# brownvc/gftorf

Hardware: AMD Instinct MI355X
Metric: train iters/sec (fwd+bwd raster) + Mpix/s, 1M Gaussians @ 640x480 ToF (higher is better)
Workload: dtype f32; 1 GPU; 1M Gaussians, 640x480, SH deg 3, RGB+ToF phasor, forward+backward; P=1000000, W=640, H=480, sh_degree=3, P_visible=954168, num_rendered=3638471, longest_tile_list=0

## Files before the change

### gftorf_amd/_lib.py

```python
import ctypes as C
import os

_HERE = os.path.dirname(os.path.abspath(__file__))
LIB_PATH = os.path.join(_HERE, "libgftorf_rast.so")
ABI_VERSION = 16
DEFORM_MAX_INPUTS = 96
ACC_STRIDE = 16

_lib = None

_fp = C.c_void_p


class Config(C.Structure):
    _fields_ = [
        ("P", C.c_int32), ("D", C.c_int32), ("M", C.c_int32), ("M_p", C.c_int32),
        ("W", C.c_int32), ("H", C.c_int32),
        ("tanfovx", C.c_float), ("tanfovy", C.c_float), ("scale_modifier", C.c_float),
        ("near_n", C.c_float), ("far_n", C.c_float), ("depth_range", C.c_float),
        ("phase_offset", C.c_float), ("dc_offset", C.c_float),
        ("use_view_dependent_phase", C.c_int32), ("prefiltered", C.c_int32), ("debug", C.c_int32),
        ("want_backward", C.c_int32),
        ("acc_zeroed", C.c_int32),
        ("grads_zeroed", C.c_int32),
        ("grads_accumulate", C.c_int32),
        ("bg_stride_c", C.c_int64), ("bg_stride_y", C.c_int64), ("bg_stride_x", C.c_int64),
    ]


FORWARD_FIELDS = [
    "bg", "means3D", "colors_precomp", "phasors_precomp", "opacities", "scales", "rotations",
    "cov3D_precomp", "viewmatrix", "projmatrix", "campos", "shs", "shs_p",
    "geom", "img", "binning",
    "out_color", "out_phasor", "out_depth", "out_normal", "out_acc", "out_entropy",
    "out_depth_distortion", "out_amp_distortion", "pixels", "out_distribution", "radii", "acc",
]

BACKWARD_FIELDS = [
    "bg", "means3D", "radii", "scales", "rotations", "cov3D_precomp", "viewmatrix", "projmatrix",
    "campos", "shs", "shs_p", "opacities", "pixels",
    "dL_dout_color", "dL_dout_phasor", "dL_dout_depth", "dL_dout_acc", "dL_dout_depth_distortion",
    "geom", "img", "binning", "acc",
    "dL_dmeans3D", "dL_dmeans2D", "dL_dcolors", "dL_dopacity", "dL_dcov3D", "dL_dsh", "dL_dsh_p",
    "dL_dscales", "dL_drotations", "dL_dphase_offset", "dL_ddc_offset", "det_partials", "dirty_rows", "rows_report",
    "phase_offset_dev", "dc_offset_dev",
]

LAYOUT_FIELDS = [
    "geom_rec_a", "geom_rec_b", "geom_depth", "geom_tiles", "geom_rect", "geom_dirgrad", "geom_clamped", "geom_need",
    "geom_blockhist", "geom_total",
    "img_pix_state", "img_ranges", "img_tile_max", "img_ctrl", "img_tile_cnt", "img_tile_cut", "img_super_tab", "img_tile_cursor",
    "img_tile_order", "img_front_len", "img_unit_flag", "img_resume_state", "img_pix_sums", "img_snaps", "img_total",
    "bin_keys", "bin_point_list", "bin_total",
]

PROFILE_FIELDS = ["preprocess_fwd_ms", "tile_count_ms", "tile_scatter_ms", "tile_sort_ms",
                  "render_fwd_ms", "render_bwd_ms", "preprocess_bwd_ms", "memset_ms"]


class ForwardIO(C.Structure):
    _fields_ = [(n, _fp) for n in FORWARD_FIELDS] + [("grads_zero", _fp), ("grads_zero_bytes", C.c_size_t), ("tile_hints", _fp), ("tile_weights", _fp),
                                                           ("cell_sched", _fp), ("phase_offset_dev", _fp), ("dc_offset_dev", _fp)]


class BackwardIO(C.Structure):
    _fields_ = [(n, _fp) for n in BACKWARD_FIELDS]


class Layout(C.Structure):
    _fields_ = [(n, C.c_size_t) for n in LAYOUT_FIELDS]


class ForwardHints(C.Structure):
    _fields_ = [("binning_instances", C.c_int64), ("max_tile_list", C.c_int64), ("whole_lists", C.c_int64),
                ("use_cell_sched", C.c_int64)]


class ForwardReport(C.Structure):
    _fields_ = [("num_rendered", C.c_int64), ("max_tile_list", C.c_int64), ("list_entries", C.c_int64), ("hinted_tiles", C.c_int64),
                ("sched_misses", C.c_int64)]


class Profile(C.Structure):
    _fields_ = [(n, C.c_double) for n in PROFILE_FIELDS] + [("forward_calls", C.c_int64),
                                                           ("backward_calls", C.c_int64)]


ASSEMBLE_PTRS_IN = ["xyz", "screenspace", "opacity", "scaling", "rotation", "rotation_raw", "feat_color",
                    "feat_phasor", "motion_mask", "d_xyz", "d_rot", "d_sh", "d_sh_p"]
ASSEMBLE_SCALARS = ["d_xyz_scalar", "d_rot_scalar", "d_sh_scalar", "d_sh_p_scalar"]
ASSEMBLE_PTRS_OUT = ["scratch", "out_means3D", "out_means2D", "out_opacity", "out_scales", "out_rotations",
                     "out_shs", "out_shs_p"]
ASSEMBLE_RAW_FLAGS = ["opacity_is_raw", "scaling_is_raw"]
ASSEMBLE_PARTS = ["feat_dc_color", "feat_rest_color", "phase_dc", "phase_rest", "amp_dc", "amp_rest"]
ASSEMBLE_FIELDS = ASSEMBLE_PTRS_IN + ASSEMBLE_SCALARS + ASSEMBLE_PTRS_OUT + ["num_offset_rows"] + ASSEMBLE_RAW_FLAGS + ASSEMBLE_PARTS
ASSEMBLE_BWD_HEAD = ["scratch", "rotation_raw", "d_rot"]
ASSEMBLE_BWD_TAIL = ["g_means3D", "g_means2D", "g_opacity", "g_scales", "g_rotations", "g_shs", "g_shs_p",
                     "g_xyz", "g_screenspace", "g_opacity_in", "g_scaling", "g_rotation", "g_rotation_raw",
                     "g_feat_color", "g_feat_phasor", "g_d_xyz", "g_d_rot", "g_d_sh", "g_d_sh_p"]
ASSEMBLE_BWD_RAW = ["opacity_raw", "scaling_raw", "g_feat_dc_color", "g_feat_rest_color", "g_phase_dc", "g_phase_rest", "g_amp_dc", "g_amp_rest"]
ASSEMBLE_BWD_FIELDS = ASSEMBLE_BWD_HEAD + ["d_rot_scalar"] + ASSEMBLE_BWD_TAIL + ["static_from_raw"] + ASSEMBLE_BWD_RAW


class AssembleIO(C.Structure):
    _fields_ = ([(n, _fp) for n in ASSEMBLE_PTRS_IN] + [(n, C.c_float) for n in ASSEMBLE_SCALARS] +
                [(n, _fp) for n in ASSEMBLE_PTRS_OUT] + [("num_offset_rows", C.c_int64)] +
                [(n, C.c_int32) for n in ASSEMBLE_RAW_FLAGS] + [(n, _fp) for n in ASSEMBLE_PARTS])


class AssembleBwdIO(C.Structure):
    _fields_ = ([(n, _fp) for n in ASSEMBLE_BWD_HEAD] + [("d_rot_scalar", C.c_float)] +
                [(n, _fp) for n in ASSEMBLE_BWD_TAIL] + [("static_from_raw", C.c_int32)] + [(n, _fp) for n in ASSEMBLE_BWD_RAW])


class DeformParams(C.Structure):
    _fields_ = [("linear_w", _fp * 8), ("linear_b", _fp * 8), ("xyz_w", _fp), ("xyz_b", _fp), ("r_w", _fp), ("r_b", _fp),
                ("g_w", _fp), ("g_b", _fp), ("b_w", _fp), ("b_b", _fp)]


DEFORM_FIELDS = [f[0] for f in DeformParams._fields_]


class AdamTensor(C.Structure):
    _fields_ = [("param", _fp), ("grad", _fp), ("exp_avg", _fp), ("exp_avg_sq", _fp), ("n", C.c_int64), ("lr", C.c_double),
                ("step", C.c_int64)]

EXPORTS = [
    "gft_abi_version", "gft_lazy_sort", "gft_last_error", "gft_geom_bytes", "gft_image_bytes", "gft_cell_sched_words", "gft_binning_bytes", "gft_acc_bytes",
    "gft_det_partials_bytes", "gft_get_layout", "gft_binning_capacity", "gft_set_binning_mode", "gft_binning_mode", "gft_set_render_mode", "gft_forward_preprocess", "gft_forward_render", "gft_forward", "gft_forward_enqueue", "gft_backward", "gft_grads_rezero",
    "gft_mark_visible", "gft_profile_enable", "gft_profile_reset", "gft_profile_read",
    "gft_assemble_scratch_bytes", "gft_assemble_forward", "gft_assemble_num_dynamic", "gft_assemble_backward",
    "gft_knn_scratch_bytes", "gft_knn_mean_dist2", "gft_adam_step",
    "gft_deform_inputs", "gft_deform_packed_bytes", "gft_deform_saved_bytes", "gft_deform_scratch_bytes", "gft_deform_pack",
    "gft_deform_forward", "gft_deform_backward", "gft_deform_compact", "gft_deform_rows_work_bytes", "gft_deform_backward_rows",
    "gft_deform_dw_splits", "gft_deform_rows_splits_capacity",
    "gft_ssim_blocks", "gft_ssim_l2_forward", "gft_ssim_l2_backward",
    "gft_image_loss_forward", "gft_image_loss_backward", "gft_pixel_loss_blocks", "gft_pixel_loss_forward", "gft_pixel_loss_backward",
    "gft_grad_norm_scratch_bytes", "gft_grad_norm", "gft_grad_scale",
    "gft_densify_stats", "gft_rows_rank_scratch_bytes", "gft_rows_rank", "gft_rows_rank_dev", "gft_rows_gather", "gft_rows_any_nonzero",
    "gft_densify_plan_scratch_bytes", "gft_densify_classify", "gft_densify_layout", "gft_rows_remap",
    "gft_split_children",
]
FLOW_EXPORTS = ["gft_flow_loss_blocks", "gft_flow_loss_forward", "gft_flow_loss_backward", "gft_flow_points", "gft_flow_project",
                "gft_flow_project_backward"]
FEATURE_EXPORTS = ["gft_render_features", "gft_render_features_backward"]
REG_EXPORTS = ["gft_reg_blocks", "gft_reg_result_words", "gft_reg_forward", "gft_reg_backward"]
REG_PARTIAL_WORDS = 8
REG_MEANS, REG_COUNTS, REG_RECIPS, REG_TOTAL = 0, 4, 6, 10
TOF_EXPORTS = ["gft_tof_depth", "gft_tof_log_blocks", "gft_tof_log_row"]
TOF_PARTIAL_WORDS = 12
TOF_LOG_WORDS, TOF_LOG_MAX_EXTRAS = 24, 8
TOF_LOG_FLOATS = ("sp", "sp_tof", "gsp", "sp_err", "sp_tof_err", "depth_err", "tof_depth_err", "amp_err", "dd", "gs_sp",
                  "gs_sp_visible")
TOF_LOG_VISIBLE, TOF_LOG_PRESENT, TOF_LOG_NUM_EXTRAS, TOF_LOG_SEQ, TOF_LOG_EXTRAS = 11, 12, 13, 14, 16
TOF_HAS_GT_DEPTH, TOF_HAS_DD, TOF_HAS_AMP, TOF_HAS_VISIBLE = 1, 2, 4, 8
QUERY_EXPORTS = ["gft_query_inputs", "gft_query_combine", "gft_query_combine_backward"]
QUERY_MAX_TIMES, QUERY_MAX_OUTPUTS = 4, 4
METRICS_EXPORTS = ["gft_metrics_blocks", "gft_view_metrics", "gft_metrics_reset"]
METRICS_VALUES = ("l1", "psnr", "l1_p", "l2_p", "psnr_p", "l1_d", "l2_d", "l2_d_tof")
METRICS_MAX_PLANES, METRICS_PARTIAL_WORDS = 8, 36
METRICS_ROW_MSE, METRICS_ROW_PSNR, METRICS_ROW_PRESENT, METRICS_ROW_PLANES, METRICS_ROW_WORDS = 8, 16, 24, 25, 28
METRICS_ACC_SUMS, METRICS_ACC_VIEWS, METRICS_ACC_PRESENT, METRICS_ACC_WORDS = 0, 16, 17, 18
METRICS_HAS_COLOUR, METRICS_HAS_TOF, METRICS_HAS_DEPTH, METRICS_HAS_TOF_DEPTH = 1, 2, 4, 8
PRESENT_EXPORTS = ["gft_present_blocks", "gft_present_sheet_bytes", "gft_present_magma", "gft_present_view", "gft_present_ranges",
                   "gft_present_ranges_reset", "gft_present_seismic", "gft_present_quad"]
PRESENT_IMAGES = (("color", 3, "uint8", lambda H, W: (H, W, 3)), ("real", 3, "uint8", lambda H, W: (H, W, 3)),
                  ("imag", 3, "uint8", lambda H, W: (H, W, 3)), ("amp", 1, "uint8", lambda H, W: (H, W)),
                  ("quad", 4, "uint8", lambda H, W: (4, H, W)), ("depth", 4, "uint8", lambda H, W: (H, W, 4)),
                  ("depth_tof", 4, "uint8", lambda H, W: (H, W, 4)), ("depth_norm", 4, "uint8", lambda H, W: (H, W, 4)),
                  ("dd", 1, "uint8", lambda H, W: (H, W)), ("depth_tof_f", 4, "float32", lambda H, W: (H, W)),
                  ("depth_norm_f", 4, "float32", lambda H, W: (H, W)))
PRESENT_HAS_COLOR, PRESENT_HAS_PHASOR, PRESENT_HAS_QUAD, PRESENT_HAS_DEPTH, PRESENT_HAS_ACC, PRESENT_HAS_DD = 1, 2, 4, 8, 16, 32
PRESENT_ALIGN, PRESENT_PARTIAL_WORDS, PRESENT_RANGE_WORDS, PRESENT_MAGMA_ROWS = 16, 2, 6, 257
PRESENT_SEISMIC_ROWS = 257
FLOWVIZ_EXPORTS = ["gft_flowviz_blocks", "gft_flowviz_wheel", "gft_flowviz_images"]
FLOWVIZ_WHEEL_ROWS, FLOWVIZ_IMAGES, FLOWVIZ_RUN = 55, 3, 4
TRACKS_EXPORTS = ["gft_tracks_integrate", "gft_tracks_table_bytes", "gft_tracks_table"]
TRACKS_PARTS = ("index", "xy", "motion", "step_ok")
PLY_EXPORTS = ["gft_ply_pack", "gft_ply_unpack"]
PLY_ROWS, PLY_MAX_SOURCES, PLY_MAX_COLUMNS = 64, 16, 240
PCD_EXPORTS = ["gft_pcd_unproject", "gft_pcd_row_bytes", "gft_pcd_pack", "gft_pcd_unpack", "gft_pcd_create"]
PCD_ROWS, PCD_MAX_ROW_BYTES, PCD_STATUS_WORDS = 256, 128, 2
PCD_MODES = ("torf_init", "ftorf_init", "proxy")
PCD_FIELDS = ("x", "y", "z", "nx", "ny", "nz", "red", "green", "blue", "phase", "amplitude", "seg_red", "seg_green", "seg_blue")


def load():
    global _lib
    if _lib is not None:
        return _lib
    if not os.path.exists(LIB_PATH):
        raise RuntimeError(
            "gftorf_amd: %s is missing. Build it with `python -m gftorf_amd.build` "
            "(hipcc, gfx950). There is no CPU fallback for the rasterizer." % LIB_PATH)
    lib = C.CDLL(LIB_PATH)
    lib.gft_abi_version.restype = C.c_int
    if lib.gft_abi_version() != ABI_VERSION:
        raise RuntimeError("gftorf_amd: libgftorf_rast.so ABI %d != expected %d, rebuild"
                           % (lib.gft_abi_version(), ABI_VERSION))
    lib.gft_last_error.restype = C.c_char_p
    lib.gft_geom_bytes.restype = C.c_size_t
    lib.gft_geom_bytes.argtypes = [C.c_int32]
    lib.gft_image_bytes.restype = C.c_size_t
    lib.gft_image_bytes.argtypes = [C.c_int32, C.c_int32]
    lib.gft_cell_sched_words.restype = C.c_size_t
    lib.gft_cell_sched_words.argtypes = [C.c_int32, C.c_int32]
    lib.gft_binning_bytes.restype = C.c_size_t
    lib.gft_binning_bytes.argtypes = [C.c_int64, C.c_int32, C.c_int32]
    lib.gft_acc_bytes.restype = C.c_size_t
    lib.gft_acc_bytes.argtypes = [C.c_int32]
    lib.gft_det_partials_bytes.restype = C.c_size_t
    lib.gft_det_partials_bytes.argtypes = [C.c_int64, C.c_int32, C.c_int32]
    lib.gft_binning_capacity.restype = C.c_int64
    lib.gft_binning_capacity.argtypes = [C.c_size_t, C.c_int32, C.c_int32]
    lib.gft_set_binning_mode.restype = C.c_int
    lib.gft_set_binning_mode.argtypes = [C.c_int]
    lib.gft_set_render_mode.restype = C.c_int
    lib.gft_set_render_mode.argtypes = [C.c_int]
    lib.gft_binning_mode.restype = C.c_int
    lib.gft_binning_mode.argtypes = [C.POINTER(Config)]
    lib.gft_get_layout.restype = C.c_int
    lib.gft_get_layout.argtypes = [C.c_int32, C.c_int32, C.c_int32, C.c_int64, C.POINTER(Layout)]
    lib.gft_forward_preprocess.restype = C.c_int
    lib.gft_forward_preprocess.argtypes = [C.c_void_p, C.POINTER(Config), C.POINTER(ForwardIO),
                                           C.POINTER(C.c_int64), C.POINTER(C.c_int64)]
    lib.gft_forward_render.restype = C.c_int
    _ptrs = C.POINTER(C.c_void_p)
    lib.gft_adam_step.restype = C.c_int
    lib.gft_adam_step.argtypes = [C.c_void_p, C.c_int32, C.POINTER(AdamTensor), C.c_int64, C.c_void_p, _ptrs, _ptrs, C.c_void_p,
                                  C.c_double, C.c_double, C.c_double, C.c_double, C.c_void_p]
    lib.gft_grad_norm_scratch_bytes.restype = C.c_size_t
    lib.gft_grad_norm_scratch_bytes.argtypes = [C.c_int64, C.c_int32]
    lib.gft_grad_norm.restype = C.c_int
    lib.gft_grad_norm.argtypes = [C.c_void_p, C.c_int32, _ptrs, C.POINTER(C.c_int64), C.c_double, C.c_void_p, C.c_size_t, C.c_void_p]
    lib.gft_grad_scale.restype = C.c_int
    lib.gft_grad_scale.argtypes = [C.c_void_p, C.c_int32, _ptrs, C.POINTER(C.c_int64), C.c_void_p]
    lib.gft_deform_packed_bytes.restype = C.c_size_t
    lib.gft_deform_packed_bytes.argtypes = []
    lib.gft_deform_saved_bytes.restype = C.c_size_t
    lib.gft_deform_saved_bytes.argtypes = [C.c_int64]
    lib.gft_deform_scratch_bytes.restype = C.c_size_t
    lib.gft_deform_scratch_bytes.argtypes = [C.c_int64]
    lib.gft_deform_pack.restype = C.c_int
    lib.gft_deform_inputs.restype = C.c_int
    lib.gft_deform_inputs.argtypes = [C.c_int, C.c_int]
    lib.gft_deform_pack.argtypes = [C.c_void_p, C.c_int, C.c_int, C.POINTER(DeformParams), C.c_void_p]
    lib.gft_deform_forward.restype = C.c_int
    lib.gft_deform_forward.argtypes = [C.c_void_p, C.c_int, C.c_int, C.c_int64, C.c_void_p, C.c_void_p, C.c_int64, C.c_void_p, C.c_void_p,
                                       C.c_void_p, C.c_void_p]
    lib.gft_deform_backward.restype = C.c_int
    lib.gft_deform_backward.argtypes = [C.c_void_p, C.c_int, C.c_int, C.c_int64, C.c_void_p, C.c_void_p, C.c_void_p, C.c_void_p, C.c_void_p,
                                        C.POINTER(DeformParams)]
    lib.gft_deform_compact.restype = C.c_int
    lib.gft_deform_compact.argtypes = [C.c_void_p, C.c_int64, C.c_int64] + [C.c_void_p] * 9
    lib.gft_deform_rows_work_bytes.restype = C.c_size_t
    lib.gft_deform_rows_work_bytes.argtypes = [C.c_int64]
    lib.gft_deform_dw_splits.restype = C.c_int
    lib.gft_deform_dw_splits.argtypes = [C.c_int64]
    lib.gft_deform_rows_splits_capacity.restype = C.c_int
    lib.gft_deform_rows_splits_capacity.argtypes = [C.c_int64]
    lib.gft_deform_backward_rows.restype = C.c_int
    lib.gft_deform_backward_rows.argtypes = [C.c_void_p, C.c_int, C.c_int, C.c_int64, C.c_void_p, C.c_void_p, C.c_void_p, C.c_int64, C.c_void_p,
                                             C.c_void_p, C.c_void_p, C.POINTER(DeformParams), C.c_void_p]
    lib.gft_ssim_blocks.restype = C.c_int64
    lib.gft_ssim_blocks.argtypes = [C.c_int32, C.c_int32, C.c_int32]
    lib.gft_ssim_l2_forward.restype = C.c_int
    lib.gft_ssim_l2_forward.argtypes = [C.c_void_p, C.c_int32, C.c_int32, C.c_int32, C.c_void_p, C.c_void_p, C.POINTER(C.c_float),
                                        C.c_void_p, C.c_void_p]
    lib.gft_ssim_l2_backward.restype = C.c_int
    lib.gft_ssim_l2_backward.argtypes = [C.c_void_p, C.c_int32, C.c_int32, C.c_int32, C.c_void_p, C.c_void_p, C.POINTER(C.c_float),
                                         C.c_void_p, C.c_void_p, C.c_void_p, C.c_float, C.c_float, C.c_void_p]
    _kind_sizes = [C.c_void_p, C.c_int32, C.c_int32, C.c_int32, C.c_int32, C.c_int32, C.c_float, C.c_void_p, C.c_void_p]
    lib.gft_image_loss_forward.restype = C.c_int
    lib.gft_image_loss_forward.argtypes = _kind_sizes + [C.POINTER(C.c_float), C.c_void_p, C.c_void_p]
    lib.gft_image_loss_backward.restype = C.c_int
    lib.gft_image_loss_backward.argtypes = _kind_sizes + [C.POINTER(C.c_float), C.c_void_p, C.c_void_p, C.c_void_p, C.c_float,
                                                          C.c_float, C.c_void_p]
    lib.gft_pixel_loss_blocks.restype = C.c_int64
    lib.gft_pixel_loss_blocks.argtypes = [C.c_int32, C.c_int32, C.c_int32]
    lib.gft_pixel_loss_forward.restype = C.c_int
    lib.gft_pixel_loss_forward.argtypes = _kind_sizes + [C.c_float, C.c_void_p]
    lib.gft_pixel_loss_backward.restype = C.c_int
    lib.gft_pixel_loss_backward.argtypes = _kind_sizes + [C.c_void_p, C.c_float, C.c_void_p]
    _flow_cams = [C.c_void_p, C.c_int32, C.c_int32] + [C.c_void_p] * 5
    lib.gft_flow_loss_blocks.restype = C.c_int64
    lib.gft_flow_loss_blocks.argtypes = [C.c_int32, C.c_int32]
    lib.gft_flow_loss_forward.restype = C.c_int
    lib.gft_flow_loss_forward.argtypes = _flow_cams + [C.c_void_p] * 4 + [C.c_float, C.c_void_p]
    lib.gft_flow_loss_backward.restype = C.c_int
    lib.gft_flow_loss_backward.argtypes = _flow_cams + [C.c_void_p] * 6 + [C.c_float, C.c_void_p, C.c_void_p]
    lib.gft_flow_points.restype = C.c_int
    lib.gft_flow_points.argtypes = _flow_cams + [C.c_void_p, C.c_void_p]
    lib.gft_flow_project.restype = C.c_int
    lib.gft_flow_project.argtypes = [C.c_void_p, C.c_int32, C.c_int32] + [C.c_void_p] * 6
    lib.gft_flow_project_backward.restype = C.c_int
    lib.gft_flow_project_backward.argtypes = [C.c_void_p, C.c_int32, C.c_int32] + [C.c_void_p] * 6
    _feat_frame = [C.c_void_p, C.POINTER(Config)] + [C.c_void_p] * 3 + [C.c_int64, C.c_int32]
    lib.gft_render_features.restype = C.c_int
    lib.gft_render_features.argtypes = _feat_frame + [C.c_void_p] * 3
    lib.gft_render_features_backward.restype = C.c_int
    lib.gft_render_features_backward.argtypes = _feat_frame + [C.c_void_p] * 3
    _reg_inputs = ([C.c_void_p, C.c_int64, C.c_int64, C.c_int64, C.c_void_p, C.c_void_p, C.c_void_p, C.c_int32, C.c_void_p, C.c_int32,
                    C.c_int32, C.c_void_p, C.c_int32])
    _reg_weights = [C.c_void_p, C.c_float, C.c_float, C.c_float, C.c_float]
    lib.gft_reg_blocks.restype = C.c_int64
    lib.gft_reg_blocks.argtypes = [C.c_int64, C.c_int64, C.c_int64]
    lib.gft_reg_result_words.restype = C.c_int64
    lib.gft_reg_result_words.argtypes = []
    lib.gft_reg_forward.restype = C.c_int
    lib.gft_reg_forward.argtypes = _reg_inputs + [C.c_void_p] + _reg_weights + [C.c_void_p, C.c_void_p]
    lib.gft_reg_backward.restype = C.c_int
    lib.gft_reg_backward.argtypes = _reg_inputs + _reg_weights + [C.c_void_p] * 6
    lib.gft_tof_depth.restype = C.c_int
    lib.gft_tof_depth.argtypes = [C.c_void_p, C.c_int64, C.c_void_p, C.c_int64, C.c_void_p, C.c_float, C.c_void_p, C.c_float, C.c_void_p]
    lib.gft_tof_log_blocks.restype = C.c_int64
    lib.gft_tof_log_blocks.argtypes = [C.c_int64, C.c_int64]
    lib.gft_tof_log_row.restype = C.c_int
    lib.gft_tof_log_row.argtypes = [C.c_void_p, C.c_int64, C.c_int64, C.c_void_p, C.c_int64, C.c_void_p, C.c_void_p, C.c_int64, C.c_void_p,
                                    C.c_float, C.c_void_p, C.c_float, C.c_float, C.c_void_p, C.c_void_p, C.c_void_p, C.c_int64, C.c_void_p,
                                    C.c_int32, _ptrs, C.c_int32, C.c_void_p, C.c_void_p, C.c_int64, C.c_void_p]
    lib.gft_query_inputs.restype = C.c_int
    lib.gft_query_inputs.argtypes = [C.c_void_p, C.c_int64, C.c_void_p, C.c_void_p, C.c_void_p, C.c_void_p, C.c_int64, C.c_int32, C.c_float,
                                     C.c_void_p, C.POINTER(C.c_float), C.c_void_p, C.c_void_p]
    lib.gft_query_combine.restype = C.c_int
    lib.gft_query_combine.argtypes = [C.c_void_p, C.c_int64, C.c_int32, C.c_int32, C.c_void_p, C.c_void_p, C.POINTER(C.c_float), _ptrs]
    lib.gft_query_combine_backward.restype = C.c_int
    lib.gft_query_combine_backward.argtypes = [C.c_void_p, C.c_int64, C.c_int32, C.c_int32, _ptrs, C.c_void_p, C.POINTER(C.c_float),
                                               C.c_void_p]
    lib.gft_metrics_blocks.restype = C.c_int64
    lib.gft_metrics_blocks.argtypes = [C.c_int64]
    lib.gft_view_metrics.restype = C.c_int
    lib.gft_view_metrics.argtypes = ([C.c_void_p] + [C.c_int64, C.c_int32, C.c_void_p, C.c_int64, C.c_void_p, C.c_int64] * 2 +
                                     [C.c_void_p, C.c_void_p, C.c_void_p, C.c_int64, C.c_void_p, C.c_float, C.c_void_p, C.c_float,
                                      C.c_void_p, C.c_void_p, C.c_void_p])
    lib.gft_metrics_reset.restype = C.c_int
    lib.gft_metrics_reset.argtypes = [C.c_void_p, C.c_void_p]
    lib.gft_present_blocks.restype = C.c_int64
    lib.gft_present_blocks.argtypes = [C.c_int64]
    lib.gft_present_sheet_bytes.restype = C.c_int64
    lib.gft_present_sheet_bytes.argtypes = [C.c_int32, C.c_int32, C.c_int32, C.POINTER(C.c_int64)]
    lib.gft_present_magma.restype = C.POINTER(C.c_uint8)
    lib.gft_present_magma.argtypes = []
    lib.gft_present_view.restype = C.c_int
    lib.gft_present_view.argtypes = [C.c_void_p, C.c_int32, C.c_int32, C.c_void_p, C.c_int64, C.c_void_p, C.c_int64, C.c_int32, C.c_void_p,
                                     C.c_void_p, C.c_void_p, C.c_void_p, C.POINTER(C.c_float), C.c_void_p, C.c_float, C.c_void_p, C.c_float,
                                     C.c_float, C.c_float, C.c_float, C.c_void_p, C.c_void_p]
    lib.gft_present_ranges.restype = C.c_int
    lib.gft_present_ranges.argtypes = [C.c_void_p, C.c_int64, C.c_void_p, C.c_int64, C.c_void_p, C.c_void_p]
    lib.gft_present_ranges_reset.restype = C.c_int
    lib.gft_present_ranges_reset.argtypes = [C.c_void_p, C.c_void_p]
    lib.gft_present_seismic.restype = C.POINTER(C.c_uint8)
    lib.gft_present_seismic.argtypes = []
    lib.gft_present_quad.restype = C.c_int
    lib.gft_present_quad.argtypes = [C.c_void_p, C.c_int32, C.c_int32, C.c_void_p, C.c_int64, C.POINTER(C.c_int32), C.c_int32, C.c_int32,
                                     C.c_void_p]
    lib.gft_flowviz_blocks.restype = C.c_int64
    lib.gft_flowviz_blocks.argtypes = [C.c_int64]
    lib.gft_flowviz_wheel.restype = C.POINTER(C.c_uint8)
    lib.gft_flowviz_wheel.argtypes = []
# ... 148 lines not shown
```

### gftorf_amd/api.py

```python
import ctypes as C
import struct as _struct
from typing import NamedTuple, Optional

import torch
import torch.nn as nn

from . import _lib


class GaussianRasterizationSettings(NamedTuple):
    image_height: int
    image_width: int
    tanfovx: float
    tanfovy: float
    bg: torch.Tensor
    scale_modifier: float
    viewmatrix: torch.Tensor
    projmatrix: torch.Tensor
    sh_degree: int
    campos: torch.Tensor
    prefiltered: bool
    debug: bool
    near_n: Optional[float] = 0.01
    far_n: Optional[float] = 100.0
# ... 373 lines not shown


def _scratch(nbytes, dev):
    t = torch.empty((nbytes,), device=dev, dtype=torch.uint8)
    if _POISON:
        t.fill_(0x7f)
    return t


def binning_capacity(binning, W, H):
    return int(_lib.load().gft_binning_capacity(binning.numel(), int(W), int(H)))


class _Settings(NamedTuple):
    bg: torch.Tensor
    scale_modifier: float
    viewmatrix: torch.Tensor
    projmatrix: torch.Tensor
    tanfovx: float
    tanfovy: float
    image_height: int
    image_width: int
    sh_degree: int
    campos: torch.Tensor
    prefiltered: bool
    debug: bool
    near_n: float
    far_n: float
    depth_range: float
    use_view_dependent_phase: bool


_PLANE_SPLIT = (3, 7, 1, 3, 1, 1, 1, 1, 3)
_FWD_FMT = "=%dQ" % len(_lib.ForwardIO._fields_)
_BWD_FMT = "=%dQ" % len(_lib.BackwardIO._fields_)
assert _struct.calcsize(_FWD_FMT) == C.sizeof(_lib.ForwardIO) and _struct.calcsize(_BWD_FMT) == C.sizeof(_lib.BackwardIO)


def _p0(t):
    return 0 if t is None else t.data_ptr()


def _save_snapshot(cpu_args, path, note):
    if cpu_args is not None:
        torch.save(cpu_args, path)
        print(note)


def _forward_inputs(s, means3D, sh, sh_p, colors_precomp, phasors_precomp, opacities, scales, rotations, cov3Ds_precomp, H, W):
    dev = means3D.device
    g = lambda t, n: _f32(t, dev, n) if _present(t) else None
    means3D_c = _f32(means3D, dev, "means3D") if means3D.size(0) else means3D
    sh_c, sh_p_c = g(sh, "shs"), g(sh_p, "shs_p")
    colors_c, phasors_c = g(colors_precomp, "colors_precomp"), g(phasors_precomp, "phasors_precomp")
    opac_c = g(opacities, "opacities")
    scales_c, rot_c, cov_c = g(scales, "scales"), g(rotations, "rotations"), g(cov3Ds_precomp, "cov3D_precomp")
    consts = (_f32(s.viewmatrix, dev, "viewmatrix"), _f32(s.projmatrix, dev, "projmatrix"), _f32(s.campos, dev, "campos"))
    return ((means3D_c, opac_c, sh_c, sh_p_c, scales_c, rot_c, cov_c, colors_c, phasors_c), consts,
            _bg_strides(s.bg, H, W, dev))


def _forward_buffers(lib, dev, P, H, W):
    planes = torch.empty((21, H, W), device=dev, dtype=torch.float32)
    radii = torch.empty((P,), device=dev, dtype=torch.int32)
    pixels = torch.empty((P, 1), device=dev, dtype=torch.float32)
    gb = state.geom_bytes.get(P)
    if gb is None:
        gb = state.geom_bytes[P] = int(lib.gft_geom_bytes(P))
    ib = state.image_bytes.get((W, H))
    if ib is None:
        ib = state.image_bytes[(W, H)] = int(lib.gft_image_bytes(W, H))
    return planes, radii, pixels, _scratch(gb, dev), _scratch(ib, dev)


def _pack_forward_io(inputs, consts, bg_c, planes, pixels, radii, geom, img, off_dev):
    means3D_c, opac_c, sh_c, sh_p_c, scales_c, rot_c, cov_c, colors_c, phasors_c = inputs
    P = radii.size(0)
    io = _lib.ForwardIO()
    pl, hw4 = planes.data_ptr(), 4 * planes.size(1) * planes.size(2)
    _struct.pack_into(_FWD_FMT, io, 0,
                      _p0(bg_c), means3D_c.data_ptr() if P else 0, _p0(colors_c), _p0(phasors_c), _p0(opac_c), _p0(scales_c),
                      _p0(rot_c), _p0(cov_c), consts[0].data_ptr(), consts[1].data_ptr(), consts[2].data_ptr(), _p0(sh_c),
                      _p0(sh_p_c), geom.data_ptr(), img.data_ptr(), 0,
                      pl, pl + 3 * hw4, pl + 10 * hw4, pl + 11 * hw4, pl + 14 * hw4, pl + 15 * hw4, pl + 16 * hw4, pl + 17 * hw4,
                      pixels.data_ptr() if P else 0, pl + 18 * hw4, radii.data_ptr() if P else 0, 0, 0, 0, 0, 0, 0,
                      *((0, 0) if off_dev is None else (_p0(off_dev[0]), _p0(off_dev[1]))))
    return io


def _update_hint(key, R, max_list=None, decay=0.95):
    prev_r, prev_l = state.instance_hint.get(key, (0, 0))
    r = max(R, int((prev_r or 0) * decay))
    state.instance_hint[key] = (r, prev_l if max_list is None else max(max_list, int(prev_l * 0.95)))
    if len(state.instance_hint) > state.MAX_SHAPES:
        state.instance_hint.pop(next(iter(state.instance_hint)))
    return r


class _Launch:
    __slots__ = ("lib", "stream", "cfg", "io", "dev", "W", "H", "cam", "use_sched")

    def __init__(self, lib, stream, cfg, io, dev, W, H, cam, use_sched):
        self.lib, self.stream, self.cfg, self.io, self.dev, self.W, self.H = lib, stream, C.byref(cfg), io, dev, W, H
        self.cam, self.use_sched = cam, use_sched

    def alloc_binning(self, cap):
        binning = _scratch(self.lib.gft_binning_bytes(cap, self.W, self.H), self.dev)
        self.io.binning = binning.data_ptr()
        return binning

    def hints(self, cap, list_hint, use_sched=0):
        n_tiles = ((self.W + 15) // 16) * ((self.H + 15) // 16)
        return _lib.ForwardHints(binning_instances=cap, max_tile_list=int(list_hint * _LIST_HEADROOM) + 1,
                                 whole_lists=_whole_lists(self.cam, n_tiles), use_cell_sched=use_sched)



def _forward_no_host_read(fr, st, hint_key, hint, list_hint):
    a = st["np"]
    if int(a[_ST_OVERFLOWS]) != st["seen"]:
        n_over, st["seen"] = int(a[_ST_OVERFLOWS]) - st["seen"], int(a[_ST_OVERFLOWS])
        worst = int(a[_ST_MAX_R])
        _update_hint(hint_key, worst, decay=1)
        raise RuntimeError("gftorf_amd: %d earlier no-host-read forward(s) of this shape had up to %d instances, "
                           "more than their binning buffer held: their outputs were undefined (the buffer has "
                           "been enlarged for the following frames)" % (n_over, worst))
    if a[3]:
        prev_R = int(a[0])
        a[3] = 0
        if fr.cam is not None:
            fr.cam.hinted_tiles = int(a[8])
        if a[1] & 1:
            raise RuntimeError("Point is filtered although prefiltered is set. This shouldn't happen!")
        hint = _update_hint(hint_key, prev_R)
    cap = _guess_cap(hint)
    binning = fr.alloc_binning(cap)
    hints = fr.hints(cap, list_hint)
    _lib.check(fr.lib.gft_forward_enqueue(fr.stream, fr.cfg, C.byref(fr.io), C.byref(hints), st["dev"].data_ptr()))
    st["host"].copy_(st["dev"], non_blocking=True)
    return -1, cap, binning, 0, False


def _forward_first_frame(fr, hint_key):
    _status_of(hint_key, fr.dev, create=True)
    num_rendered, max_list = C.c_int64(0), C.c_int64(0)
    _lib.check(fr.lib.gft_forward_preprocess(fr.stream, fr.cfg, C.byref(fr.io), C.byref(num_rendered), C.byref(max_list)))
    R = int(num_rendered.value)
    cap = _canonical_cap(R)
    binning = fr.alloc_binning(cap)
    _lib.check(fr.lib.gft_forward_render(fr.stream, fr.cfg, C.byref(fr.io), cap, int(max_list.value)))
    return R, cap, binning, int(max_list.value), False


def _forward_hinted(fr, hint, list_hint):
    cap = _guess_cap(hint, (fr.cam.cell_sched.numel() - 4) // 2 if fr.use_sched else 0)
    binning = fr.alloc_binning(cap)
    hints = fr.hints(cap, list_hint, fr.use_sched)
    report = _lib.ForwardReport()
    _lib.check(fr.lib.gft_forward(fr.stream, fr.cfg, C.byref(fr.io), C.byref(hints), C.byref(report)))
    R, max_list = int(report.num_rendered), int(report.max_tile_list)
    if fr.cam is not None:
        fr.cam.take_report(report, fr.use_sched, R <= cap)
    if R <= cap:
        return R, cap, binning, max_list, False
    cap = _canonical_cap(R)
    binning = fr.alloc_binning(cap)
    _lib.check(fr.lib.gft_forward_render(fr.stream, fr.cfg, C.byref(fr.io), cap, max_list))
    return R, cap, binning, max_list, True


def _launch_forward(fr, hint_key, capturing, nowait):
    hint, list_hint = state.instance_hint.get(hint_key, (None, 0))
    st = _status_of(hint_key, fr.dev, create=not capturing) if (nowait and hint is not None) else None
    if st is not None:
        return _forward_no_host_read(fr, st, hint_key, hint, list_hint)
    if nowait and capturing and hint is None:
        raise RuntimeError("gftorf_amd: a forward captured in a graph sizes its binning buffer from earlier frames of the "
                           "shape: render one frame of this shape (%d Gaussians, %dx%d) eagerly first" % hint_key[1:4])
    if nowait and capturing:
        raise RuntimeError("gftorf_amd: no status block for this shape: render one frame of it eagerly before capturing")
    r = _forward_first_frame(fr, hint_key) if hint is None else _forward_hinted(fr, hint, list_hint)
    _update_hint(hint_key, r[0], r[3])
    return r


def native_forward(s, means3D, sh, sh_p, colors_precomp, phasors_precomp, opacities, scales, rotations,
                   cov3Ds_precomp, ph_off, dc_off, want_bw, with_acc, stream=None, hint_slot=0, share_grads=None,
                   pre_launch=None, acc_any_stream=False, nowait=None, off_dev=None):
    lib = _lib.load()
    if means3D.dim() != 2 or means3D.size(1) != 3:
        raise RuntimeError("means3D must have dimensions (num_points, 3)")
    dev = means3D.device
    if dev.type != "cuda":
        raise RuntimeError("gftorf_amd: the rasterizer runs on a HIP device only (means3D is on %s); "
                           "there is no CPU path" % (dev,))
    capturing = torch.cuda.is_current_stream_capturing()
    if nowait is None:
        nowait = capturing or no_host_read
    if capturing and s.debug:
        raise RuntimeError("gftorf_amd: raster_settings.debug synchronises after every stage and cannot be captured in a graph")
    P = means3D.size(0)
    H, W = int(s.image_height), int(s.image_width)

    inputs, consts, bg = _forward_inputs(s, means3D, sh, sh_p, colors_precomp, phasors_precomp, opacities, scales, rotations,
                                         cov3Ds_precomp, H, W)
    means3D_c, opac_c, sh_c, sh_p_c, scales_c, rot_c, cov_c, colors_c, phasors_c = inputs
    cpu_args = None
    if s.debug:
        cpu_args = cpu_deep_copy_tuple((s.bg, means3D, colors_precomp, phasors_precomp, opacities, scales,
                                        rotations, s.scale_modifier, cov3Ds_precomp, s.viewmatrix, s.projmatrix,
                                        s.tanfovx, s.tanfovy, s.image_height, s.image_width, sh, sh_p,
                                        s.sh_degree, s.campos, s.prefiltered, s.debug, s.near_n, s.far_n,
                                        s.depth_range, s.use_view_dependent_phase, ph_off, dc_off))
    planes, radii, pixels, geom, img = _forward_buffers(lib, dev, P, H, W)
    cfg = _make_config(s, P, sh_c.size(1) if sh_c is not None else 0, sh_p_c.size(1) if sh_p_c is not None else 0, H, W,
                       ph_off, dc_off, bg[1:], want_bw)
    io = _pack_forward_io(inputs, consts, bg[0], planes, pixels, radii, geom, img, off_dev)

    lease = prep = None
    if want_bw and with_acc and P:
        lease = _take_acc(lib, dev, P, stream if stream is not None else _lib.raw_stream(dev), acc_any_stream, pooled=not capturing,
                          prezero=nowait and not capturing)
        if not lease.was_zero:
            io.acc = lease.buf.data_ptr()
        prep = prepare_backward(s, means3D_c, opac_c, sh_c, sh_p_c, scales_c, rot_c, cov_c, radii, geom, img, bg, consts,
                                ph_off, dc_off, lease.buf, colors_c is not None, cov_c is not None, want_bw, pixels,
                                share_grads=share_grads, acc_lease=lease, pooled=not capturing, off_dev=off_dev)
    acc_buf = lease.buf if lease is not None else None

    if P == 0:
        planes.zero_()
        R, cap, binning, max_list, restarted = 0, 0, torch.empty((0,), device=dev, dtype=torch.uint8), 0, False
    else:
        if stream is None:
            stream = _lib.raw_stream(dev)
        if pre_launch is not None:
            pre_launch()
        hint_key = (dev.index, P, W, H) if not hint_slot else (dev.index, P, W, H, hint_slot)
        tiles_key = (dev.index, W, H, hint_slot, s.viewmatrix.data_ptr() if _TILE_HINTS_PER_CAMERA else 0)
        cam = state.camera(tiles_key, create=not capturing) if _TILE_HINTS else None
        use_sched = cam.attach(io, lib, dev, W, H, capturing) if cam is not None else 0
        try:
            with _lib.on_device(dev):
                R, cap, binning, max_list, restarted = _launch_forward(
                    _Launch(lib, stream, cfg, io, dev, W, H, cam, use_sched), hint_key, capturing, nowait)
        except Exception:
            _save_snapshot(cpu_args, "snapshot_fw.dump",
                           "\nAn error occured in forward. Please forward snapshot_fw.dump for debugging.")
            raise
        if io.cell_sched:
            cam.sched_seen = True
    if prep is not None:
        prep.cap = cap
    if lease is not None:
        lease.zero = True

    last_call_stats.update(num_rendered=R, binning_instances=cap, restarted=restarted, max_tile_list=max_list)
    last_call_stats["forwards"] = last_call_stats.get("forwards", 0) + 1
    last_call_stats["restarts"] = last_call_stats.get("restarts", 0) + int(restarted)
    if keep_last_buffers:
        last_call_buffers.update(geom=geom, img=img, binning=binning, P=P, W=W, H=H, cap=cap)
    color, phasor, depth, normal, acc, entropy, depth_distortion, amp_distortion, distribution = planes.split(_PLANE_SPLIT)
    return dict(R=R, cap=cap, outputs=(color, phasor, depth, normal, acc, entropy, depth_distortion, amp_distortion,
                                       pixels, distribution, radii),
                geom=geom, binning=binning, img=img, acc=acc_buf, prep=prep, bg=bg, consts=consts, inputs=inputs)


class _Prep:
    __slots__ = ("grads", "cfg", "io", "acc", "acc_lease", "dev", "P", "H", "W", "pool_entry", "cap", "debug_args")

    def __init__(self, grads, cfg, io, acc, acc_lease, dev, P, H, W, pool_entry, debug_args):
        self.grads, self.cfg, self.io, self.acc, self.acc_lease = grads, cfg, io, acc, acc_lease
        self.dev, self.P, self.H, self.W = dev, P, H, W
        self.pool_entry, self.debug_args = pool_entry, debug_args
        self.cap = None


class _GradPlan(NamedTuple):
    shapes: dict
    sizes: dict
    total: int
    split_sizes: list
    layout_key: tuple
    numels: list


def _backward_plan(P, M, M_p, want_colors, want_cov, has_sh, has_sh_p, has_scales):
    plan_key = (P, M, M_p, want_colors, want_cov, has_sh, has_sh_p, has_scales)
    plan = state.bw_plans.get(plan_key)
    if plan is None:
        shapes = dict(means3D=(P, 3), means2D=(P, 3), opacities=(P, 1), colors=(P, 3) if want_colors else None,
                      cov3D=(P, 6) if want_cov else None, sh=(P, M, 3) if has_sh else None,
                      sh_p=(P, M_p, 2) if has_sh_p else None, scales=(P, 3) if has_scales else None,
                      rotations=(P, 4) if has_scales else None)
        sizes = {k: (_prod(v) + 3) // 4 * 4 for k, v in shapes.items() if v is not None}
        if len(state.bw_plans) > 64:
            state.bw_plans.clear()
        plan = state.bw_plans[plan_key] = _GradPlan(shapes, sizes, sum(sizes.values()) + 4, list(sizes.values()) + [4],
                                                    tuple(sorted(sizes.items())), [_prod(shapes[k]) for k in sizes])
    return plan


def _grad_views(buf, plan):
    pieces = buf.split(plan.split_sizes)
    g = dict.fromkeys(plan.shapes)
    for (k, size), piece, n in zip(plan.sizes.items(), pieces, plan.numels):
        g[k] = (piece if n == size else piece[:n]).view(plan.shapes[k])
    g["offsets"] = pieces[-1][:2]
# ... 246 lines not shown
```

### gftorf_amd/csrc/gft_api.hip

```cpp
#include "gft_internal.h"

#include <stdarg.h>
#include <stdio.h>
#include <string.h>
#include <cstdlib>
#include <mutex>
#include <vector>

static thread_local char g_err[512] = "";

int gft_fail(const char* fmt, ...)
{
    va_list ap;
    va_start(ap, fmt);
    vsnprintf(g_err, sizeof(g_err), fmt, ap);
    va_end(ap);
    return 1;
}

extern "C" const char* gft_last_error(void) { return g_err; }
extern "C" int gft_abi_version(void) { return GFT_ABI_VERSION; }
static size_t point_list_slots(int64_t binning_instances, int32_t W, int32_t H)
{
    if (binning_instances <= 0) return 0;
    const size_t T = (size_t)((W + GFT_TILE_X - 1) / GFT_TILE_X) * (size_t)((H + GFT_TILE_Y - 1) / GFT_TILE_Y);
    return T * (size_t)GFT_HEAD_SLOT + (size_t)binning_instances;
}
extern "C" size_t gft_det_partials_bytes(int64_t binning_instances, int32_t W, int32_t H)
{
    return point_list_slots(binning_instances, W, H) * 4 * GFT_ACC_STRIDE * sizeof(float);
}
extern "C" int64_t gft_binning_capacity(size_t bytes, int32_t W, int32_t H)
{
    const size_t T = (size_t)((W + GFT_TILE_X - 1) / GFT_TILE_X) * (size_t)((H + GFT_TILE_Y - 1) / GFT_TILE_Y);
    const size_t fixed = T * (size_t)GFT_HEAD_SLOT * 4 + GFT_ALIGN;
    if (bytes <= fixed) return 0;
    return (int64_t)((bytes - fixed) / 12);
}

static inline size_t align_up(size_t x) { return (x + GFT_ALIGN - 1) & ~(size_t)(GFT_ALIGN - 1); }

void gft_compute_layout(int32_t P, int32_t W, int32_t H, int64_t R, gft_layout* L)
{
    memset(L, 0, sizeof(*L));
    const size_t p = (size_t)(P > 0 ? P : 0);
    size_t o = 0;
    L->geom_rec_a = o;    o = align_up(o + p * 32);
    L->geom_rec_b = o;    o = align_up(o + p * 32);
    L->geom_depth = o;    o = align_up(o + p * 4);
    L->geom_tiles = o;    o = align_up(o + p * 4);
    L->geom_rect = o;     o = align_up(o + p * 8);
    L->geom_dirgrad = o;  o = align_up(o + p * 64);
    L->geom_clamped = o;  o = align_up(o + p);
    L->geom_need = o;     o = align_up(o + p);
    L->geom_blockhist = o; o = align_up(o + ((p + BIN_CHUNK - 1) / BIN_CHUNK) * GFT_BLOCKHIST_TILES * 2);
    L->geom_total = o;

    const size_t n = (size_t)W * (size_t)H;
    const size_t T = (size_t)((W + GFT_TILE_X - 1) / GFT_TILE_X) * (size_t)((H + GFT_TILE_Y - 1) / GFT_TILE_Y);
    o = 0;
    L->img_pix_state = o;   o = align_up(o + n * 16);
    L->img_ranges = o;      o = align_up(o + T * 8);
    L->img_tile_max = o;    o = align_up(o + T * 4 * 4);
    L->img_ctrl = o;        o += (GFT_CTRL_WORDS + GFT_TICKET_WORDS) * 4;
    L->img_tile_cnt = o;    o += T * 4;
    L->img_tile_cut = o;    o += T * 4;
    L->img_super_tab = o;   o = align_up(o + 4 * (size_t)GFT_SUPER_CELLS * 4);
    L->img_tile_cursor = o; o = align_up(o + T * 4);
    L->img_tile_order = o;  o = align_up(o + T * 4);
    L->img_front_len = o;   o = align_up(o + T * 4);
    L->img_unit_flag = o;   o = align_up(o + T * 16);
    L->img_resume_state = o; o = align_up(o + n * 64);
    L->img_pix_sums = o;    o = align_up(o + n * 32);
    L->img_snaps = o;       o = align_up(o + 4 * T * (size_t)(gft_bwd_segments(T) - 1) * GFT_SNAP_F4 * 64 * 16);
    L->img_total = o;

    const size_t r = (size_t)(R > 0 ? R : 0);
    o = 0;
    L->bin_keys = o;        o = align_up(o + r * 8);
    L->bin_point_list = o;  o = align_up(o + (r ? T * (size_t)GFT_HEAD_SLOT + r : 0) * 4);
    L->bin_total = o + GFT_ALIGN;
}

GeomView gft_geom_view(void* base, const gft_layout& L)
{
    char* b = (char*)base;
    GeomView g;
    g.rec_a = (float4*)(b + L.geom_rec_a);
    g.rec_b = (float4*)(b + L.geom_rec_b);
    g.depth = (float*)(b + L.geom_depth);
    g.tiles = (uint32_t*)(b + L.geom_tiles);
    g.rect = (ushort4*)(b + L.geom_rect);
    g.dirgrad = (float4*)(b + L.geom_dirgrad);
    g.clamped = (uint8_t*)(b + L.geom_clamped);
    g.need = (uint8_t*)(b + L.geom_need);
    g.blockhist = (uint16_t*)(b + L.geom_blockhist);
    return g;
}

ImgView gft_img_view(void* base, const gft_layout& L)
{
    char* b = (char*)base;
    ImgView v;
    v.pix_state = (float4*)(b + L.img_pix_state);
    v.ranges = (uint2*)(b + L.img_ranges);
    v.tile_max = (uint32_t*)(b + L.img_tile_max);
    v.ctrl = (uint32_t*)(b + L.img_ctrl);
    v.tile_cnt = (uint32_t*)(b + L.img_tile_cnt);
    v.tile_cut = (uint32_t*)(b + L.img_tile_cut);
    v.super_tab = (uint32_t*)(b + L.img_super_tab);
    v.tile_cursor = (uint32_t*)(b + L.img_tile_cursor);
    v.tile_order = (uint32_t*)(b + L.img_tile_order);
    v.front_len = (uint32_t*)(b + L.img_front_len);
    v.unit_flag = (uint32_t*)(b + L.img_unit_flag);
    v.resume_state = (float4*)(b + L.img_resume_state);
    v.pix_sums = (float4*)(b + L.img_pix_sums);
    v.snaps = (float4*)(b + L.img_snaps);
    return v;
}

BinView gft_bin_view(void* base, const gft_layout& L)
{
    char* b = (char*)base;
    BinView v;
    v.keys = (uint64_t*)(b + L.bin_keys);
    v.point_list = (uint32_t*)(b + L.bin_point_list);
    return v;
}

extern "C" size_t gft_geom_bytes(int32_t P)
{
    gft_layout L;
    gft_compute_layout(P, 16, 16, 0, &L);
    return L.geom_total + GFT_ALIGN;
}

extern "C" size_t gft_image_bytes(int32_t W, int32_t H)
{
    gft_layout L;
    gft_compute_layout(0, W, H, 0, &L);
    return L.img_total + GFT_ALIGN;
}

extern "C" size_t gft_cell_sched_words(int32_t W, int32_t H)
{
    gft_config c;
    memset(&c, 0, sizeof(c));
    c.W = W; c.H = H; c.near_n = 0.01f; c.far_n = 100.f;
    return (W > 0 && H > 0 && gft_tile_pull_ok(c)) ? gft_cell_sched_words_of(c) : 0;
}

extern "C" size_t gft_binning_bytes(int64_t R, int32_t W, int32_t H)
{
    gft_layout L;
    gft_compute_layout(0, W, H, R, &L);
    return L.bin_total;
}

extern "C" size_t gft_acc_bytes(int32_t P)
{
    const size_t p = (size_t)(P > 0 ? P : 0);
    return (p * GFT_ACC_STRIDE + 2 * ((p + 63) / 64) + 64) * sizeof(float);
}

extern "C" int gft_get_layout(int32_t P, int32_t W, int32_t H, int64_t R, gft_layout* out)
{
    if (!out) return gft_fail("gft_get_layout: out is NULL");
    gft_compute_layout(P, W, H, R, out);
    return 0;
}

enum Stage { ST_PRE_FWD, ST_TILE_COUNT, ST_TILE_SCATTER, ST_TILE_SORT, ST_RENDER_FWD, ST_RENDER_BWD, ST_PRE_BWD, ST_MEMSET, ST_COUNT };

struct Profiler {
    std::mutex mu;
    bool on = false;
    struct Rec { int stage; hipEvent_t a, b; };
    std::vector<Rec> pending;
    std::vector<hipEvent_t> pool;
    double ms[ST_COUNT] = {0};
    int64_t fwd = 0, bwd = 0;
    hipEvent_t get()
    {
        if (!pool.empty()) { hipEvent_t e = pool.back(); pool.pop_back(); return e; }
        hipEvent_t e;
        if (hipEventCreate(&e) != hipSuccess) return nullptr;
        return e;
    }
    void drain()
    {
        for (auto& r : pending) {
            float t = 0.f;
            if (hipEventSynchronize(r.b) == hipSuccess && hipEventElapsedTime(&t, r.a, r.b) == hipSuccess) ms[r.stage] += t;
            pool.push_back(r.a);
            pool.push_back(r.b);
        }
        pending.clear();
    }
};
static Profiler g_prof;

struct StageTimer {
    hipStream_t s; int stage; hipEvent_t a = nullptr, b = nullptr; bool on;
    StageTimer(hipStream_t s_, int st) : s(s_), stage(st), on(g_prof.on)
    {
        if (on) {
            std::lock_guard<std::mutex> lk(g_prof.mu);
            a = g_prof.get(); b = g_prof.get();
            if (a && b) (void)hipEventRecord(a, s); else on = false;
        }
    }
    ~StageTimer()
    {
        if (on) {
            (void)hipEventRecord(b, s);
            std::lock_guard<std::mutex> lk(g_prof.mu);
            g_prof.pending.push_back({stage, a, b});
        }
    }
};

extern "C" int gft_profile_enable(int on) { std::lock_guard<std::mutex> lk(g_prof.mu); g_prof.on = on != 0; return 0; }

extern "C" int gft_profile_reset(void)
{
    std::lock_guard<std::mutex> lk(g_prof.mu);
    g_prof.drain();
    memset(g_prof.ms, 0, sizeof(g_prof.ms));
    g_prof.fwd = g_prof.bwd = 0;
    return 0;
}

extern "C" int gft_profile_read(gft_profile* out)
{
    if (!out) return gft_fail("gft_profile_read: out is NULL");
    std::lock_guard<std::mutex> lk(g_prof.mu);
    g_prof.drain();
    out->preprocess_fwd_ms = g_prof.ms[ST_PRE_FWD];
    out->tile_count_ms = g_prof.ms[ST_TILE_COUNT];
    out->tile_scatter_ms = g_prof.ms[ST_TILE_SCATTER];
    out->tile_sort_ms = g_prof.ms[ST_TILE_SORT];
    out->render_fwd_ms = g_prof.ms[ST_RENDER_FWD];
    out->render_bwd_ms = g_prof.ms[ST_RENDER_BWD];
    out->preprocess_bwd_ms = g_prof.ms[ST_PRE_BWD];
    out->memset_ms = g_prof.ms[ST_MEMSET];
    out->forward_calls = g_prof.fwd;
    out->backward_calls = g_prof.bwd;
    return 0;
}

struct SideFill {
    hipStream_t stream = nullptr;
    hipEvent_t after_main = nullptr, filled = nullptr;
    bool pending = false;
};
static std::mutex g_side_mu;
static SideFill g_side[64];

static SideFill* side_of_current_device()
{
    int dev = 0;
    if (hipGetDevice(&dev) != hipSuccess || dev < 0 || dev >= 64) return nullptr;
    std::lock_guard<std::mutex> lk(g_side_mu);
    SideFill& f = g_side[dev];
    if (!f.stream) {
        if (hipStreamCreateWithFlags(&f.stream, hipStreamNonBlocking) != hipSuccess) { f.stream = nullptr; return nullptr; }
        if (hipEventCreateWithFlags(&f.after_main, hipEventDisableTiming) != hipSuccess ||
            hipEventCreateWithFlags(&f.filled, hipEventDisableTiming) != hipSuccess)
            return nullptr;
    }
    return &f;
}

#define GFT_STAGE(stream, cfg, name, call)                                                   \
    do {                                                                                     \
        hipError_t e_ = (call);                                                              \
        if (e_ != hipSuccess) return gft_fail("%s: launch failed: %s", name, hipGetErrorString(e_)); \
        if ((cfg)->debug) {                                                                  \
            e_ = hipStreamSynchronize(stream);                                               \
            if (e_ != hipSuccess) return gft_fail("%s: %s", name, hipGetErrorString(e_));    \
        }                                                                                    \
    } while (0)

__global__ __launch_bounds__(256) void k_zero_fill(uint4* __restrict__ p16, size_t n16, uint8_t* __restrict__ tail, size_t ntail)
{
    const size_t stride = (size_t)gridDim.x * 256;
    for (size_t i = (size_t)blockIdx.x * 256 + threadIdx.x; i < n16; i += stride) p16[i] = make_uint4(0u, 0u, 0u, 0u);
    if (blockIdx.x == 0 && threadIdx.x < ntail) tail[threadIdx.x] = 0;
}

__global__ void k_post_empty(uint32_t* status) { status[GFT_CTRL_SEQ] = 1u; }

hipError_t gft_zero_async(void* ptr, size_t bytes, hipStream_t s)
{
    if (!ptr || !bytes) return hipSuccess;
    uint8_t* p = static_cast<uint8_t*>(ptr);
    const size_t head = (16 - ((uintptr_t)p & 15)) & 15;
    if (head && head < bytes) {
        hipLaunchKernelGGL(k_zero_fill, dim3(1), dim3(256), 0, s, (uint4*)nullptr, (size_t)0, p, head);
        p += head; bytes -= head;
    } else if (head) {
        hipLaunchKernelGGL(k_zero_fill, dim3(1), dim3(256), 0, s, (uint4*)nullptr, (size_t)0, p, bytes);
// ... 53 lines not shown
    *dev_slot = g_mail.dev + (size_t)slot * GFT_CTRL_WORDS;
    *host_slot = g_mail.host + (size_t)slot * GFT_CTRL_WORDS;
    g_mail.host[(size_t)slot * GFT_CTRL_WORDS + GFT_CTRL_FLAGS] = 0u;
    return 0;
}

static int mailbox_wait(hipStream_t s, volatile uint32_t* host_slot, uint32_t seq, uint32_t out[GFT_CTRL_WORDS])
{
    for (;;) {
        for (int i = 0; i < 4096; i++) {
            if (__atomic_load_n(&host_slot[GFT_CTRL_SEQ], __ATOMIC_ACQUIRE) == seq) goto ready;
            __builtin_ia32_pause();
        }
        const hipError_t q = hipStreamQuery(s);
        if (q == hipSuccess) {
            if (__atomic_load_n(&host_slot[GFT_CTRL_SEQ], __ATOMIC_ACQUIRE) == seq) goto ready;
            return gft_fail("forward: the stream drained but the tile scan never reported");
        }
        if (q != hipErrorNotReady) return gft_fail("forward: %s", hipGetErrorString(q));
    }
ready:
    for (int i = 0; i < GFT_CTRL_WORDS; i++) out[i] = host_slot[i];
    return 0;
}

static int check_stage1(const gft_config* cfg, const gft_forward_io* io, const char* who)
{
    if (!io->means3D || !io->opacities || !io->viewmatrix || !io->projmatrix || !io->campos || !io->geom ||
        !io->radii || !io->pixels)
        return gft_fail("%s: required pointer is NULL", who);
    if ((io->shs == nullptr) == (io->colors_precomp == nullptr))
        return gft_fail("Please provide excatly one of either SHs or precomputed colors!");
    if ((io->scales == nullptr || io->rotations == nullptr) == (io->cov3D_precomp == nullptr))
        return gft_fail("Please provide exactly one of either scale/rotation pair or precomputed 3D covariance!");
    if ((io->shs != nullptr) != (cfg->M > 0) || (io->shs_p != nullptr) != (cfg->M_p > 0))
        return gft_fail("M / M_p do not match the presence of shs / shs_p");
    if (!io->img) return gft_fail("%s: img buffer is NULL", who);
    return 0;
}

static int check_stage2(const gft_forward_io* io, const char* who)
{
    if (!io->img || !io->bg || !io->out_color || !io->out_phasor || !io->out_depth || !io->out_normal ||
        !io->out_acc || !io->out_entropy || !io->out_depth_distortion || !io->out_amp_distortion ||
        !io->out_distribution)
        return gft_fail("%s: required pointer is NULL", who);
    return 0;
}

static bool lazy_sort_enabled()
{
    static const bool on = [] { const char* e = getenv("GFT_LAZY_SORT"); return e ? atoi(e) != 0 : true; }();
    return on;
}

extern "C" int gft_lazy_sort(void) { return lazy_sort_enabled() ? 1 : 0; }

static std::atomic<int> g_binning_mode{-1};
extern "C" int gft_set_binning_mode(int mode)
{
    g_binning_mode.store(mode < 0 ? -1 : (mode ? 1 : 0));
    return 0;
}
static bool pull_enabled(const gft_config* cfg)
{
    int m = g_binning_mode.load();
    if (m < 0) {
        const char* e = getenv("GFT_LAZY_BIN");
        m = e ? (atoi(e) != 0) : 1;
        g_binning_mode.store(m);
    }
    return m != 0 && lazy_sort_enabled() && gft_tile_pull_ok(*cfg);
}
extern "C" int gft_binning_mode(const gft_config* cfg) { return (cfg && pull_enabled(cfg)) ? 1 : 0; }

static std::atomic<int> g_render_mode{-2};
extern "C" int gft_set_render_mode(int mode)
{
    g_render_mode.store(mode < 0 ? -2 : (mode ? 1 : 0));
    return 0;
}
int gft_render_mode()
{
    int m = g_render_mode.load();
    if (m == -2) {
        const char* e = getenv("GFT_FWD_SEG");
        m = e ? (atoi(e) != 0 ? 1 : 0) : -1;
        g_render_mode.store(m);
    }
    return m;
}

static int enqueue_count(hipStream_t s, const gft_config* cfg, const gft_forward_io* io, const GeomView& g, const ImgView& im,
                         uint32_t* mail_dev, uint32_t seq, bool pull, int64_t status_cap = -1);

static int enqueue_stage1(hipStream_t s, const gft_config* cfg, const gft_forward_io* io, const GeomView& g,
                          const ImgView& im, uint32_t* mail_dev, uint32_t seq, bool pull, bool count = true, int64_t status_cap = -1)
{
    {
        StageTimer t(s, ST_PRE_FWD);
        GFT_STAGE(s, cfg, "preprocess_fwd", gft_launch_preprocess_fwd(s, *cfg, *io, g, im, mail_dev, pull));
    }
    if (io->grads_zero && io->grads_zero_bytes) {
        SideFill* f = side_of_current_device();
        if (!f) return gft_fail("forward: no side stream for the gradient fill");
        GFT_CHECK_HIP(hipEventRecord(f->after_main, s));
        GFT_CHECK_HIP(hipStreamWaitEvent(f->stream, f->after_main, 0));
        GFT_CHECK_HIP(gft_zero_async(io->grads_zero, io->grads_zero_bytes, f->stream));
        GFT_CHECK_HIP(hipEventRecord(f->filled, f->stream));
        f->pending = true;
    }
    return count ? enqueue_count(s, cfg, io, g, im, mail_dev, seq, pull, status_cap) : 0;
}

static int enqueue_count(hipStream_t s, const gft_config* cfg, const gft_forward_io* io, const GeomView& g, const ImgView& im,
                         uint32_t* mail_dev, uint32_t seq, bool pull, int64_t status_cap)
{
    StageTimer t(s, ST_TILE_COUNT);
    if (pull) {
        BinView none;
        none.keys = nullptr; none.point_list = nullptr;
        const int T = ((cfg->W + GFT_TILE_X - 1) / GFT_TILE_X) * ((cfg->H + GFT_TILE_Y - 1) / GFT_TILE_Y);
        GFT_STAGE(s, cfg, "super_count", gft_launch_super_bin(s, *cfg, g, im, none, mail_dev, seq, 0, 0u,
                                                              gft_fwd_segmented(T) ? nullptr : io->tile_hints, io->cell_sched, status_cap));
    } else {
        GFT_STAGE(s, cfg, "tile_count", gft_launch_tile_count(s, *cfg, g, im, mail_dev, seq, status_cap));
    }
    return 0;
}

static int enqueue_stage2(hipStream_t s, const gft_config* cfg, const gft_forward_io* io, const GeomView& g,
                          const ImgView& im, const BinView& b, bool binned, int64_t max_tile_list, bool check_cap,
                          uint32_t cap, bool pull, bool whole_lists, uint32_t* sched_mail = nullptr, uint32_t sched_seq = 0u)
{
    float* clear = (io->acc && cfg->want_backward && cfg->P > 0) ? io->acc : nullptr;
    const size_t clear_bytes = (size_t)cfg->P * GFT_ACC_STRIDE * sizeof(float);
    const bool lazy = binned && lazy_sort_enabled();
    pull = pull && binned;
    if (pull) {
        {
            StageTimer t(s, ST_TILE_SCATTER);
            if (sched_mail) {
                const int T0 = ((cfg->W + GFT_TILE_X - 1) / GFT_TILE_X) * ((cfg->H + GFT_TILE_Y - 1) / GFT_TILE_Y);
                GFT_STAGE(s, cfg, "super_append", gft_launch_super_bin(s, *cfg, g, im, b, sched_mail, sched_seq, 2, cap,
                                                                       gft_fwd_segmented(T0) ? nullptr : io->tile_hints, io->cell_sched));
            } else {
                GFT_STAGE(s, cfg, "super_scatter", gft_launch_super_bin(s, *cfg, g, im, b, nullptr, 0u, 1, cap));
            }
        }
        {
            StageTimer t(s, ST_TILE_SORT);
            const int T = ((cfg->W + GFT_TILE_X - 1) / GFT_TILE_X) * ((cfg->H + GFT_TILE_Y - 1) / GFT_TILE_Y);
            const uint32_t* th = gft_fwd_segmented(T) ? nullptr : io->tile_hints;
            GFT_STAGE(s, cfg, "tile_pull", gft_launch_tile_pull(s, *cfg, g, im, b, cap, clear, clear_bytes, th, whole_lists && th));
        }
        {
            StageTimer t(s, ST_PRE_FWD);
            GFT_STAGE(s, cfg, "appearance", gft_launch_appearance(s, *cfg, *io, g, im, cap));
        }
    } else if (binned) {
        {
            StageTimer t(s, ST_TILE_SCATTER);
            GFT_STAGE(s, cfg, "tile_scatter", gft_launch_tile_scatter(s, *cfg, g, im, b, cap, (int64_t)cap));
        }
        {
            StageTimer t(s, ST_TILE_SORT);
            if (lazy)
                GFT_STAGE(s, cfg, "tile_front", gft_launch_tile_front(s, *cfg, im, b, cap, clear, clear_bytes));
            else
                GFT_STAGE(s, cfg, "tile_sort", gft_launch_tile_sort(s, *cfg, max_tile_list, im, b, cap, clear, clear_bytes));
        }
    } else if (clear) {
        GFT_CHECK_HIP(gft_zero_async(clear, clear_bytes, s));
    }
    {
        StageTimer t(s, ST_RENDER_FWD);
        GFT_STAGE(s, cfg, "render_fwd", gft_launch_render_fwd(s, *cfg, *io, g, im, b, check_cap, cap, lazy ? 1 : 0, pull));
    }
    if (lazy) {
        {
            StageTimer t(s, ST_TILE_SORT);
            if (pull)
                GFT_STAGE(s, cfg, "tail_build", gft_launch_tail_build(s, *cfg, *io, g, im, b, cap, cfg->want_backward != 0));
            else
                GFT_STAGE(s, cfg, "tile_tail", gft_launch_tile_tail(s, *cfg, g, im, b, cap, cfg->want_backward != 0));
        }
        if (!(pull && gft_tail_resumes())) {
            StageTimer t(s, ST_RENDER_FWD);
            GFT_STAGE(s, cfg, "render_resume", gft_launch_render_fwd(s, *cfg, *io, g, im, b, check_cap, cap, 2, pull));
        }
    }
    if (g_prof.on) { std::lock_guard<std::mutex> lk(g_prof.mu); g_prof.fwd++; }
    return 0;
}

extern "C" int gft_forward_preprocess(void* hip_stream, const gft_config* cfg, const gft_forward_io* io,
                                      int64_t* num_rendered, int64_t* max_tile_list)
{
    if (max_tile_list) *max_tile_list = 0;
    if (check_config(cfg)) return 1;
    if (!io || !num_rendered) return gft_fail("gft_forward_preprocess: NULL argument");
    *num_rendered = 0;
    if (cfg->P == 0) return 0;
    if (check_stage1(cfg, io, "gft_forward_preprocess")) return 1;
    hipStream_t s = (hipStream_t)hip_stream;
    gft_layout L;
    gft_compute_layout(cfg->P, cfg->W, cfg->H, 0, &L);
    GeomView g = gft_geom_view(io->geom, L);
    ImgView im = gft_img_view(io->img, L);
    uint32_t* mail_dev; volatile uint32_t* mail_host; uint32_t seq;
    if (mailbox_acquire(&mail_dev, &mail_host, &seq)) return 1;
    if (enqueue_stage1(s, cfg, io, g, im, mail_dev, seq, pull_enabled(cfg))) return 1;
    uint32_t host[GFT_CTRL_WORDS];
    if (mailbox_wait(s, mail_host, seq, host)) return 1;
    if (host[GFT_CTRL_FLAGS] & 1u)
        return gft_fail("Point is filtered although prefiltered is set. This shouldn't happen!");
    *num_rendered = (int64_t)host[GFT_CTRL_TOTAL];
    if (max_tile_list) *max_tile_list = (int64_t)host[GFT_CTRL_MAXCNT];
    return 0;
}

extern "C" int gft_forward_render(void* hip_stream, const gft_config* cfg, const gft_forward_io* io,
                                  int64_t binning_instances, int64_t max_tile_list)
{
    if (check_config(cfg)) return 1;
    if (!io) return gft_fail("gft_forward_render: io is NULL");
    if (check_stage2(io, "gft_forward_render")) return 1;
    if (binning_instances < 0 || binning_instances > 0xffffffffll) return gft_fail("gft_forward_render: bad instance count");
    if (binning_instances > 0 && !io->binning) return gft_fail("gft_forward_render: binning buffer is NULL");
    if (cfg->P > 0 && (!io->geom || !io->radii || !io->pixels)) return gft_fail("gft_forward_render: geom/radii/pixels NULL");
    hipStream_t s = (hipStream_t)hip_stream;
    const int64_t R = cfg->P == 0 ? 0 : binning_instances;
    gft_layout L;
    gft_compute_layout(cfg->P, cfg->W, cfg->H, R, &L);
    GeomView g = gft_geom_view(io->geom, L);
    ImgView im = gft_img_view(io->img, L);
    BinView b = gft_bin_view(io->binning, L);
    const bool pull = cfg->P > 0 && pull_enabled(cfg);
    if (cfg->P == 0 || (pull && R == 0)) {
        const int gx = (cfg->W + GFT_TILE_X - 1) / GFT_TILE_X, gy = (cfg->H + GFT_TILE_Y - 1) / GFT_TILE_Y;
        GFT_CHECK_HIP(gft_zero_async(im.ranges, (size_t)gx * gy * sizeof(uint2), s));
        if (cfg->P == 0) GFT_CHECK_HIP(gft_zero_async(im.ctrl, GFT_CTRL_WORDS * sizeof(uint32_t), s));
    }
    return enqueue_stage2(s, cfg, io, g, im, b, R > 0, max_tile_list, cfg->P > 0, (uint32_t)R, pull, io->tile_hints != nullptr);
}

extern "C" int gft_forward(void* hip_stream, const gft_config* cfg, const gft_forward_io* io,
                           const gft_forward_hints* hints, gft_forward_report* report)
{
    if (report) memset(report, 0, sizeof(*report));
    if (check_config(cfg)) return 1;
    if (!io || !hints || !report) return gft_fail("gft_forward: NULL argument");
    if (check_stage2(io, "gft_forward")) return 1;
    const int64_t binning_instances = hints->binning_instances;
    if (binning_instances < 0 || binning_instances > 0xffffffffll) return gft_fail("gft_forward: bad instance count");
    if (cfg->P == 0) return gft_forward_render(hip_stream, cfg, io, 0, 0);
    if (check_stage1(cfg, io, "gft_forward")) return 1;
    if (binning_instances > 0 && !io->binning) return gft_fail("gft_forward: binning buffer is NULL");
    hipStream_t s = (hipStream_t)hip_stream;
    gft_layout L;
    gft_compute_layout(cfg->P, cfg->W, cfg->H, binning_instances, &L);
    GeomView g = gft_geom_view(io->geom, L);
    ImgView im = gft_img_view(io->img, L);
    BinView b = gft_bin_view(io->binning, L);
    uint32_t* mail_dev; volatile uint32_t* mail_host; uint32_t seq;
    if (mailbox_acquire(&mail_dev, &mail_host, &seq)) return 1;
    const bool pull = pull_enabled(cfg);
    const bool by_sched = pull && binning_instances > 0 && io->cell_sched != nullptr && hints->use_cell_sched != 0;
    if (enqueue_stage1(s, cfg, io, g, im, mail_dev, seq, pull, !by_sched)) return 1;
    if (pull && binning_instances == 0) {
        const int gx = (cfg->W + GFT_TILE_X - 1) / GFT_TILE_X, gy = (cfg->H + GFT_TILE_Y - 1) / GFT_TILE_Y;
        GFT_CHECK_HIP(gft_zero_async(im.ranges, (size_t)gx * gy * sizeof(uint2), s));
    }
    const uint32_t cap = (uint32_t)binning_instances;
    if (enqueue_stage2(s, cfg, io, g, im, b, binning_instances > 0, hints->max_tile_list, true, cap, pull, hints->whole_lists != 0,
                       by_sched ? mail_dev : nullptr, seq))
        return 1;
    uint32_t host[GFT_CTRL_WORDS];
    if (mailbox_wait(s, mail_host, seq, host)) return 1;
    if (by_sched && ((host[GFT_CTRL_FLAGS] & 2u) || host[GFT_CTRL_TOTAL] > cap)) {
        const size_t T = (size_t)((cfg->W + GFT_TILE_X - 1) / GFT_TILE_X) * (size_t)((cfg->H + GFT_TILE_Y - 1) / GFT_TILE_Y);
        GFT_CHECK_HIP(gft_zero_async(im.ctrl, (GFT_CTRL_WORDS + GFT_TICKET_WORDS + 2 * T + GFT_SUPER_CELLS) * sizeof(uint32_t), s));
        if (mailbox_acquire(&mail_dev, &mail_host, &seq)) return 1;
        mail_host[GFT_CTRL_FLAGS] = host[GFT_CTRL_FLAGS] & 1u;
        const bool render_again = host[GFT_CTRL_TOTAL] <= cap;
        if (enqueue_count(s, cfg, io, g, im, mail_dev, seq, pull)) return 1;
        if (render_again &&
            enqueue_stage2(s, cfg, io, g, im, b, true, hints->max_tile_list, true, cap, pull, hints->whole_lists != 0))
            return 1;
        if (mailbox_wait(s, mail_host, seq, host)) return 1;
        report->sched_misses = 1;
    }
    if (host[GFT_CTRL_FLAGS] & 1u)
        return gft_fail("Point is filtered although prefiltered is set. This shouldn't happen!");
    report->num_rendered = (int64_t)host[GFT_CTRL_TOTAL];
    report->max_tile_list = (int64_t)host[GFT_CTRL_MAXCNT];
    report->list_entries = pull ? (int64_t)host[GFT_CTRL_ENTRIES] : (int64_t)host[GFT_CTRL_TOTAL];
    report->hinted_tiles = pull ? (int64_t)host[GFT_CTRL_NHINT] : 0;
    if (!lazy_sort_enabled() && hints->max_tile_list > 0 && hints->max_tile_list <= GFT_SHORT_LIST_MAX &&
        host[GFT_CTRL_MAXCNT] > GFT_SHORT_LIST_MAX && host[GFT_CTRL_TOTAL] <= cap && binning_instances > 0) {
        GFT_CHECK_HIP(gft_zero_async(io->pixels, (size_t)cfg->P * sizeof(float), s));
        GFT_STAGE(s, cfg, "tile_sort_long", gft_launch_tile_sort_long(s, *cfg, im, b, cap));
        GFT_STAGE(s, cfg, "render_fwd", gft_launch_render_fwd(s, *cfg, *io, g, im, b, true, cap, 0, false));
    }
    return 0;
}

// ... 120 lines not shown
```

### gftorf_amd/csrc/gft_internal.h

```cpp
#pragma once
#include <hip/hip_runtime.h>
#include <stdint.h>
#include <stddef.h>
#include "gftorf_rast.h"

#include <atomic>
#include <cstdlib>

#define GFT_ALIGN 256

inline hipError_t gft_lds_opt_in(const void* kernel, size_t bytes, std::atomic<uint64_t>& done)
{
    int dev = 0;
    hipError_t e = hipGetDevice(&dev);
    if (e != hipSuccess) return e;
    const uint64_t bit = dev >= 0 && dev < 64 ? 1ull << dev : 0ull;
    if (bit && (done.load(std::memory_order_acquire) & bit)) return hipSuccess;
    e = hipFuncSetAttribute(kernel, hipFuncAttributeMaxDynamicSharedMemorySize, (int)bytes);
    if (e == hipSuccess && bit) done.fetch_or(bit, std::memory_order_release);
    return e;
}
#define GFT_BLOCK 256
#define GFT_NUM_ACC 15

struct GeomView {
    float4* rec_a;
    float4* rec_b;
    float* depth;
    uint32_t* tiles;
    ushort4* rect;
    float4* dirgrad;
    uint8_t* clamped;
    uint8_t* need;
    uint16_t* blockhist;
};

struct ImgView {
    float4* pix_state;
    float4* pix_sums;
    float4* snaps;
    uint2* ranges;
    uint32_t* tile_max;
    uint32_t* ctrl;
    uint32_t* tile_cnt;
    uint32_t* tile_cut;
    uint32_t* super_tab;
    uint32_t* tile_cursor;
    uint32_t* tile_order;
    uint32_t* front_len;
    uint32_t* unit_flag;
    float4* resume_state;
};

struct BinView {
    uint64_t* keys;
    uint32_t* point_list;
};

#define GFT_CTRL_TOTAL 0
#define GFT_CTRL_FLAGS 1
#define GFT_CTRL_MAXCNT 2
#define GFT_CTRL_NFLAG 4
#define GFT_CTRL_DONE 3
#define GFT_CTRL_SEQ 3
#define GFT_CTRL_ENTRIES 5
#define GFT_CTRL_POOLCUR 6
#define GFT_CTRL_DONE2 7
#define GFT_CTRL_NHINT 8
#define GFT_CTRL_RSUM 9
#define GFT_CTRL_FWDORDER 10
#define GFT_CTRL_ORDER_OK 11
#define GFT_CTRL_WORDS 16
__device__ __forceinline__ void gft_status_sticky(uint32_t* mail, uint32_t post, uint32_t R)
{
    if (!post) return;
    mail[GFT_STATUS_CAP] = post - 1u;
    if (R > post - 1u) {
        __hip_atomic_fetch_add(&mail[GFT_STATUS_OVERFLOWS], 1u, __ATOMIC_RELAXED, __HIP_MEMORY_SCOPE_SYSTEM);
        __hip_atomic_fetch_max(&mail[GFT_STATUS_MAX_R], R, __ATOMIC_RELAXED, __HIP_MEMORY_SCOPE_SYSTEM);
    }
}
#define GFT_TICKET_WORDS 32
#define GFT_SUPER_MAX 1024
#define GFT_SLAB_MAX 16
#define GFT_SUPER_CELLS (GFT_SUPER_MAX * GFT_SLAB_MAX)
#define GFT_DEPTH_BINS 4096
#define GFT_HEAD_SLOT 2048u
#define GFT_HEAD_DIRECT 2048u
#define GFT_HEAD_TARGET 940u
#define GFT_NO_TAIL 0xffffffffu
#define GFT_BLOCKHIST_TILES 2048
#ifndef BIN_THREADS
#define BIN_THREADS 1024
#endif
#ifndef BIN_ITEMS
#define BIN_ITEMS 4
#endif
#define BIN_CHUNK (BIN_THREADS * BIN_ITEMS)
#define GFT_SHORT_LIST_MAX 4096

#ifndef GFT_SEG_LEN
#define GFT_SEG_LEN 256
#endif
inline int gft_bwd_segments(size_t T)
{
    static const int cap = [] { const char* e = getenv("GFT_BWD_NSEG"); const int v = e ? atoi(e) : 0; return v > 0 ? (v > 8 ? 8 : v) : 8; }();
    const size_t v = 4 * (T ? T : 1);
    const size_t n = 65536 / v;
    return n < 1 ? 1 : (n > (size_t)cap ? cap : (int)n);
}
inline int gft_fwd_seg_waves(int T)
{
    static const int force = [] { const char* e = getenv("GFT_FWD_SEG_WAVES"); return e ? atoi(e) : 0; }();
    if (force > 0) return force > 8 ? 8 : force;
    const int n = 6144 / (4 * (T > 0 ? T : 1));
    return n < 1 ? 1 : (n > 8 ? 8 : n);
}
int gft_render_mode();
inline bool gft_fwd_segmented(int T) { return gft_render_mode() != 0 && gft_fwd_seg_waves(T) > 1; }
#define GFT_FWD_ORDER_MAX_TILES 4096
inline bool gft_fwd_ordered(int T) { return !gft_fwd_segmented(T) && T <= GFT_FWD_ORDER_MAX_TILES; }
#define GFT_SNAP_F4 3

void gft_compute_layout(int32_t P, int32_t W, int32_t H, int64_t R, gft_layout* L);
GeomView gft_geom_view(void* base, const gft_layout& L);
ImgView gft_img_view(void* base, const gft_layout& L);
BinView gft_bin_view(void* base, const gft_layout& L);

int gft_fail(const char* fmt, ...);
inline int gft_launched(const char* who)
{
    const hipError_t err = hipGetLastError();
    return err == hipSuccess ? 0 : gft_fail("%s: %s", who, hipGetErrorString(err));
}
hipError_t gft_zero_async(void* ptr, size_t bytes, hipStream_t s);
#define GFT_CHECK_HIP(expr)                                                          \
    do {                                                                             \
        hipError_t e_ = (expr);                                                      \
        if (e_ != hipSuccess)                                                        \
            return gft_fail("%s failed: %s (%s:%d)", #expr, hipGetErrorString(e_),   \
                            __FILE__, __LINE__);                                     \
    } while (0)

hipError_t gft_launch_preprocess_fwd(hipStream_t s, const gft_config& c, const gft_forward_io& io,
                                     const GeomView& g, const ImgView& im, uint32_t* mail, bool defer_appearance);
hipError_t gft_launch_appearance(hipStream_t s, const gft_config& c, const gft_forward_io& io, const GeomView& g,
                                 const ImgView& im, uint32_t cap);
hipError_t gft_launch_tile_count(hipStream_t s, const gft_config& c, const GeomView& g, const ImgView& im,
                                 uint32_t* mail, uint32_t seq, int64_t status_cap = -1);
hipError_t gft_launch_tile_scatter(hipStream_t s, const gft_config& c, const GeomView& g, const ImgView& im,
                                   const BinView& b, uint32_t cap, int64_t expect);
hipError_t gft_launch_tile_sort(hipStream_t s, const gft_config& c, int64_t max_tile_list, const ImgView& im,
                                const BinView& b, uint32_t cap, float* clear, size_t clear_bytes);
hipError_t gft_launch_tile_front(hipStream_t s, const gft_config& c, const ImgView& im, const BinView& b, uint32_t cap,
                                 float* clear, size_t clear_bytes);
hipError_t gft_launch_tile_tail(hipStream_t s, const gft_config& c, const GeomView& g, const ImgView& im,
                                const BinView& b, uint32_t cap, bool want_order);
hipError_t gft_launch_tile_sort_long(hipStream_t s, const gft_config& c, const ImgView& im, const BinView& b,
                                     uint32_t cap);
bool gft_tile_pull_ok(const gft_config& c);
bool gft_tail_resumes();
struct SuperShape { int gx, gy, T, sshift, sgx, sgy, NS, K, kshift; uint32_t near_bits; int bin_shift; };
SuperShape gft_super_shape(const gft_config& c);
hipError_t gft_launch_super_bin(hipStream_t s, const gft_config& c, const GeomView& g, const ImgView& im, const BinView& b,
                                uint32_t* mail, uint32_t seq, int pass, uint32_t cap, const uint32_t* hints = nullptr,
                                uint32_t* sched = nullptr, int64_t status_cap = -1);
size_t gft_cell_sched_words_of(const gft_config& c);
hipError_t gft_launch_tile_pull(hipStream_t s, const gft_config& c, const GeomView& g, const ImgView& im, const BinView& b,
                                uint32_t cap, float* clear, size_t clear_bytes, const uint32_t* hints, bool whole_lists);
hipError_t gft_launch_tail_build(hipStream_t s, const gft_config& c, const gft_forward_io& io, const GeomView& g,
                                 const ImgView& im, const BinView& b, uint32_t cap, bool want_order);
hipError_t gft_launch_render_fwd(hipStream_t s, const gft_config& c, const gft_forward_io& io,
                                 const GeomView& g, const ImgView& im, const BinView& b, bool check_cap, uint32_t cap,
                                 int lazy, bool pull, bool segmented = true);
hipError_t gft_launch_render_bwd(hipStream_t s, const gft_config& c, const gft_backward_io& io,
                                 const GeomView& g, const ImgView& im, const BinView& b, bool lazy, uint32_t cap);
hipError_t gft_launch_preprocess_bwd(hipStream_t s, const gft_config& c, const gft_backward_io& io,
                                     const GeomView& g);
hipError_t gft_launch_grads_rezero(hipStream_t s, const gft_config& c, const gft_backward_io& io);
hipError_t gft_launch_mark_visible(hipStream_t s, int32_t P, const float* means3D,
                                   const float* view, float near_n, float far_n, uint8_t* present);


#define GFT_DPP_ROW_SHR(n) (0x110 + (n))
#define GFT_DPP_ROW_BCAST15 0x142
#define GFT_DPP_ROW_BCAST31 0x143

__device__ __forceinline__ float gft_offset_value(const float* dev, float scalar)
{
    return dev != nullptr ? *dev : scalar;
}

__device__ __forceinline__ float gft_wave_sum_to_lane63(float v)
{
    v += __int_as_float(__builtin_amdgcn_update_dpp(0, __float_as_int(v), GFT_DPP_ROW_SHR(1), 0xf, 0xf, false));
    v += __int_as_float(__builtin_amdgcn_update_dpp(0, __float_as_int(v), GFT_DPP_ROW_SHR(2), 0xf, 0xf, false));
    v += __int_as_float(__builtin_amdgcn_update_dpp(0, __float_as_int(v), GFT_DPP_ROW_SHR(4), 0xf, 0xf, false));
    v += __int_as_float(__builtin_amdgcn_update_dpp(0, __float_as_int(v), GFT_DPP_ROW_SHR(8), 0xf, 0xf, false));
    v += __int_as_float(__builtin_amdgcn_update_dpp(0, __float_as_int(v), GFT_DPP_ROW_BCAST15, 0xa, 0xf, false));
    v += __int_as_float(__builtin_amdgcn_update_dpp(0, __float_as_int(v), GFT_DPP_ROW_BCAST31, 0xc, 0xf, false));
    return v;
}

__device__ __forceinline__ uint32_t gft_wave_sum_u32_to_lane63(uint32_t v)
{
    v += (uint32_t)__builtin_amdgcn_update_dpp(0, (int)v, GFT_DPP_ROW_SHR(1), 0xf, 0xf, false);
    v += (uint32_t)__builtin_amdgcn_update_dpp(0, (int)v, GFT_DPP_ROW_SHR(2), 0xf, 0xf, false);
    v += (uint32_t)__builtin_amdgcn_update_dpp(0, (int)v, GFT_DPP_ROW_SHR(4), 0xf, 0xf, false);
    v += (uint32_t)__builtin_amdgcn_update_dpp(0, (int)v, GFT_DPP_ROW_SHR(8), 0xf, 0xf, false);
    v += (uint32_t)__builtin_amdgcn_update_dpp(0, (int)v, GFT_DPP_ROW_BCAST15, 0xa, 0xf, false);
    v += (uint32_t)__builtin_amdgcn_update_dpp(0, (int)v, GFT_DPP_ROW_BCAST31, 0xc, 0xf, false);
    return v;
}

__device__ __forceinline__ void gft_get_rect(float px, float py, int radius, int gx, int gy,
                                             int& x0, int& y0, int& x1, int& y1)
{
    const float r = (float)radius;
    x0 = min(gx, max(0, (int)((px - r) / 16.0f)));
    y0 = min(gy, max(0, (int)((py - r) / 16.0f)));
    x1 = min(gx, max(0, (int)((((px + r) + 16.0f) - 1.0f) / 16.0f)));
    y1 = min(gy, max(0, (int)((((py + r) + 16.0f) - 1.0f) / 16.0f)));
}

__device__ __forceinline__ uint32_t gft_depth_bin(uint32_t dbits, uint32_t near_bits, int shift)
{
    const uint32_t d = dbits > near_bits ? dbits - near_bits : 0u;
    const uint32_t b = d >> shift;
    return b < GFT_DEPTH_BINS ? b : GFT_DEPTH_BINS - 1u;
}

__device__ __forceinline__ bool gft_splat_reaches_box(const float4& a0, const float4& a1, float bx0, float by0, float bw, float bh)
{
    const float ca = a0.z, cb = a0.w, cc = a1.x, op = a1.y;
    const float det = ca * cc - cb * cb;
    const float tau = __logf(255.0f * op);
    if (!(op >= 1.0f / 255.0f)) return false;
    if (!(det > 0.0f && ca > 0.0f && cc > 0.0f)) return true;
    const float ux0 = bx0 - a0.x, ux1 = ux0 + bw;
    const float uy0 = by0 - a0.y, uy1 = uy0 + bh;
    const float X = fminf(fmaxf(0.0f, ux0), ux1), Y = fminf(fmaxf(0.0f, uy0), uy1);
    const float ys = fminf(fmaxf(-cb * X * __frcp_rn(cc), uy0), uy1);
    const float xs = fminf(fmaxf(-cb * Y * __frcp_rn(ca), ux0), ux1);
    const float q1 = ca * X * X + 2.0f * cb * X * ys + cc * ys * ys;
    const float q2 = ca * xs * xs + 2.0f * cb * xs * Y + cc * Y * Y;
    return fminf(q1, q2) <= 2.0f * tau * 1.0005f + 0.01f;
}
__device__ __forceinline__ bool gft_splat_reaches_quadrant(const float4& a0, const float4& a1, float qx0, float qy0)
{
    return gft_splat_reaches_box(a0, a1, qx0, qy0, 7.0f, 7.0f);
}

#define GFT_FLAG_SET 0x80000000u
__device__ __forceinline__ uint32_t gft_flag_word(unsigned long long unsaturated)
{
    uint32_t c = (uint32_t)(unsaturated | (unsaturated >> 32));
    c |= c >> 16;
    c |= c >> 8;
    c &= 0xffu;
    const uint32_t x0 = (uint32_t)__builtin_ctz(c), x1 = 31u - (uint32_t)__builtin_clz(c);
    const uint32_t y0 = (uint32_t)__builtin_ctzll(unsaturated) >> 3, y1 = (63u - (uint32_t)__builtin_clzll(unsaturated)) >> 3;
    return GFT_FLAG_SET | x0 | (y0 << 3) | (x1 << 6) | (y1 << 9);
}
__device__ __forceinline__ bool gft_splat_reaches_flagged(uint32_t flag, const float4& a0, const float4& a1, float qx0, float qy0)
{
    if (!flag) return false;
    const uint32_t x0 = flag & 7u, y0 = (flag >> 3) & 7u, x1 = (flag >> 6) & 7u, y1 = (flag >> 9) & 7u;
    return gft_splat_reaches_box(a0, a1, qx0 + (float)x0, qy0 + (float)y0, (float)(x1 - x0), (float)(y1 - y0));
}

__device__ inline void gft_tile_order_block(int T, const uint32_t* __restrict__ quad_max, uint32_t* __restrict__ order,
                                            const uint32_t* __restrict__ flag = nullptr)
{
    constexpr int PER = 16;
    __shared__ uint32_t s_max;
    __shared__ uint32_t cnt[16][64];
    const int tid = threadIdx.x, lane = tid & 63, wave = tid >> 6;
    if (tid == 0) s_max = 0;
    for (int i = tid; i < 16 * 64; i += (int)blockDim.x) (&cnt[0][0])[i] = 0;
    auto weight = [&](int t) -> uint32_t {
        const uint4 q = reinterpret_cast<const uint4*>(quad_max)[t];
        uint32_t w = max(max(q.x, q.y), max(q.z, q.w));
        if (flag) {
            const uint4 f = reinterpret_cast<const uint4*>(flag)[t];
            if ((f.x | f.y | f.z | f.w) != 0u) w = 0xffffffffu;
        }
        return w;
    };
    uint32_t w[PER];
    uint32_t m = 0;
    {
        uint4 q[PER];
#pragma unroll
        for (int k = 0; k < PER; k++) q[k] = reinterpret_cast<const uint4*>(quad_max)[min(tid + k * (int)blockDim.x, T - 1)];
#pragma unroll
        for (int k = 0; k < PER; k++) w[k] = max(max(q[k].x, q[k].y), max(q[k].z, q[k].w));
        if (flag) {
#pragma unroll
            for (int k = 0; k < PER; k++) q[k] = reinterpret_cast<const uint4*>(flag)[min(tid + k * (int)blockDim.x, T - 1)];
#pragma unroll
            for (int k = 0; k < PER; k++)
                if ((q[k].x | q[k].y | q[k].z | q[k].w) != 0u) w[k] = 0xffffffffu;
        }
    }
#pragma unroll
    for (int k = 0; k < PER; k++) {
        if (tid + k * (int)blockDim.x >= T) w[k] = 0u;
        if (w[k] != 0xffffffffu) m = max(m, w[k]);
    }
    for (int t = tid + PER * (int)blockDim.x; t < T; t += (int)blockDim.x) {
        const uint32_t x = weight(t);
        if (x != 0xffffffffu) m = max(m, x);
    }
#pragma unroll
    for (int d = 32; d > 0; d >>= 1) m = max(m, (uint32_t)__shfl_xor((int)m, d, 64));
    __syncthreads();
    if (lane == 0 && m) atomicMax(&s_max, m);
    __syncthreads();
    const float scale = 64.0f / (float)(s_max + 1u);
    auto bucket = [&](uint32_t x) -> uint32_t { return x == 0xffffffffu ? 0u : 63u - min(63u, (uint32_t)((float)x * scale)); };
#pragma unroll
    for (int k = 0; k < PER; k++)
// ... 29 lines not shown
```

### gftorf_amd/csrc/k_pull.hip

```cpp
#include "gft_internal.h"
#include "gft_sort.h"
#include "gft_render_walk.h"
#include "gft_appearance.h"

#include <cstdlib>
#include <cstring>

#ifdef GFT_PHASE_DBG
#define PHASE_DBG(a) ((a).dbg)
#else
#define PHASE_DBG(a) 0
#endif

namespace {

#define TPULL_KEYS GFT_HEAD_SLOT
#define TPULL_KEYS_BIG 3328u
#define HEAD_DIRECT GFT_HEAD_DIRECT
#define PULL_GROUP_MAX 31u
#define PULL_WINDOW 2048u
#define HEAD_TARGET GFT_HEAD_TARGET
#define TAIL_LDS_KEYS 4096u
#define TAIL_ITEMS 4
#define TAIL_THREADS 512

__device__ __forceinline__ bool entry_hits(uint64_t e, uint32_t lx, uint32_t ly)
{
    const uint32_t rel = (uint32_t)(e >> 32);
    return lx >= (rel & 31u) && lx < ((rel >> 10) & 31u) && ly >= ((rel >> 5) & 31u) && ly < ((rel >> 15) & 31u);
}
__device__ __forceinline__ uint32_t entry_bin(uint64_t e) { return (uint32_t)(e >> 52); }

struct SuperArgs {
    int P;
    SuperShape sh;
    const ushort4* __restrict__ rect;
    const float* __restrict__ depth;
    uint32_t* cnt_copy;
    uint32_t* cur_copy;
    uint32_t* st_cnt;
    uint32_t* st_start;
    int copies;
    uint64_t* sl_ent;
    uint32_t* ctrl;
    uint32_t* mail; uint32_t seq;
    uint32_t cap;
    uint32_t post;
    const uint32_t* __restrict__ hints;
    uint32_t stage_cap;
    uint32_t* sched;
};

__device__ inline void super_write_sched(uint32_t* sched, const uint32_t* counts, int cells, uint32_t* s_wt, uint32_t* s_carry)
{
    const int tid = threadIdx.x, lane = tid & 63, wave = tid >> 6;
    constexpr int PER = 4;
    if (tid == 0) *s_carry = 0;
    __syncthreads();
    for (int c0 = 0; c0 < cells; c0 += PER * BIN_THREADS) {
        const int first = c0 + tid * PER;
        uint32_t cap[PER], sum = 0;
#pragma unroll
        for (int k = 0; k < PER; k++) {
            const uint32_t c = first + k < cells ? __hip_atomic_load(&counts[first + k], __ATOMIC_RELAXED, __HIP_MEMORY_SCOPE_AGENT) : 0u;
            cap[k] = first + k < cells ? c + (c >> 2) + 64u : 0u;
            sum += cap[k];
        }
        uint32_t x = sum;
#pragma unroll
        for (int d = 1; d < 64; d <<= 1) {
            const uint32_t y = __shfl_up(x, d, 64);
            if (lane >= d) x += y;
        }
        if (lane == 63) s_wt[wave] = x;
        __syncthreads();
        uint32_t woff = 0;
        for (int w = 0; w < wave; w++) woff += s_wt[w];
        const uint32_t carry = *s_carry;
        uint32_t run = carry + woff + x - sum;
#pragma unroll
        for (int k = 0; k < PER; k++)
            if (first + k < cells) { sched[first + k] = run; sched[cells + first + k] = cap[k]; run += cap[k]; }
        __syncthreads();
        if (tid == BIN_THREADS - 1) *s_carry = carry + woff + x;
        __syncthreads();
    }
    if (tid == 0) { sched[2 * cells] = (uint32_t)cells; sched[2 * cells + 1] = 1u; }
}

template <int PASS, bool STAGED = false>
__global__ __launch_bounds__(BIN_THREADS) void k_super_bin(SuperArgs a)
{
    extern __shared__ __attribute__((aligned(16))) uint32_t sb_dyn[];
    const int cells = a.sh.NS * a.sh.K;
    uint32_t* s_cnt = sb_dyn;
    uint32_t* s_first = sb_dyn + cells;
    uint32_t* s_loc = sb_dyn + 2 * cells;
    __shared__ uint32_t s_last, s_sum, s_carry;
    __shared__ uint32_t s_wt[BIN_THREADS / 64];
    const int tid = threadIdx.x, lane = tid & 63, wave = tid >> 6;
    if (PASS == 1 && a.ctrl[GFT_CTRL_TOTAL] > a.cap) return;
    for (int i = tid; i < cells; i += BIN_THREADS) s_cnt[i] = 0;
    if (tid == 0) s_sum = 0;
    __syncthreads();
    if (PASS == 2 && blockIdx.x == 0 && a.hints) {
        uint32_t nh = 0;
        for (int t = tid; t < a.sh.T; t += BIN_THREADS) nh += a.hints[t] != 0u ? 1u : 0u;
        nh = gft_wave_sum_u32_to_lane63(nh);
        if (lane == 63 && nh) atomicAdd(&a.ctrl[GFT_CTRL_NHINT], nh);
    }
    const int base = blockIdx.x * BIN_CHUNK;
    const int K = a.sh.K, sgx = a.sh.sgx, ss = a.sh.sshift;
    ushort4 r4[BIN_ITEMS];
    uint32_t bin[BIN_ITEMS];
    uint32_t mine = 0;
    uint32_t dbits[BIN_ITEMS];
#pragma unroll
    for (int u = 0; u < BIN_ITEMS; u++) {
        const int idx = min(base + u * BIN_THREADS + tid, a.P - 1);
        r4[u] = a.rect[idx];
        dbits[u] = __float_as_uint(a.depth[idx]);
    }
#pragma unroll
    for (int u = 0; u < BIN_ITEMS; u++) {
        const bool in = base + u * BIN_THREADS + tid < a.P;
        if (!in) r4[u] = make_ushort4(0, 0, 0, 0);
        const uint32_t tiles = (uint32_t)(r4[u].z - r4[u].x) * (uint32_t)(r4[u].w - r4[u].y);
        bin[u] = tiles ? gft_depth_bin(dbits[u], a.sh.near_bits, a.sh.bin_shift) : 0u;
        mine += tiles;
    }
    if (PASS != 1) {
        mine = gft_wave_sum_u32_to_lane63(mine);
        if (lane == 63 && mine) atomicAdd(&s_sum, mine);
    }
#pragma unroll
    for (int u = 0; u < BIN_ITEMS; u++) {
        if (!(r4[u].z > r4[u].x && r4[u].w > r4[u].y)) continue;
        const int sx0 = r4[u].x >> ss, sx1 = (r4[u].z - 1) >> ss, sy0 = r4[u].y >> ss, sy1 = (r4[u].w - 1) >> ss;
        const int slab = (int)(bin[u] >> a.sh.kshift);
        for (int sy = sy0; sy <= sy1; sy++)
            for (int sx = sx0; sx <= sx1; sx++) atomicAdd(&s_cnt[(sy * sgx + sx) * K + slab], 1u);
    }
    __syncthreads();
    if (PASS == 0) {
        const int rot = (int)(((uint64_t)blockIdx.x * (uint64_t)cells) / gridDim.x);
        for (int i = tid; i < cells; i += BIN_THREADS) {
            const int cidx = i + rot >= cells ? i + rot - cells : i + rot;
            const uint32_t c = s_cnt[cidx];
            if (c) atomicAdd(&a.cnt_copy[(size_t)(blockIdx.x & (a.copies - 1)) * cells + cidx], c);
        }
        if (tid == 0 && s_sum) atomicAdd(&a.ctrl[GFT_CTRL_RSUM], s_sum);
        asm volatile("s_waitcnt vmcnt(0)" ::: "memory");
        __syncthreads();
        if (tid == 0) {
            const uint32_t G = min((uint32_t)GFT_TICKET_WORDS, gridDim.x), grp = blockIdx.x % G;
            const uint32_t members = (gridDim.x - grp + G - 1u) / G;
            uint32_t last = 0u;
            if (atomicAdd(&a.ctrl[GFT_CTRL_WORDS + grp], 1u) == members - 1u)
                last = atomicAdd(&a.ctrl[GFT_CTRL_DONE], 1u) == G - 1u ? 1u : 0u;
            s_last = last;
        }
        __syncthreads();
        if (!s_last) return;
        if (tid == 0) s_carry = 0;
        __syncthreads();
        const int C = a.copies;
        constexpr int PER = 4;
        for (int c0 = 0; c0 < cells; c0 += PER * BIN_THREADS) {
            const int first = c0 + tid * PER;
            uint32_t v[8][PER];
#pragma unroll
            for (int cp = 0; cp < 8; cp++)
#pragma unroll
                for (int k = 0; k < PER; k++)
                    v[cp][k] = __hip_atomic_load(&a.cnt_copy[(size_t)min(cp, C - 1) * cells + min(first + k, cells - 1)],
                                                 __ATOMIC_RELAXED, __HIP_MEMORY_SCOPE_AGENT);
            uint32_t tot[PER], mine_sum = 0;
#pragma unroll
            for (int k = 0; k < PER; k++) {
                tot[k] = 0;
#pragma unroll
                for (int cp = 0; cp < 8; cp++) {
                    if (cp >= C || first + k >= cells) v[cp][k] = 0u;
                    tot[k] += v[cp][k];
                }
                mine_sum += tot[k];
            }
            uint32_t x = mine_sum;
#pragma unroll
            for (int d = 1; d < 64; d <<= 1) {
                const uint32_t y = __shfl_up(x, d, 64);
                if (lane >= d) x += y;
            }
            if (lane == 63) s_wt[wave] = x;
            __syncthreads();
            uint32_t woff = 0;
            for (int w = 0; w < wave; w++) woff += s_wt[w];
            const uint32_t carry = s_carry;
            uint32_t run = carry + woff + x - mine_sum;
#pragma unroll
            for (int k = 0; k < PER; k++) {
                const int cell = first + k;
                if (cell < cells) {
                    a.st_cnt[cell] = tot[k];
                    a.st_start[cell] = run;
                    uint32_t inner = run;
#pragma unroll
                    for (int cp = 0; cp < 8; cp++) {
                        if (cp < C) a.cur_copy[(size_t)cp * cells + cell] = inner;
                        inner += v[cp][k];
                    }
                }
                run += tot[k];
            }
            __syncthreads();
            if (tid == BIN_THREADS - 1) s_carry = carry + woff + x;
            __syncthreads();
        }
        const uint32_t entries_total = s_carry;
        if (a.sched) super_write_sched(a.sched, a.st_cnt, cells, s_wt, &s_carry);
        uint32_t nh = 0;
        if (a.hints) {
            for (int t = tid; t < a.sh.T; t += BIN_THREADS) nh += a.hints[t] != 0u ? 1u : 0u;
            nh = gft_wave_sum_u32_to_lane63(nh);
            if (tid == 0) s_sum = 0;
            __syncthreads();
            if (lane == 63 && nh) atomicAdd(&s_sum, nh);
            __syncthreads();
        }
        if (tid == 0) {
            const uint32_t R = __hip_atomic_load(&a.ctrl[GFT_CTRL_RSUM], __ATOMIC_RELAXED, __HIP_MEMORY_SCOPE_AGENT);
            a.ctrl[GFT_CTRL_TOTAL] = R;
            a.ctrl[GFT_CTRL_ENTRIES] = entries_total;
            a.ctrl[GFT_CTRL_MAXCNT] = 0u;
            a.ctrl[GFT_CTRL_NHINT] = a.hints ? s_sum : 0u;
            if (a.mail) {
                a.mail[GFT_CTRL_TOTAL] = R;
                a.mail[GFT_CTRL_MAXCNT] = 0u;
                a.mail[GFT_CTRL_ENTRIES] = entries_total;
                a.mail[GFT_CTRL_NHINT] = a.hints ? s_sum : 0u;
                gft_status_sticky(a.mail, a.post, R);
                __hip_atomic_store(&a.mail[GFT_CTRL_SEQ], a.seq, __ATOMIC_RELEASE, __HIP_MEMORY_SCOPE_SYSTEM);
            }
        }
        return;
    }
    uint32_t* s_stage_cell_base = sb_dyn + 3 * cells;
    uint64_t* stage_ent = reinterpret_cast<uint64_t*>(s_stage_cell_base + (cells & 1));
    uint16_t* stage_cell = reinterpret_cast<uint16_t*>(stage_ent + a.stage_cap);
    uint32_t n_wg = 0;
    if (STAGED) {
        const int PERC = (cells + BIN_THREADS - 1) / BIN_THREADS;
        const int c0 = tid * PERC;
        uint32_t sum = 0;
        for (int k = 0; k < PERC; k++) sum += c0 + k < cells ? s_cnt[c0 + k] : 0u;
        uint32_t x = sum;
#pragma unroll
        for (int d = 1; d < 64; d <<= 1) {
            const uint32_t y = __shfl_up(x, d, 64);
            if (lane >= d) x += y;
        }
        if (lane == 63) s_wt[wave] = x;
        __syncthreads();
        uint32_t woff = 0, tot = 0;
        for (int w = 0; w < BIN_THREADS / 64; w++) {
            if (w < wave) woff += s_wt[w];
            tot += s_wt[w];
        }
        uint32_t run = woff + x - sum;
        for (int k = 0; k < PERC; k++)
            if (c0 + k < cells) { s_loc[c0 + k] = run; run += s_cnt[c0 + k]; }
        n_wg = min(tot, a.stage_cap);
        __syncthreads();
    }
    for (int i = tid; i < cells; i += BIN_THREADS) {
        const uint32_t c = s_cnt[i];
        if (PASS == 2) {
            uint32_t first = 0xffffffffu;
            if (c) {
                const uint32_t rel = atomicAdd(&a.cnt_copy[i], c);
                const uint64_t st = a.sched[i], room = a.sched[cells + i];
                if ((uint64_t)rel + c <= room && st + rel + c <= (uint64_t)a.cap) first = (uint32_t)(st + rel);
            }
            s_first[i] = first;
        } else {
            s_first[i] = c ? atomicAdd(&a.cur_copy[(size_t)(blockIdx.x & (a.copies - 1)) * cells + i], c) : 0u;
        }
        s_cnt[i] = 0;
    }
    if (PASS == 2) {
        if (tid == 0 && s_sum) atomicAdd(&a.ctrl[GFT_CTRL_RSUM], s_sum);
        asm volatile("s_waitcnt vmcnt(0)" ::: "memory");
        __syncthreads();
        if (tid == 0) {
            const uint32_t G = min((uint32_t)GFT_TICKET_WORDS, gridDim.x), grp = blockIdx.x % G;
            const uint32_t members = (gridDim.x - grp + G - 1u) / G;
            uint32_t last = 0u;
            if (atomicAdd(&a.ctrl[GFT_CTRL_WORDS + grp], 1u) == members - 1u)
                last = atomicAdd(&a.ctrl[GFT_CTRL_DONE], 1u) == G - 1u ? 1u : 0u;
            s_last = last;
        }
    }
    __syncthreads();
#pragma unroll
    for (int u = 0; u < BIN_ITEMS; u++) {
        if (!(r4[u].z > r4[u].x && r4[u].w > r4[u].y)) continue;
        const uint32_t idx = (uint32_t)(base + u * BIN_THREADS + tid);
        const int sx0 = r4[u].x >> ss, sx1 = (r4[u].z - 1) >> ss, sy0 = r4[u].y >> ss, sy1 = (r4[u].w - 1) >> ss;
        const int slab = (int)(bin[u] >> a.sh.kshift);
        for (int sy = sy0; sy <= sy1; sy++)
            for (int sx = sx0; sx <= sx1; sx++) {
                const int cell = (sy * sgx + sx) * K + slab;
                const int ox = sx << ss, oy = sy << ss, S = 1 << ss;
                const uint32_t x0 = (uint32_t)max((int)r4[u].x - ox, 0), x1 = (uint32_t)min((int)r4[u].z - ox, S);
                const uint32_t y0 = (uint32_t)max((int)r4[u].y - oy, 0), y1 = (uint32_t)min((int)r4[u].w - oy, S);
                const uint32_t hi = x0 | (y0 << 5) | (x1 << 10) | (y1 << 15) | (bin[u] << 20);
                const uint32_t rank = atomicAdd(&s_cnt[cell], 1u);
                const uint64_t e = ((uint64_t)hi << 32) | idx;
                const uint32_t pos = STAGED ? s_loc[cell] + rank : ~0u;
                if (STAGED && pos < a.stage_cap) {
                    stage_ent[pos] = e;
                    stage_cell[pos] = (uint16_t)cell;
                } else if (PASS != 2 || s_first[cell] != 0xffffffffu) {
                    a.sl_ent[s_first[cell] + rank] = e;
                }
            }
    }
    if (STAGED) {
        __syncthreads();
        for (uint32_t i = (uint32_t)tid; i < n_wg; i += BIN_THREADS) {
            const uint32_t cell = stage_cell[i];
            if (PASS != 2 || s_first[cell] != 0xffffffffu) a.sl_ent[s_first[cell] + (i - s_loc[cell])] = stage_ent[i];
        }
    }
    if (PASS != 2) return;
    if (!s_last) return;
    __syncthreads();
    if (tid == 0) {
        s_sum = 0;
        s_last = 1;
        s_carry = 0;
    }
    __syncthreads();
    {
        constexpr int PER = 4;
        bool ok = a.sched[2 * cells] == (uint32_t)cells && a.sched[2 * cells + 1] == 1u;
        uint32_t ent = 0;
        for (int c0 = 0; c0 < cells; c0 += PER * BIN_THREADS) {
            const int first = c0 + tid * PER;
            uint32_t c[PER], ncap[PER], sum = 0;
            uint64_t st[PER + 1], room[PER];
#pragma unroll
            for (int k = 0; k < PER; k++) {
                const int cell = min(first + k, cells - 1);
                c[k] = __hip_atomic_load(&a.cnt_copy[cell], __ATOMIC_RELAXED, __HIP_MEMORY_SCOPE_AGENT);
                st[k] = a.sched[cell];
                room[k] = a.sched[cells + cell];
            }
            st[PER] = first + PER < cells ? (uint64_t)a.sched[first + PER] : (uint64_t)a.cap;
#pragma unroll
            for (int k = 0; k < PER; k++) {
                const bool in = first + k < cells;
                const uint64_t nxt = first + k + 1 < cells ? st[k + 1] : (uint64_t)a.cap;
                if (in) {
                    ok = ok && c[k] <= room[k] && st[k] + room[k] <= nxt;
                    a.st_cnt[first + k] = c[k];
                    a.st_start[first + k] = (uint32_t)st[k];
                    ent += c[k];
                }
                ncap[k] = in ? c[k] + (c[k] >> 2) + 64u : 0u;
                sum += ncap[k];
            }
            uint32_t x = sum;
#pragma unroll
            for (int d = 1; d < 64; d <<= 1) {
                const uint32_t y = __shfl_up(x, d, 64);
                if (lane >= d) x += y;
            }
            if (lane == 63) s_wt[wave] = x;
            __syncthreads();
            uint32_t woff = 0;
            for (int w = 0; w < wave; w++) woff += s_wt[w];
            const uint32_t carry = s_carry;
            uint32_t run = carry + woff + x - sum;
#pragma unroll
            for (int k = 0; k < PER; k++)
                if (first + k < cells) { a.sched[first + k] = run; a.sched[cells + first + k] = ncap[k]; run += ncap[k]; }
            __syncthreads();
            if (tid == BIN_THREADS - 1) s_carry = carry + woff + x;
            __syncthreads();
        }
        ent = gft_wave_sum_u32_to_lane63(ent);
        if (lane == 63 && ent) atomicAdd(&s_sum, ent);
        if (!ok) s_last = 0;
        if (tid == 0) { a.sched[2 * cells] = (uint32_t)cells; a.sched[2 * cells + 1] = 1u; }
        __syncthreads();
    }
    const uint32_t entries_total = s_sum;
    const bool fits = s_last != 0u;
    if (tid == 0) {
        const uint32_t R = __hip_atomic_load(&a.ctrl[GFT_CTRL_RSUM], __ATOMIC_RELAXED, __HIP_MEMORY_SCOPE_AGENT);
        const uint32_t nhint = __hip_atomic_load(&a.ctrl[GFT_CTRL_NHINT], __ATOMIC_RELAXED, __HIP_MEMORY_SCOPE_AGENT);
        a.ctrl[GFT_CTRL_TOTAL] = fits ? R : 0xffffffffu;
        a.ctrl[GFT_CTRL_ENTRIES] = entries_total;
        a.ctrl[GFT_CTRL_MAXCNT] = 0u;
        if (a.mail) {
            a.mail[GFT_CTRL_TOTAL] = R;
            a.mail[GFT_CTRL_MAXCNT] = 0u;
            a.mail[GFT_CTRL_ENTRIES] = entries_total;
            a.mail[GFT_CTRL_NHINT] = nhint;
            if (!fits) __hip_atomic_fetch_or(&a.mail[GFT_CTRL_FLAGS], 2u, __ATOMIC_RELAXED, __HIP_MEMORY_SCOPE_SYSTEM);
            __hip_atomic_store(&a.mail[GFT_CTRL_SEQ], a.seq, __ATOMIC_RELEASE, __HIP_MEMORY_SCOPE_SYSTEM);
        }
    }
}

struct PullArgs {
    SuperShape sh;
    const float* __restrict__ depth;
    const uint32_t* __restrict__ st_cnt;
    const uint32_t* __restrict__ st_start;
    const uint64_t* __restrict__ sl_ent;
    uint2* __restrict__ ranges;
    uint32_t* __restrict__ heads;
    uint32_t* __restrict__ front_len;
    uint32_t* __restrict__ unit_flag;
    uint32_t* __restrict__ tile_cnt;
    uint32_t* __restrict__ tile_cut;
    uint8_t* __restrict__ need;
    uint32_t* ctrl;
    uint32_t cap;
    float4* __restrict__ clear; size_t clear_vec4;
    const uint32_t* __restrict__ hints;
    uint32_t pool_base;
    int dbg;
};

__device__ __forceinline__ bool pull_tile_of_block(const SuperShape& sh, int b, int& tile, int& q, uint32_t& lx, uint32_t& ly)
{
    const int S2 = 1 << (2 * sh.sshift);
    const int Np = sh.NS * S2;
    const int chunk = (Np + 7) >> 3;
    const int pos = (b & 7) * chunk + (b >> 3);
    if (pos >= Np) return false;
    q = pos >> (2 * sh.sshift);
    const int local = pos & (S2 - 1);
    lx = (uint32_t)(local & ((1 << sh.sshift) - 1));
    ly = (uint32_t)(local >> sh.sshift);
    const int tx = ((q % sh.sgx) << sh.sshift) + (int)lx, ty = ((q / sh.sgx) << sh.sshift) + (int)ly;
    if (tx >= sh.gx || ty >= sh.gy) return false;
    tile = ty * sh.gx + tx;
    return true;
}

template <bool WHOLE>
__global__ __launch_bounds__(GFT_BLOCK) __attribute__((amdgpu_waves_per_eu(WHOLE ? 5 : 7, 8))) void k_tile_pull(PullArgs a)
{
    __shared__ uint64_t sk[SORT_SLOTS(WHOLE ? TPULL_KEYS_BIG : TPULL_KEYS)];
    static_assert(sizeof(uint64_t) * SORT_SLOTS(TPULL_KEYS) >= sizeof(uint32_t) * GFT_DEPTH_BINS, "histogram fits the key buffer");
    uint32_t* s_hist = reinterpret_cast<uint32_t*>(sk);
    __shared__ uint32_t s_n, s_cut, s_kf, s_gmax, s_gmax2, s_bmin, s_bmax, s_pool;
    __shared__ uint32_t s_wt[GFT_BLOCK / 64];
    __shared__ uint32_t s_cur[PULL_WINDOW / 2];
    if (a.ctrl[GFT_CTRL_TOTAL] > a.cap) return;
    auto clear_slice = [&]() {
        if (!a.clear) return;
        const float4 z = make_float4(0.f, 0.f, 0.f, 0.f);
        for (size_t i = (size_t)blockIdx.x * GFT_BLOCK + threadIdx.x; i < a.clear_vec4; i += (size_t)gridDim.x * GFT_BLOCK)
            a.clear[i] = z;
    };
    const int tid = threadIdx.x, lane = tid & 63, wave = tid >> 6;
    int tile, q;
    uint32_t lx, ly;
    if (!pull_tile_of_block(a.sh, (int)blockIdx.x, tile, q, lx, ly)) { clear_slice(); return; }
    const int K = a.sh.K;
    const bool hinted = (PHASE_DBG(a) & 16) || (a.hints != nullptr && a.hints[tile] != 0u);
    for (int i = tid; i < GFT_DEPTH_BINS; i += GFT_BLOCK) s_hist[i] = 0;
    if (tid == 0) s_n = 0;
    __syncthreads();

    uint32_t win_base = 0;
    uint32_t cshift = 0;
    uint32_t pbits = 11, pmask = 0x7ffu;
    auto scan = [&](const int tid, const uint64_t* __restrict__ list, uint32_t ln, int mode, uint32_t blo, uint32_t bhi) {
        const int lane = tid & 63;
        uint64_t nx[4];
#pragma unroll
        for (int u = 0; u < 4; u++) nx[u] = list[min((uint32_t)(u * GFT_BLOCK + tid), ln - 1u)];
        for (uint32_t i0 = 0; i0 < ln; i0 += 4 * GFT_BLOCK) {
            uint64_t e4[4];
#pragma unroll
            for (int u = 0; u < 4; u++) e4[u] = nx[u];
#pragma unroll
            for (int u = 0; u < 4; u++) nx[u] = list[min(i0 + (uint32_t)((4 + u) * GFT_BLOCK + tid), ln - 1u)];
#pragma unroll
            for (int u = 0; u < 4; u++)
                if (i0 + u * GFT_BLOCK + tid >= ln) e4[u] = 0ull;
            bool hit[4];
            unsigned long long hm[4];
            uint32_t off[4], cnt = 0;
#pragma unroll
            for (int u = 0; u < 4; u++) {
                const uint32_t eb = entry_bin(e4[u]);
                hit[u] = entry_hits(e4[u], lx, ly) && (mode == 0 || (eb >= blo && eb < bhi));
                hm[u] = __builtin_amdgcn_ballot_w64(hit[u]);
                off[u] = cnt;
                cnt += (uint32_t)__popcll(hm[u]);
            }
            if (cnt == 0u) continue;
            if (mode == 2) {
                uint32_t d4[4];
#pragma unroll
                for (int u = 0; u < 4; u++) d4[u] = (PHASE_DBG(a) & 32) ? (uint32_t)e4[u] : __float_as_uint(a.depth[hit[u] ? (uint32_t)e4[u] : 0u]);
#pragma unroll
                for (int u = 0; u < 4; u++) {
                    if (!hit[u]) continue;
                    const uint32_t b = (entry_bin(e4[u]) - win_base) >> cshift;
                    const uint32_t w = atomicAdd(&s_cur[b >> 1], (b & 1u) ? 0x10000u : 1u);
                    const uint32_t pos = ((b & 1u) ? (w >> 16) : w) & pmask;
                    if (pos < (WHOLE ? TPULL_KEYS_BIG : TPULL_KEYS)) sk[pos] = ((uint64_t)d4[u] << 32) | (uint32_t)e4[u];
                }
                continue;
            }
            uint32_t hb = 0;
            if (lane == 0) hb = atomicAdd(&s_n, cnt);
            if (mode == 0) {
#pragma unroll
                for (int u = 0; u < 4; u++)
                    if (hit[u]) atomicAdd(&s_hist[entry_bin(e4[u])], 1u);
                continue;
            }
            hb = (uint32_t)__builtin_amdgcn_readfirstlane((int)hb);
            uint32_t d4[4];
#pragma unroll
            for (int u = 0; u < 4; u++) d4[u] = __float_as_uint(a.depth[hit[u] ? (uint32_t)e4[u] : 0u]);
#pragma unroll
            for (int u = 0; u < 4; u++) {
                if (!hit[u]) continue;
                const uint32_t id = (uint32_t)e4[u];
                const uint32_t pos = hb + off[u] + (uint32_t)__popcll(hm[u] & ((1ull << lane) - 1ull));
                if (pos < TPULL_KEYS) sk[pos] = ((uint64_t)d4[u] << 32) | id;
            }
        }
    };

    int kstop = K - 1;
    uint32_t n = 0;
    for (int k = 0; k < K; k++) {
        const uint32_t ln = a.st_cnt[q * K + k];
        if (ln) scan(tid, a.sl_ent + a.st_start[q * K + k], ln, 0, 0u, 0u);
        __syncthreads();
        n = s_n;
        __syncthreads();
        if (n >= (hinted ? (WHOLE ? 0xffffffffu : HEAD_DIRECT + 1u) : HEAD_TARGET)) { kstop = k; break; }
    }
    if ((PHASE_DBG(a) & 15) == 1) { if (tid < 4) a.unit_flag[4 * tile + tid] = 0; if (tid == 0) { a.ranges[tile] = make_uint2(0u, 0u); a.front_len[tile] = 0; a.tile_cut[tile] = GFT_NO_TAIL; } return; }
    bool more_slabs = false;
    for (int k = kstop + 1; k < K; k++) more_slabs |= a.st_cnt[q * K + k] != 0u;
    uint32_t h[16], sum = 0, run0, xin;
    {
#pragma unroll
        for (int k = 0; k < 16; k++) { h[k] = s_hist[16 * tid + k]; sum += h[k]; }
        uint32_t x = sum;
#pragma unroll
        for (int d = 1; d < 64; d <<= 1) {
            const uint32_t y = __shfl_up(x, d, 64);
            if (lane >= d) x += y;
        }
        if (lane == 63) s_wt[wave] = x;
        if (tid == 0) { s_gmax = 0; s_cut = GFT_DEPTH_BINS; s_kf = 0; }
        __syncthreads();
        for (int w = 0; w < wave; w++) x += s_wt[w];
        xin = x;
        run0 = x - sum;
    }
    bool whole = WHOLE && hinted && n > HEAD_DIRECT;
    if (WHOLE && whole) {
        uint32_t gm = 0;
#pragma unroll
        for (int k = 0; k < 16; k++) gm = max(gm, h[k]);
#pragma unroll
        for (int d = 32; d > 0; d >>= 1) gm = max(gm, (uint32_t)__shfl_xor((int)gm, d, 64));
        if (lane == 0 && gm) atomicMax(&s_gmax, gm);
        __syncthreads();
        whole = s_gmax <= 255u;
        if (whole && s_gmax <= 7u) { pbits = 12; pmask = 0xfffu; }
        __syncthreads();
    }
    uint32_t first_tail = (uint32_t)(kstop + 1) << a.sh.kshift, kf = n;
    if (!whole && n > HEAD_DIRECT) {
        const uint32_t tgt = hinted ? HEAD_DIRECT : HEAD_TARGET;
        uint32_t run = run0;
        if (run < tgt && xin >= tgt) {
#pragma unroll
            for (int k = 0; k < 16; k++) {
                const uint32_t before = run;
                run += h[k];
                if (before < tgt && run >= tgt) {
                    const bool take = !hinted && (run <= 1024u || (before < 512u && run <= TPULL_KEYS));
                    s_cut = (uint32_t)(16 * tid + k) + (take ? 1u : 0u);
                    s_kf = take ? run : before;
                }
            }
        }
        __syncthreads();
        first_tail = s_cut;
        kf = s_kf;
        __syncthreads();
    }
    uint32_t hp[4];
#pragma unroll
    for (int w = 0; w < 4; w++)
        hp[w] = min(h[4 * w], 255u) | (min(h[4 * w + 1], 255u) << 8) | (min(h[4 * w + 2], 255u) << 16) | (min(h[4 * w + 3], 255u) << 24);
    auto hcnt = [&](int k) -> uint32_t { return (hp[k >> 2] >> (8 * (k & 3))) & 255u; };

    if ((PHASE_DBG(a) & 15) == 2) { if (tid < 4) a.unit_flag[4 * tile + tid] = 0; if (tid == 0) { a.ranges[tile] = make_uint2(0u, 0u); a.front_len[tile] = 0; a.tile_cut[tile] = GFT_NO_TAIL; } return; }
    uint32_t start = (uint32_t)tile * GFT_HEAD_SLOT;
    if (WHOLE && whole) {
        if (tid == 0) {
            if (PHASE_DBG(a) & 256) s_pool = 0;
            else s_pool = atomicAdd(&a.ctrl[GFT_CTRL_POOLCUR], n);
        }
        __syncthreads();
        start = a.pool_base + s_pool;
        kf = n;
    }
    const bool has_tail = !whole && (kf < n || more_slabs);
    const uint2 bk_range = kf ? make_uint2(start, start + kf) : make_uint2(0u, 0u);
    const uint32_t bk_cut = has_tail ? first_tail : GFT_NO_TAIL;
    const int k_last = whole ? K - 1 : kstop;
    uint32_t* const list = a.heads + start;

    uint32_t done = 0, lo = 0;
    for (;;) {
        uint32_t hi = first_tail, c = kf;
        int tl = tid;
        if (WHOLE) asm volatile("" : "+v"(tl), "+v"(hp[0]), "+v"(hp[1]), "+v"(hp[2]), "+v"(hp[3]));
        const int ll = tl & 63;
        if (WHOLE && whole) {
            if (tl == 0) { s_cut = GFT_DEPTH_BINS; s_kf = n - done; }
            __syncthreads();
            const uint32_t lim = done + ((pbits == 12u ? TPULL_KEYS_BIG : TPULL_KEYS) - 1u);
            if (run0 < lim && xin >= lim) {
                uint32_t run = run0;
#pragma unroll
                for (int k = 0; k < 16; k++) {
                    const uint32_t before = run;
                    run += hcnt(k);
                    if (before < lim && run >= lim) { s_cut = (uint32_t)(16 * tl + k); s_kf = before - done; }
                }
            }
            __syncthreads();
            hi = s_cut;
            c = s_kf;
        }
        if (tl == 0) { s_gmax = 0; s_gmax2 = 0; s_bmin = GFT_DEPTH_BINS; s_bmax = 0; s_n = 0; }
        __syncthreads();
        {
            uint32_t gm = 0, gm2 = 0, first = GFT_DEPTH_BINS, last1 = 0;
#pragma unroll
            for (int k = 15; k >= 0; k--) {
                const uint32_t b = (uint32_t)(16 * tl + k);
                const uint32_t hb = (b >= lo && b < hi) ? hcnt(k) : 0u;
                gm = max(gm, hb);
                if (!(k & 1)) gm2 = max(gm2, hb + ((b + 1u >= lo && b + 1u < hi) ? hcnt(k + 1) : 0u));
                if (hb) { first = b; last1 = max(last1, b + 1u); }
            }
#pragma unroll
            for (int d = 32; d > 0; d >>= 1) {
                gm = max(gm, (uint32_t)__shfl_xor((int)gm, d, 64));
                gm2 = max(gm2, (uint32_t)__shfl_xor((int)gm2, d, 64));
                first = min(first, (uint32_t)__shfl_xor((int)first, d, 64));
                last1 = max(last1, (uint32_t)__shfl_xor((int)last1, d, 64));
            }
            if (ll == 0) {
                if (gm) atomicMax(&s_gmax, gm);
                if (gm2) atomicMax(&s_gmax2, gm2);
                atomicMin(&s_bmin, first);
                atomicMax(&s_bmax, last1);
            }
        }
        __syncthreads();
        win_base = s_bmin & ~15u;
        cshift = s_bmax > win_base + PULL_WINDOW ? 1u : 0u;
        const uint32_t cmax = 0xffffu >> pbits;
        const bool grouped = (cshift ? s_gmax2 : s_gmax) <= cmax && c <= pmask;
        if (grouped && (uint32_t)(16 * tl) >= win_base && (uint32_t)(16 * tl) < win_base + (PULL_WINDOW << cshift)) {
            uint32_t r = (uint32_t)(16 * tl) >= lo ? run0 - done : 0u;
            auto hb = [&](int k) -> uint32_t {
                const uint32_t b = (uint32_t)(16 * tl + k);
                return (b >= lo && b < hi) ? hcnt(k) : 0u;
            };
            if (cshift == 0u) {
#pragma unroll
                for (int k = 0; k < 16; k += 2) {
                    const uint32_t b = (uint32_t)(16 * tl + k) - win_base;
                    const uint32_t c0 = (r & pmask) | (min(hb(k), cmax) << pbits);
                    r += hb(k);
                    const uint32_t c1 = (r & pmask) | (min(hb(k + 1), cmax) << pbits);
                    r += hb(k + 1);
                    s_cur[b >> 1] = c0 | (c1 << 16);
                }
            } else {
#pragma unroll
                for (int k = 0; k < 16; k += 4) {
                    const uint32_t cw = ((uint32_t)(16 * tl + k) - win_base) >> 1;
                    const uint32_t n0 = hb(k) + hb(k + 1), n1 = hb(k + 2) + hb(k + 3);
                    const uint32_t c0 = (r & pmask) | (min(n0, cmax) << pbits);
                    r += n0;
                    const uint32_t c1 = (r & pmask) | (min(n1, cmax) << pbits);
                    r += n1;
                    s_cur[cw >> 1] = c0 | (c1 << 16);
                }
            }
        }
        __syncthreads();
        if (c) {
            for (int k = 0; k <= k_last; k++) {
                if (((uint32_t)k << a.sh.kshift) >= hi || (((uint32_t)k + 1u) << a.sh.kshift) <= lo) continue;
                const uint32_t ln = a.st_cnt[q * K + k];
                if (ln) scan(tl, a.sl_ent + a.st_start[q * K + k], ln, grouped ? 2 : 1, lo, hi);
            }
        }
        if (done == 0u) {
            if (tl == 0) {
                const bool cut_short = (PHASE_DBG(a) & 15) == 5;
                a.ranges[tile] = cut_short ? make_uint2(0u, 0u) : bk_range;
                a.front_len[tile] = cut_short ? 0u : kf;
                a.tile_cnt[tile] = n;
                a.tile_cut[tile] = cut_short ? GFT_NO_TAIL : bk_cut;
            }
            if (tl < 4) a.unit_flag[4 * tile + tl] = 0;
        }
        __syncthreads();
        if (!(PHASE_DBG(a) & 64)) for (uint32_t i = tl; i < c; i += GFT_BLOCK) a.need[(uint32_t)sk[i]] = 1;
        if (done == 0u && !(PHASE_DBG(a) & 128)) clear_slice();
        uint32_t* __restrict__ ids = list + done;
        if (c == 0u || (PHASE_DBG(a) & 15) == 5) {
        } else if (grouped) {
            for (uint32_t p = (uint32_t)tl; p < c; p += GFT_BLOCK) {
                const uint64_t key = sk[p];
                const uint32_t b = (gft_depth_bin((uint32_t)(key >> 32), a.sh.near_bits, a.sh.bin_shift) - win_base) >> cshift;
                const uint32_t w = s_cur[b >> 1];
                const uint32_t half = (b & 1u) ? (w >> 16) : (w & 0xffffu);
                const uint32_t end = half & pmask, g = half >> pbits, l0 = end - g;
                uint32_t below = 0;
                for (uint32_t qd = 0; qd < g; qd++) below += sk[l0 + qd] < key ? 1u : 0u;
                ids[l0 + below] = (uint32_t)key;
            }
        } else if (c <= 1024u) {
            const uint32_t npad = next_pow2(c < 2u ? 2u : c);
            for (uint32_t i = (uint32_t)tl + c; i < npad; i += GFT_BLOCK) sk[i] = ~0ull;
            __syncthreads();
            if (npad == 1024u) sort1024_by_rank_and_store(sk, c, tl, ids);
            else head_sort_and_store(sk, c, npad, tl, ids);
        } else {
            static_assert(TPULL_KEYS == 2048u, "k_tile_pull sorts at most 2048 keys at a time");
            uint64_t mine[TPULL_KEYS / GFT_BLOCK];
#pragma unroll
            for (int k = 0; k < (int)(TPULL_KEYS / GFT_BLOCK); k++) {
                const uint32_t i = (uint32_t)tl + k * GFT_BLOCK;
                mine[k] = i < c ? sk[i] : ~0ull;
            }
            __syncthreads();
#pragma unroll
            for (int k = 0; k < (int)(TPULL_KEYS / GFT_BLOCK); k++) sk[sort_slot((uint32_t)tl + k * GFT_BLOCK)] = mine[k];
            __syncthreads();
            bitonic_blocked<3, 8>(sk, tl);
            for (uint32_t i = (uint32_t)tl; i < c; i += GFT_BLOCK) ids[i] = (uint32_t)sk[sort_slot(i)];
        }
        if (!WHOLE || !whole) break;
        done += c;
        lo = hi;
        if (done >= n) break;
        __syncthreads();
    }
}

struct TailArgs {
    PreFwdArgs pre;
    SuperShape sh;
    const uint32_t* __restrict__ st_cnt;
    const uint32_t* __restrict__ st_start;
    const uint64_t* __restrict__ sl_ent;
    uint2* __restrict__ ranges;
    uint32_t* point_list;
    uint32_t pool_base;
    const uint32_t* __restrict__ front_len;
    const uint32_t* __restrict__ unit_flag;
    const uint32_t* __restrict__ tile_cut;
    uint32_t* ctrl;
    uint32_t cap;
    const uint32_t* __restrict__ quad_max;
    uint32_t* __restrict__ order;
    RenderFwdArgs render;
    int resume_here;
    int dbg;
};

__device__ __forceinline__ void tail_appearance(const TailArgs& a, uint32_t id, float phase_offset)
{
    if (a.pre.g.need[id] == 1) return;
    a.pre.g.need[id] = 3;
    const float px = a.pre.io.means3D[3 * id], py = a.pre.io.means3D[3 * id + 1], pz = a.pre.io.means3D[3 * id + 2];
    const Mat16 V = load_mat(a.pre.io.viewmatrix);
    const float vz = V.m[2] * px + V.m[6] * py + V.m[10] * pz + V.m[14];
    const float vx = V.m[0] * px + V.m[4] * py + V.m[8] * pz + V.m[12];
    const float vy = V.m[1] * px + V.m[5] * py + V.m[9] * pz + V.m[13];
    appearance_fwd(a.pre, (int)id, threadIdx.x & 63, nullptr, nullptr, px, py, pz, vx, vy, vz, phase_offset);
}

__global__ __launch_bounds__(TAIL_THREADS) void k_tail_build(TailArgs a)
{
    extern __shared__ uint64_t sk_dyn[];
    uint64_t* sk = sk_dyn;
    __shared__ uint32_t s_hist[GFT_DEPTH_BINS];
    __shared__ uint32_t s_m, s_pool, s_hi, s_chunk;
    __shared__ unsigned long long s_nearest;
    if (a.ctrl[GFT_CTRL_TOTAL] > a.cap) return;
    const float phase_offset = gft_offset_value(a.pre.io.phase_offset_dev, a.pre.c.phase_offset);
    const float dc_offset = gft_offset_value(a.render.dc_offset_dev, a.render.dc_offset);
    const uint32_t nflag = a.ctrl[GFT_CTRL_NFLAG];
    const int T = a.sh.T;
    if (a.order && blockIdx.x == 0 && a.ctrl[GFT_CTRL_FWDORDER] == 0u) {
        gft_tile_order_block(T, a.quad_max, a.order, nflag ? a.unit_flag : nullptr);
        if (threadIdx.x == 0) a.ctrl[GFT_CTRL_ORDER_OK] = 1u;
    }
    if (nflag == 0u) return;
    const int tid = threadIdx.x, lane = tid & 63;
    const int K = a.sh.K;
    {
        const int tile = (int)blockIdx.x;
        const uint4 f = reinterpret_cast<const uint4*>(a.unit_flag)[tile];
        if ((f.x | f.y | f.z | f.w) == 0u) return;
        const uint32_t first_tail = a.tile_cut[tile];
        if (first_tail == GFT_NO_TAIL) return;
        const uint32_t kf = a.front_len[tile];
        const int tx = tile % a.sh.gx, ty = tile / a.sh.gx;
        const int q = (ty >> a.sh.sshift) * a.sh.sgx + (tx >> a.sh.sshift);
        const uint32_t lx = (uint32_t)(tx & ((1 << a.sh.sshift) - 1)), ly = (uint32_t)(ty & ((1 << a.sh.sshift) - 1));
        const float qx = (float)(tx * GFT_TILE_X), qy = (float)(ty * GFT_TILE_Y);
        for (int i = tid; i < GFT_DEPTH_BINS; i += TAIL_THREADS) s_hist[i] = 0;
        if (tid == 0) { s_m = 0; s_nearest = ~0ull; }
        __syncthreads();
        uint32_t keep_id = 0xffffffffu;
        if (kf == 0u) {
            for (int k = 0; k < K; k++) {
                const uint32_t ln = a.st_cnt[q * K + k];
                const uint64_t* __restrict__ list = a.sl_ent + a.st_start[q * K + k];
                for (uint32_t i = tid; i < ln; i += TAIL_THREADS) {
                    const uint64_t e = list[i];
                    if (entry_hits(e, lx, ly) && entry_bin(e) >= first_tail)
                        atomicMin(&s_nearest, ((unsigned long long)__float_as_uint(a.pre.g.depth[(uint32_t)e]) << 32) | (uint32_t)e);
                }
            }
            __syncthreads();
            keep_id = (uint32_t)s_nearest;
        }
        auto scan = [&](int mode, uint32_t lo, uint32_t hi, uint32_t* dst) {
            for (int k = 0; k < K; k++) {
                if ((((uint32_t)k + 1u) << a.sh.kshift) <= lo || ((uint32_t)k << a.sh.kshift) > hi) continue;
                const uint32_t ln = a.st_cnt[q * K + k];
                const uint64_t* __restrict__ list = a.sl_ent + a.st_start[q * K + k];
                for (uint32_t i0 = 0; i0 < ln; i0 += TAIL_ITEMS * TAIL_THREADS) {
                    uint64_t e4[TAIL_ITEMS];
#pragma unroll
                    for (int u = 0; u < TAIL_ITEMS; u++) e4[u] = list[min(i0 + u * TAIL_THREADS + tid, ln - 1u)];
#pragma unroll
                    for (int u = 0; u < TAIL_ITEMS; u++)
                        if (i0 + u * TAIL_THREADS + tid >= ln) e4[u] = 0ull;
                    bool s4[TAIL_ITEMS];
                    float4 ra[TAIL_ITEMS], rb[TAIL_ITEMS];
                    uint32_t dz[TAIL_ITEMS];
#pragma unroll
                    for (int u = 0; u < TAIL_ITEMS; u++) {
                        const uint32_t b = entry_bin(e4[u]);
                        s4[u] = entry_hits(e4[u], lx, ly) && b >= lo && b <= hi;
                        const uint32_t id = s4[u] ? (uint32_t)e4[u] : 0u;
                        ra[u] = a.pre.g.rec_a[2 * id];
                        rb[u] = a.pre.g.rec_a[2 * id + 1];
                        dz[u] = __float_as_uint(a.pre.g.depth[id]);
                    }
#pragma unroll
                    for (int u = 0; u < TAIL_ITEMS; u++) {
                        const uint32_t id = (uint32_t)e4[u], b = entry_bin(e4[u]);
                        bool sv = s4[u];
                        if (sv)
                            sv = gft_splat_reaches_flagged(f.x, ra[u], rb[u], qx, qy) || gft_splat_reaches_flagged(f.y, ra[u], rb[u], qx + 8.f, qy) ||
                                 gft_splat_reaches_flagged(f.z, ra[u], rb[u], qx, qy + 8.f) || gft_splat_reaches_flagged(f.w, ra[u], rb[u], qx + 8.f, qy + 8.f) ||
                                 id == keep_id;
                        const unsigned long long sm = __builtin_amdgcn_ballot_w64(sv);
                        if (sm == 0ull) continue;
                        uint32_t hb = 0;
                        if (lane == 0) hb = atomicAdd(&s_m, (uint32_t)__popcll(sm));
                        hb = (uint32_t)__builtin_amdgcn_readfirstlane((int)hb);
                        if (!sv) continue;
                        const uint32_t pos = hb + (uint32_t)__popcll(sm & ((1ull << lane) - 1ull));
                        if (mode == 0) atomicAdd(&s_hist[b], 1u);
                        if (mode == 2) dst[pos] = id;
                        else if (pos < TAIL_LDS_KEYS) sk[sort_slot(pos)] = ((uint64_t)dz[u] << 32) | id;
                    }
                }
            }
        };
        auto finish_lds = [&](uint32_t n, uint32_t* dst) {
            __syncthreads();
            if (PHASE_DBG(a) != 3) for (uint32_t i = tid; i < n; i += TAIL_THREADS) tail_appearance(a, (uint32_t)sk[sort_slot(i)], phase_offset);
            if (PHASE_DBG(a) == 4) return;
            if (n <= 1024u) {
                const uint32_t runs = (n + 255u) >> 8;
                for (uint32_t i = tid + n; i < 256u * runs; i += TAIL_THREADS) sk[sort_slot(i)] = ~0ull;
                __syncthreads();
                const int wave = tid >> 6;
                if ((uint32_t)wave < runs) bitonic_blocked<2, 6, WaveSync>(sk + 256 * wave, lane, WaveSync());
                __syncthreads();
                for (uint32_t i = tid; i < 256u * runs; i += TAIL_THREADS) {
                    const uint32_t run = i >> 8, pos = i & 255u;
                    const uint64_t key = sk[256u * run + sort_slot(pos)];
                    if (key == ~0ull) continue;
                    uint32_t rank = pos;
                    for (uint32_t o = 0; o < runs; o++) {
                        if (o == run) continue;
                        const uint64_t* r = sk + 256u * o;
                        uint32_t lo = 0;
#pragma unroll
                        for (uint32_t step = 128; step > 0; step >>= 1)
                            if (r[sort_slot(lo + step - 1)] < key) lo += step;
                        if (r[sort_slot(lo)] < key) lo++;
                        rank += lo;
                    }
                    dst[rank] = (uint32_t)key;
                }
                __syncthreads();
                return;
            } else {
                static_assert(TAIL_LDS_KEYS == 4096u && TAIL_THREADS == 512, "one 4096-key network: 8 keys per thread");
                for (uint32_t i = tid + n; i < TAIL_LDS_KEYS; i += TAIL_THREADS) sk[sort_slot(i)] = ~0ull;
                __syncthreads();
                bitonic_blocked<3, 9>(sk, tid);
            }
            for (uint32_t i = tid; i < n; i += TAIL_THREADS) dst[i] = (uint32_t)sk[sort_slot(i)];
            __syncthreads();
        };
        if (PHASE_DBG(a) == 1) return;
        scan(0, first_tail, GFT_DEPTH_BINS - 1u, nullptr);
        __syncthreads();
        const uint32_t m = s_m;
        if (PHASE_DBG(a) == 2) return;
        if (tid == 0) s_pool = atomicAdd(&a.ctrl[GFT_CTRL_POOLCUR], kf + m);
        __syncthreads();
        uint32_t* list = a.point_list + a.pool_base + s_pool;
        const uint32_t* head = a.point_list + a.ranges[tile].x;
        for (uint32_t i = tid; i < kf; i += TAIL_THREADS) list[i] = head[i];
        if (m <= TAIL_LDS_KEYS) {
            finish_lds(m, list + kf);
        } else {
            uint32_t done = 0, lo = first_tail;
            while (done < m) {
                if (tid == 0) {
                    uint32_t hi = lo, c = s_hist[lo];
                    while (hi + 1u < GFT_DEPTH_BINS && c + s_hist[hi + 1u] <= TAIL_LDS_KEYS) c += s_hist[++hi];
                    s_hi = hi; s_chunk = c; s_m = 0;
                }
                __syncthreads();
                const uint32_t hi = s_hi, c = s_chunk;
                uint32_t* dst = list + kf + done;
                if (c <= TAIL_LDS_KEYS) {
                    if (c) { scan(1, lo, hi, nullptr); finish_lds(c, dst); }
                } else {
                    scan(2, lo, hi, dst);
                    __threadfence_block();
                    __syncthreads();
                    for (uint32_t i = tid; i < c; i += TAIL_THREADS) tail_appearance(a, dst[i], phase_offset);
                    auto ld = [&](uint32_t i) {
                        const uint32_t id = __hip_atomic_load(&dst[i], __ATOMIC_RELAXED, __HIP_MEMORY_SCOPE_WORKGROUP);
                        return ((uint64_t)__float_as_uint(a.pre.g.depth[id]) << 32) | id;
                    };
                    bitonic_ascending<TAIL_THREADS>(c, next_pow2(c), tid, ld,
                        [&](uint32_t i, uint64_t v) { __hip_atomic_store(&dst[i], (uint32_t)v, __ATOMIC_RELAXED, __HIP_MEMORY_SCOPE_WORKGROUP); },
                        [] { __threadfence_block(); __syncthreads(); });
                }
                done += c;
                lo = hi + 1u;
                __syncthreads();
            }
        }
        if (tid == 0) a.ranges[tile] = make_uint2(a.pool_base + s_pool, a.pool_base + s_pool + kf + m);
        __threadfence();
        __syncthreads();
        if (a.resume_here) {
            const int w = tid >> 6;
            const uint32_t fl = w == 0 ? f.x : w == 1 ? f.y : w == 2 ? f.z : f.w;
            if (w < 4 && fl != 0u) {
                float4* stage = reinterpret_cast<float4*>(sk_dyn) + (size_t)w * (RB * 4);
                render_fwd_walk(a.render, 4 * tile + w, lane, stage, stage + RB * 2, dc_offset);
            }
        }
    }
}

}

bool gft_tail_resumes()
{
    static const bool on = [] { const char* e = getenv("GFT_TAIL_RESUME"); return e ? atoi(e) != 0 : true; }();
    return on;
}

SuperShape gft_super_shape(const gft_config& c)
{
    static const int env_slabs = [] { const char* e = getenv("GFT_SLABS"); return e ? atoi(e) : 0; }();
    SuperShape sh;
    sh.gx = (c.W + GFT_TILE_X - 1) / GFT_TILE_X;
    sh.gy = (c.H + GFT_TILE_Y - 1) / GFT_TILE_Y;
    sh.T = sh.gx * sh.gy;
    sh.sshift = 1;
    for (;;) {
        const int S = 1 << sh.sshift;
        sh.sgx = (sh.gx + S - 1) / S;
        sh.sgy = (sh.gy + S - 1) / S;
        sh.NS = sh.sgx * sh.sgy;
        if (sh.NS <= GFT_SUPER_MAX) break;
        sh.sshift++;
    }
    int K = sh.sshift >= 2 ? 4 : 1;
    if (env_slabs == 1 || env_slabs == 2 || env_slabs == 4 || env_slabs == 8 || env_slabs == 16) K = env_slabs;
    sh.K = K;
    sh.kshift = 12;
    for (int k = K; k > 1; k >>= 1) sh.kshift--;
    const float nr = c.near_n > 1e-6f ? c.near_n : 1e-6f;
    const float fr = c.far_n > nr ? c.far_n : 2.0f * nr;
    uint32_t nb, fb;
    memcpy(&nb, &nr, 4);
    memcpy(&fb, &fr, 4);
    sh.near_bits = nb;
    sh.bin_shift = 0;
    while (((fb - nb) >> sh.bin_shift) >= (uint32_t)GFT_DEPTH_BINS - 1u) sh.bin_shift++;
    return sh;
}

bool gft_tile_pull_ok(const gft_config& c) { return gft_super_shape(c).sshift <= 4; }

constexpr size_t SUPER_SCATTER_LDS = 160 * 1024 - 256;
static_assert(SUPER_SCATTER_LDS >= (size_t)GFT_SUPER_CELLS * 8, "the direct scatter's two cell tables");

size_t gft_cell_sched_words_of(const gft_config& c) { const SuperShape sh = gft_super_shape(c); return 2 * (size_t)sh.NS * sh.K + 4; }

hipError_t gft_launch_super_bin(hipStream_t s, const gft_config& c, const GeomView& g, const ImgView& im, const BinView& b,
                                uint32_t* mail, uint32_t seq, int pass, uint32_t cap, const uint32_t* hints, uint32_t* sched,
                                int64_t status_cap)
{
    SuperArgs a;
    a.post = (status_cap >= 0 && mail) ? (uint32_t)status_cap + 1u : 0u;
    a.hints = pass != 1 ? hints : nullptr;
    a.sched = pass != 1 ? sched : nullptr;
    if (pass == 2 && !sched) return hipErrorInvalidValue;
    a.P = c.P;
    a.sh = gft_super_shape(c);
    a.rect = g.rect; a.depth = g.depth;
    a.cnt_copy = im.super_tab; a.cur_copy = im.super_tab + GFT_SUPER_CELLS;
    a.st_cnt = im.super_tab + 2 * GFT_SUPER_CELLS; a.st_start = im.super_tab + 3 * GFT_SUPER_CELLS;
    static const int env_copies = [] { const char* e = getenv("GFT_SUPER_COPIES"); return e ? atoi(e) : 0; }();
    a.copies = (env_copies == 1 || env_copies == 2 || env_copies == 4) ? env_copies : 8;
    while (a.copies > 1 && (size_t)a.copies * a.sh.NS * a.sh.K > (size_t)GFT_SUPER_CELLS) a.copies >>= 1;
    a.sl_ent = pass != 0 ? b.keys : nullptr;
    a.ctrl = im.ctrl; a.mail = mail; a.seq = seq; a.cap = cap;
    const int blocks = (c.P + BIN_CHUNK - 1) / BIN_CHUNK;
    const int cells = a.sh.NS * a.sh.K;
    a.stage_cap = 0;
    if (pass != 0 && cells >= 1024 && cells <= 4096) {
        const size_t room = SUPER_SCATTER_LDS - ((size_t)cells * 12 + 8);
        a.stage_cap = (uint32_t)((room / 10) & ~(size_t)3);
    }
    const size_t lds = a.stage_cap ? (size_t)cells * 12 + 8 + (size_t)a.stage_cap * 10
                                   : (size_t)cells * 2 * sizeof(uint32_t);
    {
        static std::atomic<uint64_t> done[5];
        hipError_t e = gft_lds_opt_in(reinterpret_cast<const void*>(&k_super_bin<0>), (size_t)GFT_SUPER_CELLS * 8, done[0]);
        if (e == hipSuccess) e = gft_lds_opt_in(reinterpret_cast<const void*>(&k_super_bin<1>), (size_t)GFT_SUPER_CELLS * 8, done[1]);
        if (e == hipSuccess) e = gft_lds_opt_in(reinterpret_cast<const void*>(&k_super_bin<1, true>), SUPER_SCATTER_LDS, done[2]);
        if (e == hipSuccess) e = gft_lds_opt_in(reinterpret_cast<const void*>(&k_super_bin<2>), (size_t)GFT_SUPER_CELLS * 8, done[3]);
        if (e == hipSuccess) e = gft_lds_opt_in(reinterpret_cast<const void*>(&k_super_bin<2, true>), SUPER_SCATTER_LDS, done[4]);
        if (e != hipSuccess) return e;
    }
    if (pass == 0) hipLaunchKernelGGL(k_super_bin<0>, dim3(blocks), dim3(BIN_THREADS), lds, s, a);
    else if (pass == 2 && a.stage_cap) hipLaunchKernelGGL((k_super_bin<2, true>), dim3(blocks), dim3(BIN_THREADS), lds, s, a);
    else if (pass == 2) hipLaunchKernelGGL(k_super_bin<2>, dim3(blocks), dim3(BIN_THREADS), lds, s, a);
    else if (a.stage_cap) hipLaunchKernelGGL((k_super_bin<1, true>), dim3(blocks), dim3(BIN_THREADS), lds, s, a);
    else hipLaunchKernelGGL(k_super_bin<1>, dim3(blocks), dim3(BIN_THREADS), lds, s, a);
    return hipGetLastError();
}

hipError_t gft_launch_tile_pull(hipStream_t s, const gft_config& c, const GeomView& g, const ImgView& im, const BinView& b,
                                uint32_t cap, float* clear, size_t clear_bytes, const uint32_t* hints, bool whole_lists)
{
    PullArgs a;
    a.sh = gft_super_shape(c);
    a.depth = g.depth;
    a.st_cnt = im.super_tab + 2 * GFT_SUPER_CELLS; a.st_start = im.super_tab + 3 * GFT_SUPER_CELLS;
    a.sl_ent = b.keys;
    a.ranges = im.ranges; a.heads = b.point_list; a.front_len = im.front_len; a.unit_flag = im.unit_flag;
    a.tile_cnt = im.tile_cnt; a.tile_cut = im.tile_cut; a.need = g.need;
    a.ctrl = im.ctrl; a.cap = cap;
    a.clear = reinterpret_cast<float4*>(clear); a.clear_vec4 = clear_bytes / 16;
    a.hints = hints; a.pool_base = (uint32_t)a.sh.T * GFT_HEAD_SLOT;
    a.dbg = 0;
#ifdef GFT_PHASE_DBG
    static const int dbg = [] { const char* e = getenv("GFT_PULL_DBG"); return e ? atoi(e) : 0; }();
    a.dbg = dbg;
    if ((dbg & 15) == 4) { a.clear = nullptr; a.dbg = dbg & 16; }
#endif
    const int Np = a.sh.NS << (2 * a.sh.sshift);
    if (whole_lists || (PHASE_DBG(a) & 16)) hipLaunchKernelGGL(k_tile_pull<true>, dim3(8 * ((Np + 7) / 8)), dim3(GFT_BLOCK), 0, s, a);
    else hipLaunchKernelGGL(k_tile_pull<false>, dim3(8 * ((Np + 7) / 8)), dim3(GFT_BLOCK), 0, s, a);
    return hipGetLastError();
}

hipError_t gft_launch_tail_build(hipStream_t s, const gft_config& c, const gft_forward_io& io, const GeomView& g,
                                 const ImgView& im, const BinView& b, uint32_t cap, bool want_order)
{
    TailArgs a;
    a.pre = gft_pre_fwd_args(c, io, g, im, nullptr, true);
    a.sh = gft_super_shape(c);
    a.st_cnt = im.super_tab + 2 * GFT_SUPER_CELLS; a.st_start = im.super_tab + 3 * GFT_SUPER_CELLS;
    a.sl_ent = b.keys;
    a.ranges = im.ranges; a.point_list = b.point_list; a.pool_base = (uint32_t)a.sh.T * GFT_HEAD_SLOT;
    a.front_len = im.front_len; a.unit_flag = im.unit_flag; a.tile_cut = im.tile_cut;
    a.ctrl = im.ctrl; a.cap = cap;
    a.quad_max = im.tile_max; a.order = want_order ? im.tile_order : nullptr;
    a.resume_here = gft_tail_resumes() ? 1 : 0;
    a.render = gft_render_fwd_args(c, io, g, im, b, true, cap, 2, true);
    a.dbg = 0;
#ifdef GFT_PHASE_DBG
    static const int tdbg = [] { const char* e = getenv("GFT_TAIL_DBG"); return e ? atoi(e) : 0; }();
    a.dbg = tdbg;
#endif
    const size_t lds = (size_t)SORT_SLOTS(TAIL_LDS_KEYS) * 8;
    {
        static std::atomic<uint64_t> done{0};
        const hipError_t e = gft_lds_opt_in(reinterpret_cast<const void*>(&k_tail_build), lds, done);
        if (e != hipSuccess) return e;
    }
    hipLaunchKernelGGL(k_tail_build, dim3(a.sh.T), dim3(TAIL_THREADS), lds, s, a);
    return hipGetLastError();
}
```

### include/gftorf_rast.h

```cpp
#ifndef GFTORF_RAST_H
#define GFTORF_RAST_H

#include <stddef.h>
#include <stdint.h>

#ifdef __cplusplus
extern "C" {
#endif

#define GFT_ABI_VERSION 16

#define GFT_NUM_CHANNELS 3
#define GFT_NUM_CHANNELS_PHASOR 7
#define GFT_NUM_CHANNELS_CWTOF 2
#define GFT_TILE_X 16
#define GFT_TILE_Y 16
#define GFT_ACC_STRIDE 16

typedef struct gft_config {
    int32_t P;
    int32_t D;
    int32_t M;
    int32_t M_p;
    int32_t W, H;
    float tanfovx, tanfovy;
    float scale_modifier;
    float near_n, far_n;
    float depth_range;
    float phase_offset, dc_offset;
    int32_t use_view_dependent_phase;
    int32_t prefiltered;
    int32_t debug;
    int32_t want_backward;
    int32_t acc_zeroed;
    int32_t grads_zeroed;
    int32_t grads_accumulate;
    int64_t bg_stride_c, bg_stride_y, bg_stride_x;
} gft_config;

typedef struct gft_forward_io {
    const float* bg;
    const float* means3D;
    const float* colors_precomp;
    const float* phasors_precomp;
    const float* opacities;
    const float* scales;
    const float* rotations;
    const float* cov3D_precomp;
    const float* viewmatrix;
    const float* projmatrix;
    const float* campos;
    const float* shs;
    const float* shs_p;
    void* geom;
    void* img;
    void* binning;
    float* out_color;
    float* out_phasor;
    float* out_depth;
    float* out_normal;
    float* out_acc;
    float* out_entropy;
    float* out_depth_distortion;
    float* out_amp_distortion;
    float* pixels;
    float* out_distribution;
    int32_t* radii;
    float* acc;
    void* grads_zero;
    size_t grads_zero_bytes;
    uint32_t* tile_hints;
    uint32_t* tile_weights;
    uint32_t* cell_sched;
    const float* phase_offset_dev;
    const float* dc_offset_dev;
} gft_forward_io;

typedef struct gft_backward_io {
    const float* bg;
    const float* means3D;
    const int32_t* radii;
    const float* scales;
    const float* rotations;
    const float* cov3D_precomp;
    const float* viewmatrix;
    const float* projmatrix;
    const float* campos;
    const float* shs;
    const float* shs_p;
    const float* opacities;
    const float* pixels;
    const float* dL_dout_color;
    const float* dL_dout_phasor;
    const float* dL_dout_depth;
    const float* dL_dout_acc;
    const float* dL_dout_depth_distortion;
    const void* geom;
    const void* img;
    const void* binning;
    float* acc;
    float* dL_dmeans3D;
    float* dL_dmeans2D;
    float* dL_dcolors;
    float* dL_dopacity;
    float* dL_dcov3D;
    float* dL_dsh;
    float* dL_dsh_p;
    float* dL_dscales;
    float* dL_drotations;
    float* dL_dphase_offset;
    float* dL_ddc_offset;
    float* det_partials;
    uint8_t* dirty_rows;
    uint32_t* rows_report;
    const float* phase_offset_dev;
    const float* dc_offset_dev;
} gft_backward_io;

typedef struct gft_layout {
    size_t geom_rec_a;
    size_t geom_rec_b;
    size_t geom_depth;
    size_t geom_tiles;
    size_t geom_rect;
    size_t geom_dirgrad;
    size_t geom_clamped;
    size_t geom_need;
    size_t geom_blockhist;
    size_t geom_total;
    size_t img_pix_state;
    size_t img_ranges;
    size_t img_tile_max;
    size_t img_ctrl;
    size_t img_tile_cnt;
    size_t img_tile_cut;
    size_t img_super_tab;
    size_t img_tile_cursor;
    size_t img_tile_order;
    size_t img_front_len;
    size_t img_unit_flag;
    size_t img_resume_state;
    size_t img_pix_sums;
    size_t img_snaps;
    size_t img_total;
    size_t bin_keys;
    size_t bin_point_list;
    size_t bin_total;
} gft_layout;

typedef struct gft_profile {
    double preprocess_fwd_ms, tile_count_ms, tile_scatter_ms, tile_sort_ms, render_fwd_ms;
    double render_bwd_ms, preprocess_bwd_ms, memset_ms;
    int64_t forward_calls, backward_calls;
} gft_profile;

int gft_abi_version(void);
int gft_lazy_sort(void);
const char* gft_last_error(void);

size_t gft_geom_bytes(int32_t P);
size_t gft_image_bytes(int32_t W, int32_t H);
size_t gft_cell_sched_words(int32_t W, int32_t H);
size_t gft_binning_bytes(int64_t R, int32_t W, int32_t H);
size_t gft_acc_bytes(int32_t P);
size_t gft_det_partials_bytes(int64_t binning_instances, int32_t W, int32_t H);
int64_t gft_binning_capacity(size_t bytes, int32_t W, int32_t H);
int gft_set_binning_mode(int mode);
int gft_binning_mode(const gft_config* cfg);
int gft_set_render_mode(int mode);
int gft_get_layout(int32_t P, int32_t W, int32_t H, int64_t R, gft_layout* out );

int gft_forward_preprocess(void* hip_stream, const gft_config* cfg,
                           const gft_forward_io* io, int64_t* num_rendered ,
                           int64_t* max_tile_list );

int gft_forward_render(void* hip_stream, const gft_config* cfg,
                       const gft_forward_io* io, int64_t binning_instances,
                       int64_t max_tile_list );

typedef struct gft_forward_hints {
    int64_t binning_instances;
    int64_t max_tile_list;
    int64_t whole_lists;
    int64_t use_cell_sched;
} gft_forward_hints;

typedef struct gft_forward_report {
    int64_t num_rendered;
    int64_t max_tile_list;
    int64_t list_entries;
    int64_t hinted_tiles;
    int64_t sched_misses;
} gft_forward_report;

int gft_forward(void* hip_stream, const gft_config* cfg, const gft_forward_io* io,
                const gft_forward_hints* hints, gft_forward_report* report );

#define GFT_STATUS_WORDS 16
#define GFT_STATUS_STICKY 12
#define GFT_STATUS_CAP 12
#define GFT_STATUS_OVERFLOWS 13
#define GFT_STATUS_MAX_R 14
int gft_forward_enqueue(void* hip_stream, const gft_config* cfg, const gft_forward_io* io,
                        const gft_forward_hints* hints, uint32_t* status );

int gft_backward(void* hip_stream, const gft_config* cfg,
                 const gft_backward_io* io, int64_t binning_instances);

int gft_grads_rezero(void* hip_stream, const gft_config* cfg, const gft_backward_io* io);

int gft_mark_visible(void* hip_stream, int32_t P, const float* means3D,
                     const float* viewmatrix, const float* projmatrix,
                     float near_n, float far_n, uint8_t* present);

int gft_profile_enable(int on);
int gft_profile_reset(void);
int gft_profile_read(gft_profile* out );

#ifdef __cplusplus
}
#endif
#endif
```

Measured before the change: 2647 it/s.

## Split super-cell depth slabs at an adaptive per-cell depth cut

Each super-cell slab is split into near and far segments at a per-supercell depth cut. The cut is learned from the previous frame's tail need, recorded by tile_pull through atomicMax. Binning counts and scatters both halves, with the far half filled from the end of the cell's room via a packed 64-bit atomic. The tile pull and tail-build scans then skip segments outside the needed depth range, so less of the far list gets rescanned. The cost is doubled cell tables, extra LDS, possibly fewer slabs or counter copies, and a schedule that now depends on state carried across frames.

Result: no change. 2671 it/s (median of 6 runs) (+0.9%).

```diff
diff --git a/gftorf_amd/_lib.py b/gftorf_amd/_lib.py
--- a/gftorf_amd/_lib.py
+++ b/gftorf_amd/_lib.py
@@ -126,7 +126,7 @@
                 ("step", C.c_int64)]
 
 EXPORTS = [
-    "gft_abi_version", "gft_lazy_sort", "gft_last_error", "gft_geom_bytes", "gft_image_bytes", "gft_cell_sched_words", "gft_binning_bytes", "gft_acc_bytes",
+    "gft_abi_version", "gft_lazy_sort", "gft_last_error", "gft_geom_bytes", "gft_image_bytes", "gft_cell_sched_words", "gft_cell_sched_cells", "gft_binning_bytes", "gft_acc_bytes",
     "gft_det_partials_bytes", "gft_get_layout", "gft_binning_capacity", "gft_set_binning_mode", "gft_binning_mode", "gft_set_render_mode", "gft_forward_preprocess", "gft_forward_render", "gft_forward", "gft_forward_enqueue", "gft_backward", "gft_grads_rezero",
     "gft_mark_visible", "gft_profile_enable", "gft_profile_reset", "gft_profile_read",
     "gft_assemble_scratch_bytes", "gft_assemble_forward", "gft_assemble_num_dynamic", "gft_assemble_backward",
@@ -205,6 +205,8 @@
     lib.gft_image_bytes.argtypes = [C.c_int32, C.c_int32]
     lib.gft_cell_sched_words.restype = C.c_size_t
     lib.gft_cell_sched_words.argtypes = [C.c_int32, C.c_int32]
+    lib.gft_cell_sched_cells.restype = C.c_size_t
+    lib.gft_cell_sched_cells.argtypes = [C.c_int32, C.c_int32]
     lib.gft_binning_bytes.restype = C.c_size_t
     lib.gft_binning_bytes.argtypes = [C.c_int64, C.c_int32, C.c_int32]
     lib.gft_acc_bytes.restype = C.c_size_t
diff --git a/gftorf_amd/api.py b/gftorf_amd/api.py
--- a/gftorf_amd/api.py
+++ b/gftorf_amd/api.py
@@ -549,8 +549,18 @@
     return R, cap, binning, int(max_list.value), False
 
 
+_sched_cells_of = {}
+
+
+def _sched_cells(lib, W, H):
+    n = _sched_cells_of.get((W, H))
+    if n is None:
+        n = _sched_cells_of[(W, H)] = int(lib.gft_cell_sched_cells(W, H))
+    return n
+
+
 def _forward_hinted(fr, hint, list_hint):
-    cap = _guess_cap(hint, (fr.cam.cell_sched.numel() - 4) // 2 if fr.use_sched else 0)
+    cap = _guess_cap(hint, _sched_cells(fr.lib, fr.W, fr.H) if fr.use_sched else 0)
     binning = fr.alloc_binning(cap)
     hints = fr.hints(cap, list_hint, fr.use_sched)
     report = _lib.ForwardReport()
diff --git a/gftorf_amd/csrc/gft_api.hip b/gftorf_amd/csrc/gft_api.hip
--- a/gftorf_amd/csrc/gft_api.hip
+++ b/gftorf_amd/csrc/gft_api.hip
@@ -65,7 +65,7 @@
     L->img_ctrl = o;        o += (GFT_CTRL_WORDS + GFT_TICKET_WORDS) * 4;
     L->img_tile_cnt = o;    o += T * 4;
     L->img_tile_cut = o;    o += T * 4;
-    L->img_super_tab = o;   o = align_up(o + 4 * (size_t)GFT_SUPER_CELLS * 4);
+    L->img_super_tab = o;   o = align_up(o + (4 * (size_t)GFT_SUPER_CELLS + GFT_SUPER_MAX) * 4);
     L->img_tile_cursor = o; o = align_up(o + T * 4);
     L->img_tile_order = o;  o = align_up(o + T * 4);
     L->img_front_len = o;   o = align_up(o + T * 4);
@@ -109,6 +109,7 @@
     v.tile_cnt = (uint32_t*)(b + L.img_tile_cnt);
     v.tile_cut = (uint32_t*)(b + L.img_tile_cut);
     v.super_tab = (uint32_t*)(b + L.img_super_tab);
+    v.super_cut = v.super_tab + 4 * (size_t)GFT_SUPER_CELLS;
     v.tile_cursor = (uint32_t*)(b + L.img_tile_cursor);
     v.tile_order = (uint32_t*)(b + L.img_tile_order);
     v.front_len = (uint32_t*)(b + L.img_front_len);
@@ -148,6 +149,14 @@
     memset(&c, 0, sizeof(c));
     c.W = W; c.H = H; c.near_n = 0.01f; c.far_n = 100.f;
     return (W > 0 && H > 0 && gft_tile_pull_ok(c)) ? gft_cell_sched_words_of(c) : 0;
+}
+
+extern "C" size_t gft_cell_sched_cells(int32_t W, int32_t H)
+{
+    gft_config c;
+    memset(&c, 0, sizeof(c));
+    c.W = W; c.H = H; c.near_n = 0.01f; c.far_n = 100.f;
+    return (W > 0 && H > 0 && gft_tile_pull_ok(c)) ? gft_cell_sched_cells_of(c) : 0;
 }
 
 extern "C" size_t gft_binning_bytes(int64_t R, int32_t W, int32_t H)
@@ -507,7 +516,8 @@
             StageTimer t(s, ST_TILE_SORT);
             const int T = ((cfg->W + GFT_TILE_X - 1) / GFT_TILE_X) * ((cfg->H + GFT_TILE_Y - 1) / GFT_TILE_Y);
             const uint32_t* th = gft_fwd_segmented(T) ? nullptr : io->tile_hints;
-            GFT_STAGE(s, cfg, "tile_pull", gft_launch_tile_pull(s, *cfg, g, im, b, cap, clear, clear_bytes, th, whole_lists && th));
+            GFT_STAGE(s, cfg, "tile_pull", gft_launch_tile_pull(s, *cfg, g, im, b, cap, clear, clear_bytes, th, whole_lists && th,
+                                                                  io->cell_sched));
         }
         {
             StageTimer t(s, ST_PRE_FWD);
diff --git a/gftorf_amd/csrc/gft_internal.h b/gftorf_amd/csrc/gft_internal.h
--- a/gftorf_amd/csrc/gft_internal.h
+++ b/gftorf_amd/csrc/gft_internal.h
@@ -45,6 +45,7 @@
     uint32_t* tile_cnt;
     uint32_t* tile_cut;
     uint32_t* super_tab;
+    uint32_t* super_cut;
     uint32_t* tile_cursor;
     uint32_t* tile_order;
     uint32_t* front_len;
@@ -85,6 +86,21 @@
 #define GFT_SLAB_MAX 16
 #define GFT_SUPER_CELLS (GFT_SUPER_MAX * GFT_SLAB_MAX)
 #define GFT_DEPTH_BINS 4096
+__host__ __device__ __forceinline__ uint32_t gft_cut_word(uint32_t w) { return (w == 0u || w > GFT_DEPTH_BINS) ? (uint32_t)GFT_DEPTH_BINS : w; }
+__host__ __device__ __forceinline__ uint32_t gft_next_cut(uint32_t cut_word, uint32_t need_word)
+{
+    const uint32_t cut = gft_cut_word(cut_word);
+    if (need_word == 0u) return cut;
+    if (need_word >= GFT_DEPTH_BINS) return GFT_DEPTH_BINS;
+    const uint32_t margin = (need_word >> 3) > 8u ? (need_word >> 3) : 8u;
+    if (need_word > cut || need_word + 2u * margin < cut) return need_word + margin < GFT_DEPTH_BINS ? need_word + margin : (uint32_t)GFT_DEPTH_BINS;
+    return cut;
+}
+__host__ __device__ __forceinline__ uint32_t gft_seg_first_bin(int kshift, uint32_t cut, int j)
+{
+    const uint32_t base = (uint32_t)(j >> 1) << kshift, top = base + (1u << kshift);
+    return (j & 1) ? (cut < base ? base : (cut > top ? top : cut)) : base;
+}
 #define GFT_HEAD_SLOT 2048u
 #define GFT_HEAD_DIRECT 2048u
 #define GFT_HEAD_TARGET 940u
@@ -166,8 +182,11 @@
                                 uint32_t* mail, uint32_t seq, int pass, uint32_t cap, const uint32_t* hints = nullptr,
                                 uint32_t* sched = nullptr, int64_t status_cap = -1);
 size_t gft_cell_sched_words_of(const gft_config& c);
+size_t gft_cell_sched_cells_of(const gft_config& c);
+bool gft_depth_cut_on();
 hipError_t gft_launch_tile_pull(hipStream_t s, const gft_config& c, const GeomView& g, const ImgView& im, const BinView& b,
-                                uint32_t cap, float* clear, size_t clear_bytes, const uint32_t* hints, bool whole_lists);
+                                uint32_t cap, float* clear, size_t clear_bytes, const uint32_t* hints, bool whole_lists,
+                                uint32_t* sched = nullptr);
 hipError_t gft_launch_tail_build(hipStream_t s, const gft_config& c, const gft_forward_io& io, const GeomView& g,
                                  const ImgView& im, const BinView& b, uint32_t cap, bool want_order);
 hipError_t gft_launch_render_fwd(hipStream_t s, const gft_config& c, const gft_forward_io& io,
diff --git a/gftorf_amd/csrc/k_pull.hip b/gftorf_amd/csrc/k_pull.hip
--- a/gftorf_amd/csrc/k_pull.hip
+++ b/gftorf_amd/csrc/k_pull.hip
@@ -49,6 +49,8 @@
     const uint32_t* __restrict__ hints;
     uint32_t stage_cap;
     uint32_t* sched;
+    uint32_t* frame_cut;
+    int cut_on;
 };
 
 __device__ inline void super_write_sched(uint32_t* sched, const uint32_t* counts, int cells, uint32_t* s_wt, uint32_t* s_carry)
@@ -62,7 +64,8 @@
         uint32_t cap[PER], sum = 0;
 #pragma unroll
         for (int k = 0; k < PER; k++) {
-            const uint32_t c = first + k < cells ? __hip_atomic_load(&counts[first + k], __ATOMIC_RELAXED, __HIP_MEMORY_SCOPE_AGENT) : 0u;
+            const uint32_t c = first + k < cells ? __hip_atomic_load(&counts[2 * (first + k)], __ATOMIC_RELAXED, __HIP_MEMORY_SCOPE_AGENT) +
+                                                   __hip_atomic_load(&counts[2 * (first + k) + 1], __ATOMIC_RELAXED, __HIP_MEMORY_SCOPE_AGENT) : 0u;
             cap[k] = first + k < cells ? c + (c >> 2) + 64u : 0u;
             sum += cap[k];
         }
@@ -88,21 +91,31 @@
     if (tid == 0) { sched[2 * cells] = (uint32_t)cells; sched[2 * cells + 1] = 1u; }
 }
 
+__device__ inline void super_close_cuts(const SuperArgs& a, const uint32_t* s_cutq)
+{
+    const int NS = a.sh.NS, cells = NS * a.sh.K;
+    for (int i = threadIdx.x; i < NS; i += BIN_THREADS) {
+        a.frame_cut[i] = s_cutq[i];
+        if (a.sched) { a.sched[2 * cells + 4 + i] = s_cutq[i]; a.sched[2 * cells + 4 + NS + i] = 0u; }
+    }
+}
+
 template <int PASS, bool STAGED = false>
 __global__ __launch_bounds__(BIN_THREADS) void k_super_bin(SuperArgs a)
 {
     extern __shared__ __attribute__((aligned(16))) uint32_t sb_dyn[];
     const int cells = a.sh.NS * a.sh.K;
+    const int vcells = 2 * cells;
     uint32_t* s_cnt = sb_dyn;
-    uint32_t* s_first = sb_dyn + cells;
-    uint32_t* s_loc = sb_dyn + 2 * cells;
+    uint32_t* s_first = sb_dyn + vcells;
+    uint32_t* s_loc = sb_dyn + 2 * vcells;
     __shared__ uint32_t s_last, s_sum, s_carry;
+    __shared__ uint32_t s_cutq[GFT_SUPER_MAX];
     __shared__ uint32_t s_wt[BIN_THREADS / 64];
     const int tid = threadIdx.x, lane = tid & 63, wave = tid >> 6;
     if (PASS == 1 && a.ctrl[GFT_CTRL_TOTAL] > a.cap) return;
-    for (int i = tid; i < cells; i += BIN_THREADS) s_cnt[i] = 0;
+    for (int i = tid; i < vcells; i += BIN_THREADS) s_cnt[i] = 0;
     if (tid == 0) s_sum = 0;
-    __syncthreads();
     if (PASS == 2 && blockIdx.x == 0 && a.hints) {
         uint32_t nh = 0;
         for (int t = tid; t < a.sh.T; t += BIN_THREADS) nh += a.hints[t] != 0u ? 1u : 0u;
@@ -121,6 +134,9 @@
         r4[u] = a.rect[idx];
         dbits[u] = __float_as_uint(a.depth[idx]);
     }
+    for (int i = tid; i < a.sh.NS; i += BIN_THREADS)
+        s_cutq[i] = PASS == 1 ? gft_cut_word(a.frame_cut[i])
+                  : (a.sched && a.cut_on) ? gft_next_cut(a.sched[2 * cells + 4 + i], a.sched[2 * cells + 4 + a.sh.NS + i]) : (uint32_t)GFT_DEPTH_BINS;
 #pragma unroll
     for (int u = 0; u < BIN_ITEMS; u++) {
         const bool in = base + u * BIN_THREADS + tid < a.P;
@@ -129,6 +145,7 @@
         bin[u] = tiles ? gft_depth_bin(dbits[u], a.sh.near_bits, a.sh.bin_shift) : 0u;
         mine += tiles;
     }
+    __syncthreads();
     if (PASS != 1) {
         mine = gft_wave_sum_u32_to_lane63(mine);
         if (lane == 63 && mine) atomicAdd(&s_sum, mine);
@@ -139,15 +156,18 @@
         const int sx0 = r4[u].x >> ss, sx1 = (r4[u].z - 1) >> ss, sy0 = r4[u].y >> ss, sy1 = (r4[u].w - 1) >> ss;
         const int slab = (int)(bin[u] >> a.sh.kshift);
         for (int sy = sy0; sy <= sy1; sy++)
-            for (int sx = sx0; sx <= sx1; sx++) atomicAdd(&s_cnt[(sy * sgx + sx) * K + slab], 1u);
+            for (int sx = sx0; sx <= sx1; sx++) {
+                const int q = sy * sgx + sx;
+                atomicAdd(&s_cnt[2 * (q * K + slab) + (bin[u] >= s_cutq[q] ? 1 : 0)], 1u);
+            }
     }
     __syncthreads();
     if (PASS == 0) {
-        const int rot = (int)(((uint64_t)blockIdx.x * (uint64_t)cells) / gridDim.x);
-        for (int i = tid; i < cells; i += BIN_THREADS) {
-            const int cidx = i + rot >= cells ? i + rot - cells : i + rot;
+        const int rot = (int)(((uint64_t)blockIdx.x * (uint64_t)vcells) / gridDim.x);
+        for (int i = tid; i < vcells; i += BIN_THREADS) {
+            const int cidx = i + rot >= vcells ? i + rot - vcells : i + rot;
             const uint32_t c = s_cnt[cidx];
-            if (c) atomicAdd(&a.cnt_copy[(size_t)(blockIdx.x & (a.copies - 1)) * cells + cidx], c);
+            if (c) atomicAdd(&a.cnt_copy[(size_t)(blockIdx.x & (a.copies - 1)) * vcells + cidx], c);
         }
         if (tid == 0 && s_sum) atomicAdd(&a.ctrl[GFT_CTRL_RSUM], s_sum);
         asm volatile("s_waitcnt vmcnt(0)" ::: "memory");
@@ -166,14 +186,14 @@
         __syncthreads();
         const int C = a.copies;
         constexpr int PER = 4;
-        for (int c0 = 0; c0 < cells; c0 += PER * BIN_THREADS) {
+        for (int c0 = 0; c0 < vcells; c0 += PER * BIN_THREADS) {
             const int first = c0 + tid * PER;
             uint32_t v[8][PER];
 #pragma unroll
             for (int cp = 0; cp < 8; cp++)
 #pragma unroll
                 for (int k = 0; k < PER; k++)
-                    v[cp][k] = __hip_atomic_load(&a.cnt_copy[(size_t)min(cp, C - 1) * cells + min(first + k, cells - 1)],
+                    v[cp][k] = __hip_atomic_load(&a.cnt_copy[(size_t)min(cp, C - 1) * vcells + min(first + k, vcells - 1)],
                                                  __ATOMIC_RELAXED, __HIP_MEMORY_SCOPE_AGENT);
             uint32_t tot[PER], mine_sum = 0;
 #pragma unroll
@@ -181,7 +201,7 @@
                 tot[k] = 0;
 #pragma unroll
                 for (int cp = 0; cp < 8; cp++) {
-                    if (cp >= C || first + k >= cells) v[cp][k] = 0u;
+                    if (cp >= C || first + k >= vcells) v[cp][k] = 0u;
                     tot[k] += v[cp][k];
                 }
                 mine_sum += tot[k];
@@ -201,13 +221,13 @@
 #pragma unroll
             for (int k = 0; k < PER; k++) {
                 const int cell = first + k;
-                if (cell < cells) {
+                if (cell < vcells) {
                     a.st_cnt[cell] = tot[k];
                     a.st_start[cell] = run;
                     uint32_t inner = run;
 #pragma unroll
                     for (int cp = 0; cp < 8; cp++) {
-                        if (cp < C) a.cur_copy[(size_t)cp * cells + cell] = inner;
+                        if (cp < C) a.cur_copy[(size_t)cp * vcells + cell] = inner;
                         inner += v[cp][k];
                     }
                 }
@@ -219,6 +239,7 @@
         }
         const uint32_t entries_total = s_carry;
         if (a.sched) super_write_sched(a.sched, a.st_cnt, cells, s_wt, &s_carry);
+        super_close_cuts(a, s_cutq);
         uint32_t nh = 0;
         if (a.hints) {
             for (int t = tid; t < a.sh.T; t += BIN_THREADS) nh += a.hints[t] != 0u ? 1u : 0u;
@@ -245,15 +266,15 @@
         }
         return;
     }
-    uint32_t* s_stage_cell_base = sb_dyn + 3 * cells;
-    uint64_t* stage_ent = reinterpret_cast<uint64_t*>(s_stage_cell_base + (cells & 1));
+    uint32_t* s_stage_cell_base = sb_dyn + 3 * vcells;
+    uint64_t* stage_ent = reinterpret_cast<uint64_t*>(s_stage_cell_base);
     uint16_t* stage_cell = reinterpret_cast<uint16_t*>(stage_ent + a.stage_cap);
     uint32_t n_wg = 0;
     if (STAGED) {
-        const int PERC = (cells + BIN_THREADS - 1) / BIN_THREADS;
+        const int PERC = (vcells + BIN_THREADS - 1) / BIN_THREADS;
         const int c0 = tid * PERC;
         uint32_t sum = 0;
-        for (int k = 0; k < PERC; k++) sum += c0 + k < cells ? s_cnt[c0 + k] : 0u;
+        for (int k = 0; k < PERC; k++) sum += c0 + k < vcells ? s_cnt[c0 + k] : 0u;
         uint32_t x = sum;
 #pragma unroll
         for (int d = 1; d < 64; d <<= 1) {
@@ -269,24 +290,35 @@
         }
         uint32_t run = woff + x - sum;
         for (int k = 0; k < PERC; k++)
-            if (c0 + k < cells) { s_loc[c0 + k] = run; run += s_cnt[c0 + k]; }
+            if (c0 + k < vcells) { s_loc[c0 + k] = run; run += s_cnt[c0 + k]; }
         n_wg = min(tot, a.stage_cap);
         __syncthreads();
     }
-    for (int i = tid; i < cells; i += BIN_THREADS) {
-        const uint32_t c = s_cnt[i];
-        if (PASS == 2) {
-            uint32_t first = 0xffffffffu;
-            if (c) {
-                const uint32_t rel = atomicAdd(&a.cnt_copy[i], c);
+    if (PASS == 2) {
+        unsigned long long* cnt64 = reinterpret_cast<unsigned long long*>(a.cnt_copy);
+        for (int i = tid; i < cells; i += BIN_THREADS) {
+            const uint32_t cn = s_cnt[2 * i], cf = s_cnt[2 * i + 1];
+            uint32_t fn = 0xffffffffu, ff = 0xffffffffu;
+            if (cn | cf) {
+                const unsigned long long old = atomicAdd(&cnt64[i], (unsigned long long)cn | ((unsigned long long)cf << 32));
+                const uint64_t reln = (uint32_t)old, relf = (uint32_t)(old >> 32);
                 const uint64_t st = a.sched[i], room = a.sched[cells + i];
-                if ((uint64_t)rel + c <= room && st + rel + c <= (uint64_t)a.cap) first = (uint32_t)(st + rel);
-            }
-            s_first[i] = first;
-        } else {
-            s_first[i] = c ? atomicAdd(&a.cur_copy[(size_t)(blockIdx.x & (a.copies - 1)) * cells + i], c) : 0u;
-        }
-        s_cnt[i] = 0;
+                if (reln + cn + relf + cf <= room && st + room <= (uint64_t)a.cap) {
+                    fn = (uint32_t)(st + reln);
+                    ff = (uint32_t)(st + room - relf - cf);
+                }
+            }
+            s_first[2 * i] = fn;
+            s_first[2 * i + 1] = ff;
+            s_cnt[2 * i] = 0;
+            s_cnt[2 * i + 1] = 0;
+        }
+    } else {
+        for (int i = tid; i < vcells; i += BIN_THREADS) {
+            const uint32_t c = s_cnt[i];
+            s_first[i] = c ? atomicAdd(&a.cur_copy[(size_t)(blockIdx.x & (a.copies - 1)) * vcells + i], c) : 0u;
+            s_cnt[i] = 0;
+        }
     }
     if (PASS == 2) {
         if (tid == 0 && s_sum) atomicAdd(&a.ctrl[GFT_CTRL_RSUM], s_sum);
@@ -310,7 +342,8 @@
         const int slab = (int)(bin[u] >> a.sh.kshift);
         for (int sy = sy0; sy <= sy1; sy++)
             for (int sx = sx0; sx <= sx1; sx++) {
-                const int cell = (sy * sgx + sx) * K + slab;
+                const int q = sy * sgx + sx;
+                const int cell = 2 * (q * K + slab) + (bin[u] >= s_cutq[q] ? 1 : 0);
                 const int ox = sx << ss, oy = sy << ss, S = 1 << ss;
                 const uint32_t x0 = (uint32_t)max((int)r4[u].x - ox, 0), x1 = (uint32_t)min((int)r4[u].z - ox, S);
                 const uint32_t y0 = (uint32_t)max((int)r4[u].y - oy, 0), y1 = (uint32_t)min((int)r4[u].w - oy, S);
@@ -348,12 +381,14 @@
         uint32_t ent = 0;
         for (int c0 = 0; c0 < cells; c0 += PER * BIN_THREADS) {
             const int first = c0 + tid * PER;
-            uint32_t c[PER], ncap[PER], sum = 0;
+            uint32_t c[PER], cfar[PER], ncap[PER], sum = 0;
             uint64_t st[PER + 1], room[PER];
 #pragma unroll
             for (int k = 0; k < PER; k++) {
                 const int cell = min(first + k, cells - 1);
-                c[k] = __hip_atomic_load(&a.cnt_copy[cell], __ATOMIC_RELAXED, __HIP_MEMORY_SCOPE_AGENT);
+                const unsigned long long both = __hip_atomic_load(reinterpret_cast<unsigned long long*>(a.cnt_copy) + cell, __ATOMIC_RELAXED, __HIP_MEMORY_SCOPE_AGENT);
+                cfar[k] = (uint32_t)(both >> 32);
+                c[k] = (uint32_t)both + cfar[k];
                 st[k] = a.sched[cell];
                 room[k] = a.sched[cells + cell];
             }
@@ -363,9 +398,11 @@
                 const bool in = first + k < cells;
                 const uint64_t nxt = first + k + 1 < cells ? st[k + 1] : (uint64_t)a.cap;
                 if (in) {
-                    ok = ok && c[k] <= room[k] && st[k] + room[k] <= nxt;
-                    a.st_cnt[first + k] = c[k];
-                    a.st_start[first + k] = (uint32_t)st[k];
+                    ok = ok && c[k] >= cfar[k] && c[k] <= room[k] && st[k] + room[k] <= nxt;
+                    a.st_cnt[2 * (first + k)] = c[k] - cfar[k];
+                    a.st_start[2 * (first + k)] = (uint32_t)st[k];
+                    a.st_cnt[2 * (first + k) + 1] = cfar[k];
+                    a.st_start[2 * (first + k) + 1] = (uint32_t)(st[k] + room[k] - cfar[k]);
                     ent += c[k];
                 }
                 ncap[k] = in ? c[k] + (c[k] >> 2) + 64u : 0u;
@@ -394,6 +431,7 @@
         if (lane == 63 && ent) atomicAdd(&s_sum, ent);
         if (!ok) s_last = 0;
         if (tid == 0) { a.sched[2 * cells] = (uint32_t)cells; a.sched[2 * cells + 1] = 1u; }
+        super_close_cuts(a, s_cutq);
         __syncthreads();
     }
     const uint32_t entries_total = s_sum;
@@ -420,6 +458,8 @@
     const float* __restrict__ depth;
     const uint32_t* __restrict__ st_cnt;
     const uint32_t* __restrict__ st_start;
+    const uint32_t* __restrict__ frame_cut;
+    uint32_t* need_post;
     const uint64_t* __restrict__ sl_ent;
     uint2* __restrict__ ranges;
     uint32_t* __restrict__ heads;
@@ -473,7 +513,10 @@
     int tile, q;
     uint32_t lx, ly;
     if (!pull_tile_of_block(a.sh, (int)blockIdx.x, tile, q, lx, ly)) { clear_slice(); return; }
-    const int K = a.sh.K;
+    const int NSEG = 2 * a.sh.K;
+    const uint32_t cutq = gft_cut_word(a.frame_cut[q]);
+    const uint32_t* __restrict__ seg_cnt = a.st_cnt + q * NSEG;
+    const uint32_t* __restrict__ seg_start = a.st_start + q * NSEG;
     const bool hinted = (PHASE_DBG(a) & 16) || (a.hints != nullptr && a.hints[tile] != 0u);
     for (int i = tid; i < GFT_DEPTH_BINS; i += GFT_BLOCK) s_hist[i] = 0;
     if (tid == 0) s_n = 0;
@@ -544,11 +587,13 @@
         }
     };
 
-    int kstop = K - 1;
+    int kstop = NSEG - 1;
     uint32_t n = 0;
-    for (int k = 0; k < K; k++) {
-        const uint32_t ln = a.st_cnt[q * K + k];
-        if (ln) scan(tid, a.sl_ent + a.st_start[q * K + k], ln, 0, 0u, 0u);
+    const uint32_t cnt0 = seg_cnt[0], cnt1 = seg_cnt[1], start0 = seg_start[0], start1 = seg_start[1];
+    for (int k = 0; k < NSEG; k++) {
+        const uint32_t ln = k == 0 ? cnt0 : k == 1 ? cnt1 : seg_cnt[k];
+        if (!ln) continue;
+        scan(tid, a.sl_ent + (k == 0 ? start0 : k == 1 ? start1 : seg_start[k]), ln, 0, 0u, 0u);
         __syncthreads();
         n = s_n;
         __syncthreads();
@@ -556,7 +601,8 @@
     }
     if ((PHASE_DBG(a) & 15) == 1) { if (tid < 4) a.unit_flag[4 * tile + tid] = 0; if (tid == 0) { a.ranges[tile] = make_uint2(0u, 0u); a.front_len[tile] = 0; a.tile_cut[tile] = GFT_NO_TAIL; } return; }
     bool more_slabs = false;
-    for (int k = kstop + 1; k < K; k++) more_slabs |= a.st_cnt[q * K + k] != 0u;
+    for (int k = kstop + 1; k < NSEG; k++) more_slabs |= seg_cnt[k] != 0u;
+    const bool split = !hinted && !(kstop & 1) && seg_cnt[kstop + 1] != 0u;
     uint32_t h[16], sum = 0, run0, xin;
     {
 #pragma unroll
@@ -587,8 +633,8 @@
         if (whole && s_gmax <= 7u) { pbits = 12; pmask = 0xfffu; }
         __syncthreads();
     }
-    uint32_t first_tail = (uint32_t)(kstop + 1) << a.sh.kshift, kf = n;
-    if (!whole && n > HEAD_DIRECT) {
+    uint32_t first_tail = gft_seg_first_bin(a.sh.kshift, cutq, kstop + 1), kf = n;
+    if (!whole && (n > HEAD_DIRECT || split)) {
         const uint32_t tgt = hinted ? HEAD_DIRECT : HEAD_TARGET;
         uint32_t run = run0;
         if (run < tgt && xin >= tgt) {
@@ -628,7 +674,7 @@
     const bool has_tail = !whole && (kf < n || more_slabs);
     const uint2 bk_range = kf ? make_uint2(start, start + kf) : make_uint2(0u, 0u);
     const uint32_t bk_cut = has_tail ? first_tail : GFT_NO_TAIL;
-    const int k_last = whole ? K - 1 : kstop;
+    const int k_last = whole ? NSEG - 1 : kstop;
     uint32_t* const list = a.heads + start;
 
     uint32_t done = 0, lo = 0;
@@ -717,9 +763,9 @@
         __syncthreads();
         if (c) {
             for (int k = 0; k <= k_last; k++) {
-                if (((uint32_t)k << a.sh.kshift) >= hi || (((uint32_t)k + 1u) << a.sh.kshift) <= lo) continue;
-                const uint32_t ln = a.st_cnt[q * K + k];
-                if (ln) scan(tl, a.sl_ent + a.st_start[q * K + k], ln, grouped ? 2 : 1, lo, hi);
+                if (gft_seg_first_bin(a.sh.kshift, cutq, k) >= hi || gft_seg_first_bin(a.sh.kshift, cutq, k + 1) <= lo) continue;
+                const uint32_t ln = seg_cnt[k];
+                if (ln) scan(tl, a.sl_ent + seg_start[k], ln, grouped ? 2 : 1, lo, hi);
             }
         }
         if (done == 0u) {
@@ -729,6 +775,7 @@
                 a.front_len[tile] = cut_short ? 0u : kf;
                 a.tile_cnt[tile] = n;
                 a.tile_cut[tile] = cut_short ? GFT_NO_TAIL : bk_cut;
+                if (a.need_post && n) atomicMax(&a.need_post[q], (hinted || !has_tail) ? (uint32_t)GFT_DEPTH_BINS : max(first_tail, 1u));
             }
             if (tl < 4) a.unit_flag[4 * tile + tl] = 0;
         }
@@ -782,6 +829,7 @@
     SuperShape sh;
     const uint32_t* __restrict__ st_cnt;
     const uint32_t* __restrict__ st_start;
+    const uint32_t* __restrict__ frame_cut;
     const uint64_t* __restrict__ sl_ent;
     uint2* __restrict__ ranges;
     uint32_t* point_list;
@@ -828,7 +876,7 @@
     }
     if (nflag == 0u) return;
     const int tid = threadIdx.x, lane = tid & 63;
-    const int K = a.sh.K;
+    const int NSEG = 2 * a.sh.K;
     {
         const int tile = (int)blockIdx.x;
         const uint4 f = reinterpret_cast<const uint4*>(a.unit_flag)[tile];
@@ -840,14 +888,15 @@
         const int q = (ty >> a.sh.sshift) * a.sh.sgx + (tx >> a.sh.sshift);
         const uint32_t lx = (uint32_t)(tx & ((1 << a.sh.sshift) - 1)), ly = (uint32_t)(ty & ((1 << a.sh.sshift) - 1));
         const float qx = (float)(tx * GFT_TILE_X), qy = (float)(ty * GFT_TILE_Y);
+        const uint32_t cutq = gft_cut_word(a.frame_cut[q]);
         for (int i = tid; i < GFT_DEPTH_BINS; i += TAIL_THREADS) s_hist[i] = 0;
         if (tid == 0) { s_m = 0; s_nearest = ~0ull; }
         __syncthreads();
         uint32_t keep_id = 0xffffffffu;
         if (kf == 0u) {
-            for (int k = 0; k < K; k++) {
-                const uint32_t ln = a.st_cnt[q * K + k];
-                const uint64_t* __restrict__ list = a.sl_ent + a.st_start[q * K + k];
+            for (int k = 0; k < NSEG; k++) {
+                const uint32_t ln = a.st_cnt[q * NSEG + k];
+                const uint64_t* __restrict__ list = a.sl_ent + a.st_start[q * NSEG + k];
                 for (uint32_t i = tid; i < ln; i += TAIL_THREADS) {
                     const uint64_t e = list[i];
                     if (entry_hits(e, lx, ly) && entry_bin(e) >= first_tail)
@@ -858,10 +907,10 @@
             keep_id = (uint32_t)s_nearest;
         }
         auto scan = [&](int mode, uint32_t lo, uint32_t hi, uint32_t* dst) {
-            for (int k = 0; k < K; k++) {
-                if ((((uint32_t)k + 1u) << a.sh.kshift) <= lo || ((uint32_t)k << a.sh.kshift) > hi) continue;
-                const uint32_t ln = a.st_cnt[q * K + k];
-                const uint64_t* __restrict__ list = a.sl_ent + a.st_start[q * K + k];
+            for (int k = 0; k < NSEG; k++) {
+                if (gft_seg_first_bin(a.sh.kshift, cutq, k + 1) <= lo || gft_seg_first_bin(a.sh.kshift, cutq, k) > hi) continue;
+                const uint32_t ln = a.st_cnt[q * NSEG + k];
+                const uint64_t* __restrict__ list = a.sl_ent + a.st_start[q * NSEG + k];
                 for (uint32_t i0 = 0; i0 < ln; i0 += TAIL_ITEMS * TAIL_THREADS) {
                     uint64_t e4[TAIL_ITEMS];
 #pragma unroll
@@ -1025,6 +1074,7 @@
     }
     int K = sh.sshift >= 2 ? 4 : 1;
     if (env_slabs == 1 || env_slabs == 2 || env_slabs == 4 || env_slabs == 8 || env_slabs == 16) K = env_slabs;
+    while (K > 1 && 2 * (size_t)sh.NS * K > (size_t)GFT_SUPER_CELLS) K >>= 1;
     sh.K = K;
     sh.kshift = 12;
     for (int k = K; k > 1; k >>= 1) sh.kshift--;
@@ -1041,10 +1091,17 @@
 
 bool gft_tile_pull_ok(const gft_config& c) { return gft_super_shape(c).sshift <= 4; }
 
-constexpr size_t SUPER_SCATTER_LDS = 160 * 1024 - 256;
+constexpr size_t SUPER_SCATTER_LDS = 160 * 1024 - 256 - GFT_SUPER_MAX * 4;
 static_assert(SUPER_SCATTER_LDS >= (size_t)GFT_SUPER_CELLS * 8, "the direct scatter's two cell tables");
 
-size_t gft_cell_sched_words_of(const gft_config& c) { const SuperShape sh = gft_super_shape(c); return 2 * (size_t)sh.NS * sh.K + 4; }
+size_t gft_cell_sched_cells_of(const gft_config& c) { const SuperShape sh = gft_super_shape(c); return (size_t)sh.NS * sh.K; }
+size_t gft_cell_sched_words_of(const gft_config& c) { const SuperShape sh = gft_super_shape(c); return 2 * (size_t)sh.NS * sh.K + 4 + 2 * (size_t)sh.NS; }
+
+bool gft_depth_cut_on()
+{
+    static const bool on = [] { const char* e = getenv("GFT_DEPTH_CUT"); return e ? atoi(e) != 0 : true; }();
+    return on;
+}
 
 hipError_t gft_launch_super_bin(hipStream_t s, const gft_config& c, const GeomView& g, const ImgView& im, const BinView& b,
                                 uint32_t* mail, uint32_t seq, int pass, uint32_t cap, const uint32_t* hints, uint32_t* sched,
@@ -1062,18 +1119,19 @@
     a.st_cnt = im.super_tab + 2 * GFT_SUPER_CELLS; a.st_start = im.super_tab + 3 * GFT_SUPER_CELLS;
     static const int env_copies = [] { const char* e = getenv("GFT_SUPER_COPIES"); return e ? atoi(e) : 0; }();
     a.copies = (env_copies == 1 || env_copies == 2 || env_copies == 4) ? env_copies : 8;
-    while (a.copies > 1 && (size_t)a.copies * a.sh.NS * a.sh.K > (size_t)GFT_SUPER_CELLS) a.copies >>= 1;
+    while (a.copies > 1 && (size_t)a.copies * 2 * a.sh.NS * a.sh.K > (size_t)GFT_SUPER_CELLS) a.copies >>= 1;
+    a.frame_cut = im.super_cut; a.cut_on = gft_depth_cut_on() ? 1 : 0;
     a.sl_ent = pass != 0 ? b.keys : nullptr;
     a.ctrl = im.ctrl; a.mail = mail; a.seq = seq; a.cap = cap;
     const int blocks = (c.P + BIN_CHUNK - 1) / BIN_CHUNK;
-    const int cells = a.sh.NS * a.sh.K;
+    const int cells = a.sh.NS * a.sh.K, vcells = 2 * cells;
     a.stage_cap = 0;
     if (pass != 0 && cells >= 1024 && cells <= 4096) {
-        const size_t room = SUPER_SCATTER_LDS - ((size_t)cells * 12 + 8);
+        const size_t room = SUPER_SCATTER_LDS - ((size_t)vcells * 12 + 8);
         a.stage_cap = (uint32_t)((room / 10) & ~(size_t)3);
     }
-    const size_t lds = a.stage_cap ? (size_t)cells * 12 + 8 + (size_t)a.stage_cap * 10
-                                   : (size_t)cells * 2 * sizeof(uint32_t);
+    const size_t lds = a.stage_cap ? (size_t)vcells * 12 + 8 + (size_t)a.stage_cap * 10
+                                   : (size_t)vcells * 2 * sizeof(uint32_t);
     {
         static std::atomic<uint64_t> done[5];
         hipError_t e = gft_lds_opt_in(reinterpret_cast<const void*>(&k_super_bin<0>), (size_t)GFT_SUPER_CELLS * 8, done[0]);
@@ -1092,12 +1150,15 @@
 }
 
 hipError_t gft_launch_tile_pull(hipStream_t s, const gft_config& c, const GeomView& g, const ImgView& im, const BinView& b,
-                                uint32_t cap, float* clear, size_t clear_bytes, const uint32_t* hints, bool whole_lists)
+                                uint32_t cap, float* clear, size_t clear_bytes, const uint32_t* hints, bool whole_lists,
+                                uint32_t* sched)
 {
     PullArgs a;
     a.sh = gft_super_shape(c);
     a.depth = g.depth;
     a.st_cnt = im.super_tab + 2 * GFT_SUPER_CELLS; a.st_start = im.super_tab + 3 * GFT_SUPER_CELLS;
+    a.frame_cut = im.super_cut;
+    a.need_post = (sched && gft_depth_cut_on()) ? sched + 2 * (size_t)a.sh.NS * a.sh.K + 4 + a.sh.NS : nullptr;
     a.sl_ent = b.keys;
     a.ranges = im.ranges; a.heads = b.point_list; a.front_len = im.front_len; a.unit_flag = im.unit_flag;
     a.tile_cnt = im.tile_cnt; a.tile_cut = im.tile_cut; a.need = g.need;
@@ -1123,6 +1184,7 @@
     a.pre = gft_pre_fwd_args(c, io, g, im, nullptr, true);
     a.sh = gft_super_shape(c);
     a.st_cnt = im.super_tab + 2 * GFT_SUPER_CELLS; a.st_start = im.super_tab + 3 * GFT_SUPER_CELLS;
+    a.frame_cut = im.super_cut;
     a.sl_ent = b.keys;
     a.ranges = im.ranges; a.point_list = b.point_list; a.pool_base = (uint32_t)a.sh.T * GFT_HEAD_SLOT;
     a.front_len = im.front_len; a.unit_flag = im.unit_flag; a.tile_cut = im.tile_cut;
diff --git a/include/gftorf_rast.h b/include/gftorf_rast.h
--- a/include/gftorf_rast.h
+++ b/include/gftorf_rast.h
@@ -161,6 +161,7 @@
 size_t gft_geom_bytes(int32_t P);
 size_t gft_image_bytes(int32_t W, int32_t H);
 size_t gft_cell_sched_words(int32_t W, int32_t H);
+size_t gft_cell_sched_cells(int32_t W, int32_t H);
 size_t gft_binning_bytes(int64_t R, int32_t W, int32_t H);
 size_t gft_acc_bytes(int32_t P);
 size_t gft_det_partials_bytes(int64_t binning_instances, int32_t W, int32_t H);
```
